# xuhao1/TaichiSLAM

Hardware: AMD Instinct MI355X
Metric: depth-frames/s integrated (640x480->512^3 TSDF) (higher is better)
Workload: dtype f16 storage / f32 + int64 fixed-point arithmetic; 1 GPU; BASELINE configs[1]: single 640x480 u16 depth stream (sphere room r=3 m, 1 deg/frame) -> DenseTSDF 512^3 / 2 cm, recast_step 2, max_ray 5 m; one stream+submap per GPU

## Files before the change

taichislam_amd/csrc/tsl_integrate.hip:

```cpp
#include "tsl_tsdf.hpp"
#include <hip/hip_ext.h>

namespace tsl {

#ifdef TSL_TIMING
#define TSL_T0() const int _wv = (blockIdx.x * (int)blockDim.x + (int)threadIdx.x) >> 6
#define TSL_TICK(F, k) do { long long _n = wall_clock64(); if (lane_id() == 0 && _wv < 16384) (F).dbg[_wv * 16 + (k)] = _n; } while (0)
#else
#define TSL_T0() do {} while (0)
#define TSL_TICK(F, k) do {} while (0)
#endif

#define SCATTER_TILE 4096

struct RayRegs { float pf0, pf1, pf2, d0, d1, d2, P0, P1, P2, w; long long qden; int n; };

__device__ __forceinline__ uint32_t wave_min_u32(uint32_t v)
{
    for (int d = 32; d > 0; d >>= 1) { const uint32_t o = (uint32_t)__shfl_xor((int)v, d); v = o < v ? o : v; }
    return v;
}
__device__ __forceinline__ RayRegs make_ray(const uint4 rec, int n, const FrameParams& P)
{
    RayRegs R;
    R.n = n;
    R.pf0 = h2f((h16)(rec.x & 0xffffu)); R.pf1 = h2f((h16)(rec.x >> 16)); R.pf2 = h2f((h16)(rec.y & 0xffffu));
    R.d0 = h2f((h16)(rec.y >> 16)); R.d1 = h2f((h16)(rec.z & 0xffffu)); R.d2 = h2f((h16)(rec.z >> 16));
    R.w = __uint_as_float(rec.w);
    R.qden = to_fix(R.w);
    R.P0 = R.pf0 + P.T[0]; R.P1 = R.pf1 + P.T[1]; R.P2 = R.pf2 + P.T[2];
    return R;
}
template <bool WITH_N = true>
__device__ __forceinline__ RayRegs load_ray(const FrameDev& F, const FrameParams& P, int r) { return make_ray(F.rayA[r], WITH_N ? F.rayN[r] : 0, P); }
__device__ __forceinline__ void step_voxel(const RayRegs& R, const FrameParams& P, int j, float* x, int* xi)
{
    const float jf = (float)j;
    x[0] = (R.d0 * jf) * P.vs + P.T[0]; x[1] = (R.d1 * jf) * P.vs + P.T[1]; x[2] = (R.d2 * jf) * P.vs + P.T[2];
    xi[0] = rnd_i(div_vs(x[0], P.vs, P.rvs, P.fastdiv)); xi[1] = rnd_i(div_vs(x[1], P.vs, P.rvs, P.fastdiv)); xi[2] = rnd_i(div_vs(x[2], P.vs, P.rvs, P.fastdiv));
}
__device__ __forceinline__ long long step_term(const RayRegs& R, const float* x)
{
    const float v0 = R.P0 - x[0], v1 = R.P1 - x[1], v2 = R.P2 - x[2];
    const float s2 = (v0 * v0 + v1 * v1) + v2 * v2;
    const float dist = s2 >= 1.2621774483536189e-29f ? sqrt_rn_norm(s2) : sqrt_rn(s2);
    const float dot = (v0 * R.pf0 + v1 * R.pf1) + v2 * R.pf2;
    const float sd = dist * (float)sgn_f(dot);
    return to_fix_wave(R.w * sd);
}
template <bool COOP = true>
__device__ __forceinline__ void mark_occupied(const MapDev& M, const FrameParams& P, const RayRegs& R)
{
    const int oi = rnd_i(div_vs(R.P0, P.vs, P.rvs, P.fastdiv)), oj = rnd_i(div_vs(R.P1, P.vs, P.rvs, P.fastdiv)), ok = rnd_i(div_vs(R.P2, P.vs, P.rvs, P.fastdiv));
    if (in_volume(M, oi, oj, ok)) {
        int l; const int b = brick_of(M, oi, oj, ok, &l);
        const int p = pool_claim<COOP>(M, P.slot, b);
        if (p >= 0) M.occ[(size_t)p * TSL_BRK3 + l] = 1;
    }
}
template <bool COOP = true>
__device__ __forceinline__ int frame_slot_slow(const MapDev& M, const FrameDev& F, int s, int b)
{
    const int sl = COOP ? claim_index(F.slot_tab + b, &F.counters[1], F.max_frame_bricks) : claim_index_1(F.slot_tab + b, &F.counters[1], F.max_frame_bricks);
    if (sl >= 0) {
        const int p = pool_claim<COOP>(M, s, b);
        if (p >= 0) { F.touched[sl] = p; F.touched_b[sl] = b; }
        else return -1;
    } else frame_fail(M, F, 2);
    return sl;
}
__device__ __forceinline__ int frame_slot(const MapDev& M, const FrameDev& F, int s, int b)
{
    const int sl = F.slot_tab[b];
    return sl >= 0 ? sl : frame_slot_slow(M, F, s, b);
}

__device__ __forceinline__ uint32_t apply_update(uint32_t old, long long qnum, long long qden)
{
    const float num = from_fix(qnum), den = from_fix(qden);
    const h16 T0 = (h16)(old & 0xffffu), W0 = (h16)(old >> 16);
    const h16 Tn = f2h((h2f(hmul(T0, W0)) + num) / (h2f(W0) + den));
    float wn = h2f(W0) + den; if (TSL_WMAX < wn) wn = TSL_WMAX;
    return (uint32_t)Tn | ((uint32_t)f2h(wn) << 16);
}
__device__ __forceinline__ uint32_t apply_update_f(uint32_t old, float num, float den)
{
    const h16 T0 = (h16)(old & 0xffffu), W0 = (h16)(old >> 16);
    const h16 Tn = f2h((h2f(hmul(T0, W0)) + num) / (h2f(W0) + den));
    float wn = h2f(W0) + den; if (TSL_WMAX < wn) wn = TSL_WMAX;
    return (uint32_t)Tn | ((uint32_t)f2h(wn) << 16);
}

template <int VARIANT>
__global__ void __launch_bounds__(256) k_integrate(MapDev M, FrameDev F, const FrameParams* __restrict__ Pp)
{
    const FrameParams& P = *Pp;
    const int split = P.split;
    const int gid = blockIdx.x * 256 + threadIdx.x;
    const int r = gid / split, sub = gid - r * split;
    const int nrays = *F.nrays;
    const bool live = r < nrays;
    long long n_ok = 0, n_oob = 0;
    RayRegs R; R.n = 0; R.qden = 0;
    if (live) { R = load_ray(F, P, r); if (sub == 0) mark_occupied(M, P, R); }
    int cur_b = -1; unsigned long long* cur_acc = nullptr;
    int nmax = R.n;
    if (VARIANT == 1) { for (int d = 32; d > 0; d >>= 1) { int o = __shfl_xor(nmax, d); nmax = o > nmax ? o : nmax; } }
    const int iters = (nmax + split - 1) / split;
    for (int it = 0; it < iters; ++it) {
        const int j = 1 + sub + it * split;
        const bool act = live && j <= R.n;
        unsigned long long* dst = nullptr;
        long long qn = 0;
        if (act) {
            float x[3]; int xi[3];
            step_voxel(R, P, j, x, xi);
            if (in_volume(M, xi[0], xi[1], xi[2])) {
                qn = step_term(R, x);
                int l; const int b = brick_of(M, xi[0], xi[1], xi[2], &l);
                if (b != cur_b) { cur_b = b; const int sl = frame_slot(M, F, P.slot, b); cur_acc = sl >= 0 ? F.acc + (size_t)sl * (TSL_BRK3 * 2) : nullptr; }
                if (cur_acc) { dst = cur_acc + (size_t)l * 2; ++n_ok; }
            } else ++n_oob;
        }
        if (VARIANT == 1) {
            const unsigned long long m = __ballot(dst != nullptr);
            if (m) {
                const int leader = (int)__builtin_ctzll(m);
                const unsigned long long lead = __shfl((unsigned long long)dst, leader);
                const bool same = (dst == nullptr) || ((unsigned long long)dst == lead);
                if (__all(same)) {
                    const long long sn = wave_sum_ll(dst ? qn : 0), sdn = wave_sum_ll(dst ? R.qden : 0);
                    if (lane_id() == leader) {
                        __hip_atomic_fetch_add(dst, (unsigned long long)sn, __ATOMIC_RELAXED, __HIP_MEMORY_SCOPE_AGENT);
                        __hip_atomic_fetch_add(dst + 1, (unsigned long long)sdn, __ATOMIC_RELAXED, __HIP_MEMORY_SCOPE_AGENT);
                    }
                    continue;
                }
            }
        }
        if (dst) {
            __hip_atomic_fetch_add(dst, (unsigned long long)qn, __ATOMIC_RELAXED, __HIP_MEMORY_SCOPE_AGENT);
            __hip_atomic_fetch_add(dst + 1, (unsigned long long)R.qden, __ATOMIC_RELAXED, __HIP_MEMORY_SCOPE_AGENT);
        }
    }
    n_ok = wave_sum_ll(n_ok); n_oob = wave_sum_ll(n_oob);
    if (lane_id() == 0) {
        if (n_ok) atomic_add_i64(&F.stats->steps, n_ok);
        if (n_oob) atomic_add_i64(&F.stats->steps_oob, n_oob);
    }
}

__global__ void __launch_bounds__(256) k_finalize(MapDev M, FrameDev F, const int* list, const int* nlist)
{
    const int ntouched = min(F.counters[1], F.max_frame_bricks);
    const int nwork = list ? min(*nlist, F.max_frame_bricks) : ntouched;
    long long uniq = 0;
    for (int q = blockIdx.x; q < nwork; q += gridDim.x) {
        const int sl = list ? list[q] : q;
        const int p = F.touched[sl];
        if (threadIdx.x == 0) M.touch[p] = 1;
        ulonglong2* acc = reinterpret_cast<ulonglong2*>(F.acc + (size_t)sl * (TSL_BRK3 * 2));
        uint32_t* tw = M.tw + (size_t)p * TSL_BRK3;
        int8_t* obs = M.obs + (size_t)p * TSL_BRK3;
        ulonglong2 a[TSL_BRK3 / 256]; uint32_t old[TSL_BRK3 / 256];
#pragma unroll
        for (int q = 0; q < TSL_BRK3 / 256; ++q) { a[q] = acc[q * 256 + threadIdx.x]; old[q] = tw[q * 256 + threadIdx.x]; }
#pragma unroll
        for (int q = 0; q < TSL_BRK3 / 256; ++q) {
            const int l = q * 256 + threadIdx.x;
            if (a[q].y != 0ull) {
                tw[l] = apply_update(old[q], (long long)a[q].x, (long long)a[q].y);
                obs[l] = 1;
                acc[l] = make_ulonglong2(0ull, 0ull);
                ++uniq;
            }
        }
    }
    for (int sl = blockIdx.x * 256 + threadIdx.x; sl < ntouched; sl += gridDim.x * 256) F.slot_tab[F.touched_b[sl]] = TSL_EMPTY;
    uniq = wave_sum_ll(uniq);
    if (lane_id() == 0 && uniq) atomic_add_i64(&F.stats->unique, uniq);
    if (!list && blockIdx.x == 0 && threadIdx.x == 0) F.stats->bricks = ntouched;
}

__device__ __forceinline__ int axis_coord(float d, float T, const FrameParams& P, int j) { return rnd_i(div_vs((d * (float)j) * P.vs + T, P.vs, P.rvs, P.fastdiv)); }
__device__ __forceinline__ int axis_cell(int c, int h, int N, int nb) { const int u = c + h; return u < 0 ? -1 : (u >= N ? nb : (u >> 4)); }

__device__ __forceinline__ int next_axis_event(float d, float inv_d, float T, const FrameParams& P, float t_over_vs, int j, int jb, int cell, int h, int N, int nb)
{
    if (j >= jb) return jb + 1;
    int bound;
    bool up;
    if (d > 0.0f) { if (cell >= nb) return jb + 1; up = true; bound = (cell < 0 ? 0 : min((cell + 1) * 16, N)) - h; }
    else if (d < 0.0f) { if (cell < 0) return jb + 1; up = false; bound = (cell >= nb ? N - 1 : cell * 16 - 1) - h; }
    else return jb + 1;
    const float est = ((float)bound + (up ? -0.5f : 0.5f) - t_over_vs) * inv_d;
    int e = (int)fminf(fmaxf(ceilf(est), (float)(j + 1)), (float)jb);
    #define TSL_PRED(q) (up ? (axis_coord(d, T, P, (q)) >= bound) : (axis_coord(d, T, P, (q)) <= bound))
    if (TSL_PRED(e)) { while (e - 1 > j && TSL_PRED(e - 1)) --e; }
    else { ++e; while (e <= jb && !TSL_PRED(e)) ++e; }
    #undef TSL_PRED
    return e;
}

#define LH_SIZE 1024
#define LH_EMPTY (-1)
template <int LOG2 = 10>
__device__ __forceinline__ int lh_slot(int* keys, int b)
{
    unsigned h = ((unsigned)b * 2654435761u) >> (32 - LOG2);
    for (int probe = 0; probe < (1 << LOG2); ++probe) {
        const int k = keys[h];
        if (k == b) return (int)h;
        if (k == LH_EMPTY) { const int old = atomicCAS(&keys[h], LH_EMPTY, b); if (old == LH_EMPTY || old == b) return (int)h; }
        h = (h + 1) & ((1u << LOG2) - 1u);
    }
    return -1;
}

#define SEG_RAY_SLOTS 16
#define SEG_LH_LOG2 9
#define SEG_LH (1 << SEG_LH_LOG2)
template <bool FUSED>
__global__ void __launch_bounds__(256) k_segments(MapDev M, BatchDev B)
{
    if ((int)blockIdx.y >= B.n) return;
    const FrameDev& F = B.f[blockIdx.y];
    const FrameParams& P = *B.p[blockIdx.y];
    __shared__ int s_key[SEG_LH];
    __shared__ int s_cnt[SEG_LH];
    TSL_T0();
    TSL_TICK(F, 8);
    for (int i = threadIdx.x; i < SEG_LH; i += 256) { s_key[i] = LH_EMPTY; s_cnt[i] = 0; }
    __syncthreads();
    TSL_TICK(F, 0);

    const int split = P.split;
    const int gid = blockIdx.x * 256 + threadIdx.x;
    const int r = gid / split, sub = gid - r * split;
    const int nrays = FUSED ? F.counters[6] : *F.nrays;
    long long n_ok = 0, n_oob = 0;
    const bool working = __any(r < nrays);
    const int spl = SEG_RAY_SLOTS / split;
    unsigned long long* myseg = F.seg + (size_t)gid * spl;
    int nslot = 0;
    bool ok = r < nrays;
    uint4 rec = make_uint4(0, 0, 0, 0);
    int nsteps = 0;
    if (FUSED) {
        const int lane = threadIdx.x & 63;
        bool big = false;
        int gn = 0, sl = 0;
        uint32_t first = 0;
        unsigned long long vkey = 0ull;
        ok = false;
        if (r < nrays && sub == 0) {
            sl = F.act[r];
            const uint4* sp = reinterpret_cast<const uint4*>(F.htab + sl);
            const uint4 w0 = sp[0], w1 = sp[1], w2 = sp[2], w3 = sp[3];
            vkey = ((unsigned long long)w0.x | ((unsigned long long)w0.y << 32)) - 1ull;
            gn = (int)w0.z;
            if (gn > H_INL) big = true;
            else {
                uint32_t id[H_INL] = { w0.w, w1.x, w1.y, w1.z, w1.w, w2.x, w2.y, w2.z, w2.w, w3.x, w3.y, w3.z, w3.w };
                uint2 pl[H_INL];
#pragma unroll
                for (int q = 0; q < H_INL; ++q) {
                    if (q >= gn) id[q] = 0xffffffffu;
                    pl[q] = q < gn ? F.pix[id[q]] : make_uint2(0u, 0u);
                }
                PixAcc A = {};
                for (int k = 0; k < gn; ++k) {
                    uint32_t best = 0xffffffffu; uint2 bp = make_uint2(0u, 0u);
#pragma unroll
                    for (int q = 0; q < H_INL; ++q) { const bool t = id[q] < best; best = t ? id[q] : best; bp.x = t ? pl[q].x : bp.x; bp.y = t ? pl[q].y : bp.y; }
#pragma unroll
                    for (int q = 0; q < H_INL; ++q) id[q] = id[q] == best ? 0xffffffffu : id[q];
                    if (k == 0) first = best;
                    if (P.tex) acc_colour(P, F, best, A);
                    acc_payload(bp, A);
                }
                ok = finish_ray(P, F, A, first, &rec, &nsteps);
            }
        }
        for (unsigned long long bm = __ballot(big); bm; bm &= bm - 1ull) {
            const int src = (int)__builtin_ctzll(bm);
            const int n = __shfl(gn, src), sl0 = __shfl(sl, src);
            const unsigned long long vk = ((unsigned long long)(uint32_t)__shfl((int)(vkey >> 32), src) << 32) | (unsigned long long)(uint32_t)__shfl((int)(uint32_t)vkey, src);
            const int nblk = (n + H_INL - 1) / H_INL;
            const uint32_t hmask = (1u << P.hlog2) - 1u;
            auto find_block = [&](int bq) -> int {
                if (bq == 0) return sl0;
                const unsigned long long k2 = h_key(vk, bq);
                uint32_t h = h_hash64(k2, P.hlog2);
                for (uint32_t probe = 0; probe <= hmask; ++probe) {
                    const unsigned long long cur = F.htab[h].key;
                    if (cur == k2) return (int)h;
                    if (cur == H_EMPTY) return -1;
                    h = (h + 1u) & hmask;
                }
                return -1;
            };
            const int mine = lane < nblk ? find_block(lane) : -1;
            const bool too_many = n > GROUP_BIG_CAP;
            if (too_many && lane == 0) atomicOr(M.err, 8);
            PixAcc A = {};
            long long last = -1; uint32_t f0 = 0;
            for (int k = 0; k < n && !too_many; ++k) {
                uint32_t best = 0xffffffffu;
                for (int bq = lane; bq < nblk; bq += 64) {
                    const int hs = bq == lane ? mine : find_block(bq);
                    if (hs < 0) continue;
                    const int cb = min(H_INL, n - bq * H_INL);
                    const uint32_t* ids = F.htab[hs].pix;
                    for (int q = 0; q < cb; ++q) { const uint32_t v = ids[q]; if ((long long)v > last && v < best) best = v; }
                }
                best = wave_min_u32(best);
                if (best == 0xffffffffu) break;
                if (k == 0) f0 = best;
                acc_pixel(P, F, best, A);
                last = (long long)best;
            }
            uint4 rc; int ns = 0;
            const bool k2 = A.cnt == n && finish_ray(P, F, A, f0, &rc, &ns, lane == src);
            if (lane == src) { rec = rc; nsteps = ns; ok = k2; first = f0; }
        }
        if (r < nrays && sub == 0) {
            F.rayA[r] = rec; F.rayFirst[r] = first;
            if (P.seq) {
                uint32_t u[3];
#pragma unroll
                for (int a = 0; a < 3; ++a) {
                    unsigned long long x = (vkey >> (2 - a)) & 0x1249249249249249ull;
                    x = (x | (x >> 2)) & 0x10c30c30c30c30c3ull; x = (x | (x >> 4)) & 0x100f00f00f00f00full; x = (x | (x >> 8)) & 0x1f0000ff0000ffull;
                    x = (x | (x >> 16)) & 0x1f00000000ffffull; x = (x | (x >> 32)) & 0x1fffffull;
                    u[a] = (uint32_t)x;
                }
                const unsigned long long nblk = (unsigned long long)(P.pcl_ext / P.pcl_blk), blk = (unsigned long long)P.pcl_blk;
                const unsigned long long kb = ((u[0] / P.pcl_blk) * nblk + (u[1] / P.pcl_blk)) * nblk + (u[2] / P.pcl_blk);
                const unsigned long long kl = ((u[0] % P.pcl_blk) * blk + (u[1] % P.pcl_blk)) * blk + (u[2] % P.pcl_blk);
                reinterpret_cast<unsigned long long*>(F.keys)[r] = kb * blk * blk * blk + kl;
                F.rayN[r] = ok ? nsteps : 0;
            }
        }
        block_count_add(&F.stats->v_pcl, r < nrays && sub == 0);
        block_count_add(&F.stats->v_skipped, r < nrays && sub == 0 && !ok);
        if (gid == 0) *F.nrays = nrays;
        const int src = lane - sub;
        rec.x = (uint32_t)__shfl((int)rec.x, src); rec.y = (uint32_t)__shfl((int)rec.y, src); rec.z = (uint32_t)__shfl((int)rec.z, src); rec.w = (uint32_t)__shfl((int)rec.w, src);
        nsteps = __shfl(nsteps, src);
        ok = __shfl((int)ok, src) != 0;
    }
    if (ok) {
        const RayRegs R = FUSED ? make_ray(rec, nsteps, P) : load_ray(F, P, r);
        if (sub == 0) mark_occupied(M, P, R);
        TSL_TICK(F, 1);
        const int len = (R.n + split - 1) / split;
        const int ja = 1 + sub * len, jb = min(R.n, ja + len - 1);
        const float d[3] = { R.d0, R.d1, R.d2 };
        const float id[3] = { __builtin_amdgcn_rcpf(R.d0), __builtin_amdgcn_rcpf(R.d1), __builtin_amdgcn_rcpf(R.d2) };
        const float tv[3] = { P.T[0] / P.vs, P.T[1] / P.vs, P.T[2] / P.vs };
        const int hh[3] = { M.hN, M.hN, M.hNz }, NN[3] = { M.N, M.N, M.Nz }, nb[3] = { M.nbx, M.nbx, M.nbz };
        if (ja <= jb) {
            int cell[3], ev[3];
#pragma unroll
            for (int a = 0; a < 3; ++a) {
                cell[a] = axis_cell(axis_coord(d[a], P.T[a], P, ja), hh[a], NN[a], nb[a]);
                ev[a] = next_axis_event(d[a], id[a], P.T[a], P, tv[a], ja, jb, cell[a], hh[a], NN[a], nb[a]);
            }
            int j = ja;
            while (j <= jb) {
                const int e = min(min(ev[0], ev[1]), ev[2]);
                const bool inside = cell[0] >= 0 && cell[0] < nb[0] && cell[1] >= 0 && cell[1] < nb[1] && cell[2] >= 0 && cell[2] < nb[2];
                if (inside) {
                    const int b = (cell[0] * M.nbx + cell[1]) * M.nbz + cell[2];
                    n_ok += e - j;
                    for (int j0 = j; j0 < e; j0 += SEG_MAX_CNT) {
                        const int cnt = min(e - j0, SEG_MAX_CNT);
                        const unsigned long long en = ((unsigned long long)b << STG_B_SHIFT) | ((unsigned long long)r << (SEG_CNT_BITS + SEG_J_BITS)) |
                                                      ((unsigned long long)j0 << SEG_CNT_BITS) | (unsigned long long)cnt;
                        bool stored = true;
                        if (nslot < spl) myseg[nslot++] = en;
                        else {
                            const long long pos = (long long)nrays * SEG_RAY_SLOTS + __hip_atomic_fetch_add(&F.counters[2], 1, __ATOMIC_RELAXED, __HIP_MEMORY_SCOPE_AGENT);
                            if (pos < F.seg_cap) F.seg[pos] = en; else { stored = false; frame_fail(M, F, 4); }
                        }
                        if (stored) {
                            const int hs = lh_slot<SEG_LH_LOG2>(s_key, b);
                            if (hs >= 0) atomicAdd(&s_cnt[hs], 1);
                            else if (__hip_atomic_fetch_add(&F.bhist[b], 1, __ATOMIC_RELAXED, __HIP_MEMORY_SCOPE_AGENT) == 0) {
                                const int q = __hip_atomic_fetch_add(&F.counters[1], 1, __ATOMIC_RELAXED, __HIP_MEMORY_SCOPE_AGENT);
                                if (q < F.max_frame_bricks) F.act_b[q] = b; else frame_fail(M, F, 2);
                            }
                        }
                    }
                } else n_oob += e - j;
                j = e;
                if (j > jb) break;
#pragma unroll
                for (int a = 0; a < 3; ++a) if (ev[a] == j) {
                    cell[a] += d[a] > 0.0f ? 1 : -1;
                    ev[a] = next_axis_event(d[a], id[a], P.T[a], P, tv[a], j, jb, cell[a], hh[a], NN[a], nb[a]);
                }
            }
        }
    }
    if (r < nrays) for (int q = nslot; q < spl; ++q) myseg[q] = ~0ull;
    TSL_TICK(F, 2);
    __syncthreads();
    TSL_TICK(F, 3);
    TSL_TICK(F, 5);
    for (int i = threadIdx.x; i < SEG_LH; i += 256) {
        const int c = s_cnt[i];
        const int b = c ? s_key[i] : 0;
        const bool first = c && __hip_atomic_fetch_add(&F.bhist[b], c, __ATOMIC_RELAXED, __HIP_MEMORY_SCOPE_AGENT) == 0;
        const int q = wave_reserve(&F.counters[1], first);
        if (first) { if (q < F.max_frame_bricks) F.act_b[q] = b; else frame_fail(M, F, 2); }
    }
    TSL_TICK(F, 6);
#ifdef TSL_TIMING
    if (lane_id() == 0 && _wv < 16384) F.dbg[_wv * 16 + 15] = working;
#endif
    (void)working;
    n_ok = wave_sum_ll(n_ok); n_oob = wave_sum_ll(n_oob);
    {
        __shared__ long long s_steps[2];
        if (threadIdx.x == 0) { s_steps[0] = 0; s_steps[1] = 0; }
        __syncthreads();
        if (lane_id() == 0) {
            if (n_ok) atomicAdd(reinterpret_cast<unsigned long long*>(&s_steps[0]), (unsigned long long)n_ok);
            if (n_oob) atomicAdd(reinterpret_cast<unsigned long long*>(&s_steps[1]), (unsigned long long)n_oob);
        }
        __syncthreads();
        if (threadIdx.x == 0) {
            if (s_steps[0]) atomic_add_i64(&F.stats->steps, s_steps[0]);
            if (s_steps[1]) atomic_add_i64(&F.stats->steps_oob, s_steps[1]);
        }
    }
}

__device__ __forceinline__ int plan_class(int w) { return w >= 2560 ? 0 : (w >= 1280 ? 1 : (w >= 512 ? 2 : 3)); }
__global__ void __launch_bounds__(256) k_plan(MapDev M, BatchDev B, int psegs, int unit_max, int unit_half)
{
    if ((int)blockIdx.y >= B.n) return;
    const int y = blockIdx.y;
    const FrameDev& F = B.f[y];
    const int listed = F.counters[1];
    const int nact = min(listed, F.max_frame_bricks);
    if ((int)blockIdx.x * 256 >= nact && blockIdx.x) return;
    const int i = blockIdx.x * 256 + threadIdx.x;
    int v = 0, b = 0, np = 0, pcls = -1, ucls = -1, tm = 0, wb = 0, tmu = 0, tmp = 0, wu = 0;
    if (i < nact) {
        b = F.act_b[i];
        v = F.bhist[b];
        int vq[TSL_NB];
#pragma unroll
        for (int q = 0; q < TSL_NB; ++q) { vq[q] = q < B.n ? B.f[q].bhist[b] : 0; if (vq[q] > 0) tm |= 1 << q; wb += vq[q]; }
        if (wb > unit_max) { tmp = tm; }
        else if (wb > unit_half) {
            int acc = 0;
#pragma unroll
            for (int q = 0; q < TSL_NB; ++q) if ((tm >> q) & 1) { if (2 * acc < wb) { tmu |= 1 << q; wu += vq[q]; } else tmp |= 1 << q; acc += vq[q]; }
        } else { tmu = tm; wu = wb; }
        if (tmu && (tmu & -tmu) == (1 << y)) ucls = plan_class(wu);
        if (((tmp >> y) & 1) && v > 0) { np = (v + psegs - 1) / psegs; pcls = plan_class((v + np - 1) / np); }
    }
    const int off = block_reserve_n(&F.counters[3], v);
    const int s0 = block_reserve_n(&B.f[0].counters[HDR_SLAB], np);
    int p0 = 0, u0 = 0;
    for (int c = 0; c < PLAN_NCLS; ++c) {
        const int q = block_reserve_n(&F.counters[HDR_PARTS + c], pcls == c ? np : 0); if (pcls == c) p0 = q;
        const int u = block_reserve_n(&B.f[0].counters[HDR_UNITS + c], ucls == c ? 1 : 0); if (ucls == c) u0 = u;
    }
    if (i < nact) {
        F.boffset[b] = off;
        F.bnseg[b] = v;
        const int pool = (np || ucls >= 0) ? pool_claim<false>(M, B.p[y]->slot, b) : -1;
        if (ucls >= 0) {
            if (u0 < B.f[0].unit_cap) B.f[0].unit_tab[(size_t)ucls * B.f[0].unit_cap + u0] = make_int4(b, wu, pool, tmu);
            else for (int q = 0; q < B.n; ++q) if ((tm >> q) & 1) frame_fail(M, B.f[q], 2);
        }
        if (np && pool >= 0) {
            if ((tmp & -tmp) == (1 << y)) {
                const int hi = __hip_atomic_fetch_add(&B.f[0].counters[HDR_HEAVY], 1, __ATOMIC_RELAXED, __HIP_MEMORY_SCOPE_AGENT);
                if (hi < B.f[0].max_frame_bricks) B.f[0].heavy_tab[hi] = make_int4(b, pool, tmp, 0);
                else for (int q = 0; q < B.n; ++q) if ((tm >> q) & 1) frame_fail(M, B.f[q], 2);
            }
            if (s0 + np > F.max_frame_bricks || np >= (1 << PART_NP_BITS) || p0 + np > F.part_cap) frame_fail(M, F, 2);
            else {
                F.bslab[b] = s0 | (np << SLAB_SLOT_BITS);
                const int per = (v + np - 1) / np;
                int4* tab = F.part_tab + (size_t)pcls * F.part_cap;
                for (int k = 0; k < np; ++k) {
                    const int pos = k * per, n = min(v, pos + per) - pos;
                    tab[p0 + k] = make_int4(off + pos, (int)((uint32_t)n | ((uint32_t)np << 16)), pool, s0 + k);
                }
            }
        }
    }
    if (i == 0) { F.stats->bricks = listed; if (listed > F.max_frame_bricks) frame_fail(M, F, 2); }
}

__global__ void __launch_bounds__(256) k_scatter(BatchDev B)
{
    if ((int)blockIdx.y >= B.n) return;
    const FrameDev& F = B.f[blockIdx.y];
    __shared__ int s_key[LH_SIZE];
    __shared__ int s_cnt[LH_SIZE];
    __shared__ int s_base[LH_SIZE];
    if (B.p[blockIdx.y]->group) {
        const int na = F.counters[6], nx = F.counters[7];
        for (int i = blockIdx.x * 256 + threadIdx.x; i < na + nx; i += gridDim.x * 256) {
            HSlot* const hs = F.htab + (i < na ? F.act[i] : F.actx[i - na]);
            hs->key = H_EMPTY; hs->cnt = 0;
        }
    }
    const int total = (int)min((long long)*F.nrays * SEG_RAY_SLOTS + F.counters[2], (long long)F.seg_cap);
    const int ntiles = (total + SCATTER_TILE - 1) / SCATTER_TILE;
    for (int tile = blockIdx.x; tile < ntiles; tile += gridDim.x) {
        for (int i = threadIdx.x; i < LH_SIZE; i += 256) { s_key[i] = LH_EMPTY; s_cnt[i] = 0; }
        __syncthreads();
        const int t0 = tile * SCATTER_TILE;
        unsigned long long key[SCATTER_TILE / 256]; int rank[SCATTER_TILE / 256]; int hs[SCATTER_TILE / 256];
#pragma unroll
        for (int q = 0; q < SCATTER_TILE / 256; ++q) {
            const int i = t0 + q * 256 + threadIdx.x;
            rank[q] = -1; hs[q] = -1;
            if (i < total) {
                key[q] = F.seg[i];
                if (key[q] != ~0ull) {
                    const int b = (int)(key[q] >> STG_B_SHIFT);
                    hs[q] = lh_slot<10>(s_key, b);
                    if (hs[q] >= 0) rank[q] = atomicAdd(&s_cnt[hs[q]], 1);
                    else rank[q] = F.boffset[b] + __hip_atomic_fetch_add(&F.bcursor[b], 1, __ATOMIC_RELAXED, __HIP_MEMORY_SCOPE_AGENT);
                }
            }
        }
        __syncthreads();
        for (int i = threadIdx.x; i < LH_SIZE; i += 256) {
            const int c = s_cnt[i];
            if (c) { const int b = s_key[i]; s_base[i] = F.boffset[b] + __hip_atomic_fetch_add(&F.bcursor[b], c, __ATOMIC_RELAXED, __HIP_MEMORY_SCOPE_AGENT); }
        }
        __syncthreads();
#pragma unroll
        for (int q = 0; q < SCATTER_TILE / 256; ++q)
            if (rank[q] >= 0) F.seg_sorted[(hs[q] >= 0 ? s_base[hs[q]] : 0) + rank[q]] = key[q];
        __syncthreads();
    }
}

#ifdef TSL_NOSWZ
__device__ __forceinline__ int acc_swz5(int l) { return l; }
#else
__device__ __forceinline__ int acc_swz5(int l) { return l ^ (((l >> 8) ^ (l >> 5)) & 31); }
#endif
struct StepK { float vs, rvs, T0, T1, T2; int hN, hNz; };

template <bool FASTDIV>
__device__ __forceinline__ void step_eval(const RayRegs& R, const StepK& K, int j, int* slot, float* qf)
{
    const float jf = (float)j;
    const float x0 = (R.d0 * jf) * K.vs + K.T0, x1 = (R.d1 * jf) * K.vs + K.T1, x2 = (R.d2 * jf) * K.vs + K.T2;
    const int i0 = rnd_i(div_vs(x0, K.vs, K.rvs, FASTDIV ? 1 : 0)), i1 = rnd_i(div_vs(x1, K.vs, K.rvs, FASTDIV ? 1 : 0)), i2 = rnd_i(div_vs(x2, K.vs, K.rvs, FASTDIV ? 1 : 0));
    *slot = acc_swz5((((i0 + K.hN) & 15) << 8) | (((i1 + K.hN) & 15) << 4) | ((i2 + K.hNz) & 15));
    const float v0 = R.P0 - x0, v1 = R.P1 - x1, v2 = R.P2 - x2;
    const float s2 = (v0 * v0 + v1 * v1) + v2 * v2;
    const float dist = sqrt_rn_norm(fmaxf(s2, 1.2621774483536189e-29f));
    const float dot = (v0 * R.pf0 + v1 * R.pf1) + v2 * R.pf2;
    const float sd = dot == 0.0f ? 0.0f : copysignf(dist, dot);
    *qf = rintf((R.w * sd) * TSL_FIX_SCALE);
}

__device__ __forceinline__ bool fits_i32(long long q) { return q == (long long)(int)q; }
__device__ __forceinline__ float from_fix32(long long q) { return (float)(int)q * (float)TSL_FIX_INV; }

#define FLUSH_CHUNK 4
template <int N>
__device__ __forceinline__ void apply_chunk(const uint32_t* old, const long long* qn, const long long* qd, uint32_t* nv, bool all_small)
{
    if (all_small) {
#pragma unroll
        for (int q = 0; q < N; ++q) nv[q] = apply_update_f(old[q], from_fix32(qn[q]), from_fix32(qd[q]));
    } else {
#pragma unroll
        for (int q = 0; q < N; ++q) nv[q] = apply_update_f(old[q], from_fix(qn[q]), from_fix(qd[q]));
    }
}

__device__ __forceinline__ int uni(int v) { return __builtin_amdgcn_readfirstlane(v); }
#define IT_UNIT 0
#define IT_POOL 1
#define IT_SLAB 2
#define IT_NP   3
#define IT_TMALL 4
#define IT_FMASK 5
#define IT_OFF  6
#define IT_N    (IT_OFF + TSL_NB)
#define IT_WORDS (IT_N + TSL_NB + 2)
#define NRANGE (PLAN_NCLS * (TSL_NB + 1))

template <bool TEX, bool FASTDIV, int NT, int SPT, int WPE>
__global__ void __launch_bounds__(NT, WPE) k_integrate_batch(MapDev M, BatchDev B, int kind)
{
    constexpr int CSEGS = SPT * NT, VPT = TSL_BRK3 / NT, CH = VPT < FLUSH_CHUNK ? VPT : FLUSH_CHUNK;
    static_assert(VPT <= 16, "the written / first-touch masks hold 16 voxels per thread");
#ifdef TSL_EXP_SLOT16
    __shared__ ulonglong2 s_acc[TSL_BRK3];
#define S_NUM(i) s_acc[i].x
#define S_DEN(i) s_acc[i].y
#else
    __shared__ unsigned long long s_num[TSL_BRK3];
    __shared__ unsigned long long s_den[TSL_BRK3];
#define S_NUM(i) s_num[i]
#define S_DEN(i) s_den[i]
#endif
    __shared__ unsigned long long s_keys[CSEGS];
    __shared__ uint32_t s_win[TEX ? TSL_BRK3 : 1];
    __shared__ int s_bin[64];
    __shared__ int s_claim[2];
    __shared__ int s_uq[TSL_NB];
    __shared__ int s_cum[NRANGE + 1];
    __shared__ int s_it[3][IT_WORDS];
    uint32_t okmask = 0u;
#pragma unroll
    for (int q = 0; q < TSL_NB; ++q) if (q < B.n) {
        const FrameDev& Fq = B.f[q];
        if (Fq.counters[HDR_FAIL] == 0) okmask |= 1u << q;
        const int nact = min(Fq.counters[1], Fq.max_frame_bricks);
        for (int i = blockIdx.x * NT + threadIdx.x; i < nact; i += gridDim.x * NT) { const int b = Fq.act_b[i]; Fq.bhist[b] = 0; Fq.bcursor[b] = 0; }
    }
    if (threadIdx.x < TSL_NB) s_uq[threadIdx.x] = 0;
    if (threadIdx.x == 0) {
        int acc = 0, k = 0;
#ifdef TSL_CLASS_MAJOR
        for (int c = 0; c < PLAN_NCLS; ++c) {
            s_cum[k++] = acc; acc += min(B.f[0].counters[HDR_UNITS + c], B.f[0].unit_cap);
            for (int q = 0; q < TSL_NB; ++q) { s_cum[k++] = acc; if ((okmask >> q) & 1u) acc += min(B.f[q].counters[HDR_PARTS + c], B.f[q].part_cap); }
        }
#else
        for (int c = 0; c < PLAN_NCLS; ++c) { s_cum[k++] = acc; if (kind != 2) acc += min(B.f[0].counters[HDR_UNITS + c], B.f[0].unit_cap); }
        for (int c = 0; c < PLAN_NCLS; ++c)
            for (int q = 0; q < TSL_NB; ++q) { s_cum[k++] = acc; if (kind != 1 && ((okmask >> q) & 1u)) acc += min(B.f[q].counters[HDR_PARTS + c], B.f[q].part_cap); }
#endif
        s_cum[NRANGE] = acc;
        s_claim[0] = __hip_atomic_fetch_add(&B.f[0].counters[kind == 2 ? HDR_CLAIM2 : HDR_CLAIM], 1, __ATOMIC_RELAXED, __HIP_MEMORY_SCOPE_AGENT);
    }
    __syncthreads();
    const int total = uni(s_cum[NRANGE]);
    int* const claim = &B.f[0].counters[kind == 2 ? HDR_CLAIM2 : HDR_CLAIM];
    auto entry_of = [&](int r, int* kq) -> int4 {
        int k = 0;
#pragma unroll
        for (int j = 1; j < NRANGE; ++j) k += r >= uni(s_cum[j]) ? 1 : 0;
#ifdef TSL_CLASS_MAJOR
        const int local = r - uni(s_cum[k]), cls = k / (TSL_NB + 1), sub = k - cls * (TSL_NB + 1);
#else
        const int local = r - uni(s_cum[k]), cls = k < PLAN_NCLS ? k : (k - PLAN_NCLS) / TSL_NB, sub = k < PLAN_NCLS ? 0 : 1 + (k - PLAN_NCLS) % TSL_NB;
#endif
        *kq = sub - 1;
        if (sub == 0) return B.f[0].unit_tab[(size_t)cls * B.f[0].unit_cap + local];
        const FrameDev& Fq = B.f[sub - 1];
        return Fq.part_tab[(size_t)cls * Fq.part_cap + local];
    };
    auto info_of = [&](const int4 e, int kq, int* io, int* in) {
        *io = 0; *in = 0;
        const int q = threadIdx.x;
        if (q < TSL_NB) {
            if (kq < 0) { if ((((uint32_t)e.w) & okmask) >> q & 1u) { *io = B.f[q].boffset[e.x]; *in = B.f[q].bnseg[e.x]; } }
            else if (q == kq) { *io = e.x; *in = e.y & 0xffff; }
        }
    };
    auto commit = [&](int slot, const int4 e, int kq, int io, int in) {
        int* it = s_it[slot];
        if (threadIdx.x < TSL_NB) { it[IT_OFF + threadIdx.x] = io; it[IT_N + threadIdx.x] = in; }
        if (threadIdx.x == 0) {
            const uint32_t tm = kq < 0 ? (uint32_t)e.w & okmask : 1u << kq;
            uint32_t fm = tm;
            int pool = e.z;
            if (fm == 0u) { fm = 1u; pool = -1; }
            it[IT_UNIT] = kq < 0 ? 1 : 0; it[IT_POOL] = pool; it[IT_SLAB] = kq < 0 ? 0 : e.w; it[IT_NP] = kq < 0 ? 1 : (e.y >> 16) & ((1 << PART_NP_BITS) - 1);
            it[IT_TMALL] = (int)tm; it[IT_FMASK] = (int)fm;
        }
    };
    const int r0 = uni(s_claim[0]);
    if (r0 >= total) return;
    { int kq, io, in; const int4 e = entry_of(r0, &kq); info_of(e, kq, &io, &in); commit(0, e, kq, io, in); }
    __syncthreads();
    auto steps_of = [&](int sl, uint32_t fm) -> int {
        int n = 0;
#pragma unroll
        for (int q = 0; q < TSL_NB; ++q) if ((fm >> q) & 1u) n += max(1, (uni(s_it[sl][IT_N + q]) + CSEGS - 1) / CSEGS);
        return n;
    };
    long long uniq = 0;
    int t = 0, slot = 0, c = 0; (void)t;
    int n_known = 0;
    bool exhausted = false;
    int f = __builtin_ctz((uint32_t)uni(s_it[0][IT_FMASK]));

    unsigned long long kk[SPT]; uint4 recs[SPT]; uint32_t wids[SPT];
#define TSL_SORT_DEAL(KIN, NSEG, FD)                                                                                    \
    {                                                                                                                   \
        int rr[SPT];                                                                                                    \
        _Pragma("unroll") for (int q = 0; q < SPT; ++q) {                                                               \
            const int i = q * NT + (int)threadIdx.x; rr[q] = -1;                                                        \
            if (i < (NSEG)) rr[q] = atomicAdd(&s_bin[63 - (int)(KIN[q] & 63ull)], 1);                                   \
        }                                                                                                               \
        __syncthreads();                                                                                                \
        if (threadIdx.x < 64) {                                                                                         \
            const int cb = s_bin[threadIdx.x]; int inc = cb;                                                            \
            for (int d = 1; d < 64; d <<= 1) { const int o = __shfl_up(inc, d); if ((int)threadIdx.x >= d) inc += o; }  \
            s_bin[threadIdx.x] = inc - cb;                                                                              \
        }                                                                                                               \
        __syncthreads();                                                                                                \
        _Pragma("unroll") for (int q = 0; q < SPT; ++q) if (rr[q] >= 0) s_keys[s_bin[63 - (int)(KIN[q] & 63ull)] + rr[q]] = KIN[q]; \
        __syncthreads();                                                                                                \
        _Pragma("unroll") for (int q = 0; q < SPT; ++q) {                                                               \
            const int i = q * NT + ((q & 1) ? NT - 1 - (int)threadIdx.x : (int)threadIdx.x);                            \
            if (i < (NSEG)) {                                                                                           \
                kk[q] = s_keys[i];                                                                                      \
                const int r = (int)((kk[q] >> (SEG_CNT_BITS + SEG_J_BITS)) & ((1u << STG_RAY_BITS) - 1));               \
                recs[q] = (FD).rayA[r];                                                                                 \
                wids[q] = TEX ? (FD).rayFirst[r] + 1u : 0u;                                                             \
            }                                                                                                           \
        }                                                                                                               \
        if (threadIdx.x < 64) s_bin[threadIdx.x] = 0;               \
    }
#define TSL_PRIME(SL, FQ)                                                                                               \
    {                                                                                                                   \
        const FrameDev& F0 = B.f[FQ];                                                                                   \
        const int off0 = uni(s_it[SL][IT_OFF + (FQ)]), nseg0 = min(uni(s_it[SL][IT_N + (FQ)]), CSEGS);                  \
        unsigned long long k0[SPT];                                                                                     \
        _Pragma("unroll") for (int q = 0; q < SPT; ++q) { const int i = q * NT + threadIdx.x; k0[q] = i < nseg0 ? F0.seg_sorted[off0 + i] : 0ull; } \
        TSL_SORT_DEAL(k0, nseg0, F0)                                                                                    \
    }

    {
#ifdef TSL_EXP_SLOT16
        for (int i = threadIdx.x; i < TSL_BRK3; i += NT) s_acc[i] = make_ulonglong2(0ull, 0ull);
#else
        ulonglong2* zn = reinterpret_cast<ulonglong2*>(s_num); ulonglong2* zd = reinterpret_cast<ulonglong2*>(s_den);
        for (int i = threadIdx.x; i < TSL_BRK3 / 2; i += NT) { zn[i] = make_ulonglong2(0ull, 0ull); zd[i] = make_ulonglong2(0ull, 0ull); }
#endif
        if (TEX) for (int i = threadIdx.x; i < TSL_BRK3; i += NT) s_win[i] = 0u;
        if (threadIdx.x < 64) s_bin[threadIdx.x] = 0;
        __syncthreads();
        TSL_PRIME(0, f)
    }
    uint32_t old[VPT];
    uint32_t vmask = 0u;
    bool have_old = false;
    for (;;) {
        const int* const it = s_it[slot];
        const int slot1 = slot == 2 ? 0 : slot + 1, slot2 = slot == 0 ? 2 : slot - 1;
        const bool unit = uni(it[IT_UNIT]) != 0;
        const int p = uni(it[IT_POOL]), rk = uni(it[IT_SLAB]);
        const uint32_t fmask = (uint32_t)uni(it[IT_FMASK]);
        const int n_f = uni(it[IT_N + f]);
        const FrameDev& F = B.f[f];
        const FrameParams& P = *B.p[f];
        const StepK K = { P.vs, P.rvs, P.T[0], P.T[1], P.T[2], M.hN, M.hNz };
        const uint32_t later = fmask >> (f + 1);
        const bool first_frame = (fmask & ((1u << f) - 1u)) == 0u, last_frame = later == 0u;
        const bool first_step = first_frame && c == 0;
        const int nseg = min(CSEGS, n_f - c * CSEGS);
        const bool last_chunk = (c + 1) * CSEGS >= n_f;
        const bool last_step = last_chunk && last_frame;
        int known = max(1, (n_f + CSEGS - 1) / CSEGS) - 1 - c + steps_of(slot, later << (f + 1));
        if (n_known >= 1) known += steps_of(slot1, (uint32_t)uni(s_it[slot1][IT_FMASK]));
        const bool do_claim = !exhausted && n_known < 2 && known <= 1;
        if (do_claim && threadIdx.x == 0) s_claim[0] = __hip_atomic_fetch_add(claim, 1, __ATOMIC_RELAXED, __HIP_MEMORY_SCOPE_AGENT);
#ifdef TSL_TIMING
        long long* const _rec = F.dbg + 131072 + (size_t)blockIdx.x * 128 + (size_t)(t < 16 ? t : 15) * 8;
        if (threadIdx.x == 0 && first_step) { _rec[0] = wall_clock64(); _rec[1] = (unit ? 1 : 0) | (uni(it[IT_NP]) << 8) | ((long long)fmask << 32); _rec[2] = 0; _rec[5] = 0; }
        if (threadIdx.x == 0 && c == 0) _rec[2] += n_f;
        long long* const _ph = F.dbg + 196608 + (size_t)blockIdx.x * 128 + (size_t)(t < 16 ? t : 15) * 8;
        if (threadIdx.x == 0 && first_step) { _ph[0] = _ph[1] = _ph[2] = _ph[3] = _ph[4] = 0; }
        const long long _ta = wall_clock64();
#endif
        const bool has_next = !last_step || n_known >= 1;
        int fx = f, cx = c + 1, slotx = slot;
        if (last_chunk) {
            cx = 0;
            if (!last_frame) fx = f + 1 + __builtin_ctz(later);
            else if (has_next) { slotx = slot1; fx = __builtin_ctz((uint32_t)uni(s_it[slotx][IT_FMASK])); }
        }
        const FrameDev& Fx = B.f[fx];
        unsigned long long kn[SPT];
        const int offx = uni(s_it[slotx][IT_OFF + fx]) + cx * CSEGS;
        const int nsegn = has_next ? min(CSEGS, uni(s_it[slotx][IT_N + fx]) - cx * CSEGS) : 0;
#pragma unroll
        for (int q = 0; q < SPT; ++q) { const int i = q * NT + threadIdx.x; kn[q] = i < nsegn ? Fx.seg_sorted[offx + i] : 0ull; }
        const uint32_t* const twr = M.tw + (size_t)(p >= 0 ? p : 0) * TSL_BRK3;
        if (first_step) { have_old = false; vmask = 0u; }
        if (!TEX && unit && p >= 0 && first_step) {
#pragma unroll
            for (int q = 0; q < VPT; ++q) old[q] = twr[q * NT + threadIdx.x];
            have_old = true;
        }
#pragma unroll
        for (int q = 0; q < SPT; ++q) {
            const int i = q * NT + ((q & 1) ? NT - 1 - (int)threadIdx.x : (int)threadIdx.x);
            if (i >= nseg) continue;
            const unsigned long long key = kk[q];
            const int cnt = (int)(key & ((1u << SEG_CNT_BITS) - 1)), j0 = (int)((key >> SEG_CNT_BITS) & ((1u << SEG_J_BITS) - 1));
            const RayRegs R = make_ray(recs[q], 0, P);
            const uint32_t wid = wids[q];
#ifndef TSL_EXP_STAGGER
#define TSL_EXP_STAGGER 27
#endif
            int off = ((int)((threadIdx.x * (unsigned)TSL_EXP_STAGGER) & 63u) * cnt) >> 6;
            for (int s = 0; s < cnt; s += 2) {
                const int ja = j0 + off; off = (off + 1 == cnt) ? 0 : off + 1;
                const int jb = j0 + off; off = (off + 1 == cnt) ? 0 : off + 1;
                int la, lb; float qa, qb;
                step_eval<FASTDIV>(R, K, ja, &la, &qa);
                step_eval<FASTDIV>(R, K, jb, &lb, &qb);
                long long na = (long long)(int)qa, nb = (long long)(int)qb;
                if (__builtin_expect(__any(!(fabsf(qa) < 2147483648.0f) || !(fabsf(qb) < 2147483648.0f)), 0)) { na = __float2ll_rn(qa); nb = __float2ll_rn(qb); }
                atomicAdd(&S_NUM(la), (unsigned long long)na);
                atomicAdd(&S_DEN(la), (unsigned long long)R.qden);
                if (TEX) atomicMax(&s_win[la], wid);
                const bool vb = s + 1 < cnt;
#ifdef TSL_EXP_ADDZERO
                atomicAdd(&S_NUM(lb), (unsigned long long)(vb ? nb : 0ll));
                atomicAdd(&S_DEN(lb), (unsigned long long)(vb ? R.qden : 0ll));
                if (TEX) atomicMax(&s_win[lb], vb ? wid : 0u);
#else
                if (vb) { atomicAdd(&S_NUM(lb), (unsigned long long)nb); atomicAdd(&S_DEN(lb), (unsigned long long)R.qden); if (TEX) atomicMax(&s_win[lb], wid); }
#endif
            }
        }
        __syncthreads();
#ifdef TSL_TIMING
        if (threadIdx.x == 0 && last_step) _rec[3] = wall_clock64();
        const long long _tb = wall_clock64();
#endif
        bool fetching = false;
        int4 ne = make_int4(0, 0, -1, 0); int nkq = 0, nio = 0, nin = 0;
        if (do_claim) {
            const int r = uni(s_claim[0]);
            if (r < total) { fetching = true; ne = entry_of(r, &nkq); } else exhausted = true;
        }
        if (has_next) TSL_SORT_DEAL(kn, nsegn, Fx)
        if (fetching) info_of(ne, nkq, &nio, &nin);
#ifdef TSL_TIMING
        const long long _tc = wall_clock64();
        if (threadIdx.x == 0) { _ph[0] += _tb - _ta; _ph[1] += _tc - _tb; _ph[4] += 1; }
#endif
        if (!last_chunk) {
            if (fetching) { commit(n_known == 0 ? slot1 : slot2, ne, nkq, nio, nin); ++n_known; __syncthreads(); }
            ++c; continue;
        }
        if (p >= 0 && threadIdx.x == 0) M.touch[p] = 1;
        if (p >= 0 && unit) {
            uint32_t* tw = M.tw + (size_t)p * TSL_BRK3;
            if (!have_old) {
#pragma unroll
                for (int q = 0; q < VPT; ++q) old[q] = tw[q * NT + threadIdx.x];
                have_old = true;
            }
            if (first_frame) {
#pragma unroll
                for (int q = 0; q < VPT; ++q) vmask |= ((old[q] >> 16) == 0u ? 1u : 0u) << (16 + q);
            }
#pragma unroll
            for (int h = 0; h < VPT; h += CH) {
                long long qn[CH], qd[CH]; uint32_t nv[CH]; bool small = true, anyu = false;
#pragma unroll
                for (int q = 0; q < CH; ++q) {
                    const int ls = acc_swz5((h + q) * NT + threadIdx.x);
                    qn[q] = (long long)S_NUM(ls); qd[q] = (long long)S_DEN(ls); S_NUM(ls) = 0ull; S_DEN(ls) = 0ull;
                    small = small && fits_i32(qn[q]) && fits_i32(qd[q]); anyu = anyu || qd[q] != 0;
                }
                if (!__any(anyu)) continue;
                apply_chunk<CH>(old + h, qn, qd, nv, __all(small));
#pragma unroll
                for (int q = 0; q < CH; ++q) {
                    const bool upd = qd[q] != 0;
                    old[h + q] = upd ? nv[q] : old[h + q];
                    vmask |= (upd ? 1u : 0u) << (h + q);
                    uniq += upd ? 1 : 0;
                    if (TEX && upd) {
                        const int l = (h + q) * NT + threadIdx.x;
                        reinterpret_cast<uint2*>(M.col)[(size_t)p * TSL_BRK3 + l] = F.colpix[s_win[acc_swz5(l)] - 1u];
                    }
                }
            }
            if (TEX) for (int i = threadIdx.x; i < TSL_BRK3; i += NT) s_win[i] = 0u;
            if (last_frame) {
                int8_t* obs = M.obs + (size_t)p * TSL_BRK3;
#pragma unroll
                for (int q = 0; q < VPT; ++q) {
                    const int l = q * NT + threadIdx.x;
                    if ((vmask >> q) & 1u) {
                        tw[l] = old[q];
                        if ((vmask >> (16 + q)) & 1u) obs[l] = 1;
                    }
                }
            }
        } else if (p >= 0) {
            ulonglong2* acc = reinterpret_cast<ulonglong2*>(F.acc) + (size_t)rk * TSL_BRK3;
#pragma unroll
            for (int q = 0; q < VPT; ++q) {
                const int l = q * NT + threadIdx.x, ls = acc_swz5(l);
                acc[l] = make_ulonglong2(S_NUM(ls), S_DEN(ls));
                S_NUM(ls) = 0ull; S_DEN(ls) = 0ull;
                if (TEX) { F.accw[(size_t)rk * TSL_BRK3 + l] = s_win[ls]; s_win[ls] = 0u; }
            }
        } else {
#ifdef TSL_EXP_SLOT16
            for (int i = threadIdx.x; i < TSL_BRK3; i += NT) s_acc[i] = make_ulonglong2(0ull, 0ull);
#else
            ulonglong2* zn = reinterpret_cast<ulonglong2*>(s_num); ulonglong2* zd = reinterpret_cast<ulonglong2*>(s_den);
            for (int i = threadIdx.x; i < TSL_BRK3 / 2; i += NT) { zn[i] = make_ulonglong2(0ull, 0ull); zd[i] = make_ulonglong2(0ull, 0ull); }
#endif
            if (TEX) for (int i = threadIdx.x; i < TSL_BRK3; i += NT) s_win[i] = 0u;
        }
#ifdef TSL_TIMING
        const long long _td = wall_clock64();
#endif
        {
            const long long u = wave_sum_ll(uniq);
            if (lane_id() == 0 && u) atomicAdd(&s_uq[f], (int)u);
            uniq = 0;
        }
        if (fetching) { commit(n_known == 0 ? slot1 : slot2, ne, nkq, nio, nin); ++n_known; }
#ifdef TSL_TIMING
        if (threadIdx.x == 0 && last_step) _rec[4] = wall_clock64();
        if (threadIdx.x == 0) { _ph[2] += _td - _tc; _ph[3] += wall_clock64() - _td; }
#endif
        if (!has_next && n_known == 0) break;
        __syncthreads();
        c = 0;
        if (last_frame) { ++t; slot = slot1; --n_known; f = __builtin_ctz((uint32_t)uni(s_it[slot][IT_FMASK])); }
        else f = fx;
        if (!has_next) TSL_PRIME(slot, f)
    }
#undef TSL_PRIME
#undef TSL_SORT_DEAL
    __syncthreads();
    if (threadIdx.x < TSL_NB && s_uq[threadIdx.x]) atomic_add_i64(&B.f[threadIdx.x].stats->unique, (long long)s_uq[threadIdx.x]);
}

#ifndef APPLY_SPLIT
#define APPLY_SPLIT 8
#endif
#ifndef APPLY_ROUND
#define APPLY_ROUND 2
#endif
template <bool TEX>
__global__ void __launch_bounds__(256) k_apply_slab(MapDev M, BatchDev B)
{
    __shared__ int s_uq[TSL_NB];
    constexpr int VP = TSL_BRK3 / APPLY_SPLIT / 256;
    uint32_t okmask = 0u;
#pragma unroll
    for (int q = 0; q < TSL_NB; ++q) if (q < B.n && B.f[q].counters[HDR_FAIL] == 0) okmask |= 1u << q;
    const int nheavy = min(B.f[0].counters[HDR_HEAVY], B.f[0].max_frame_bricks);
    const ulonglong2* const slab = reinterpret_cast<const ulonglong2*>(B.f[0].acc);
    if (threadIdx.x < TSL_NB) s_uq[threadIdx.x] = 0;
    __syncthreads();
    for (int item = blockIdx.x; item < nheavy * APPLY_SPLIT; item += gridDim.x) {
        const int4 e = B.f[0].heavy_tab[item / APPLY_SPLIT];
        const int b = e.x, p = e.y;
        const uint32_t tm = (uint32_t)e.z & okmask;
        if (p < 0 || tm == 0u) continue;
        const int l0 = (item % APPLY_SPLIT) * (TSL_BRK3 / APPLY_SPLIT) + (int)threadIdx.x;
        uint32_t* tw = M.tw + (size_t)p * TSL_BRK3;
        int w[TSL_NB];
#pragma unroll
        for (int q = 0; q < TSL_NB; ++q) w[q] = ((tm >> q) & 1u) ? B.f[q].bslab[b] : 0;
        uint32_t cur[VP], first[VP];
#pragma unroll
        for (int k = 0; k < VP; ++k) { cur[k] = tw[l0 + k * 256]; first[k] = cur[k]; }
        ulonglong2 a[TSL_NB][VP]; uint32_t win[TSL_NB][VP];
#pragma unroll
        for (int q = 0; q < TSL_NB; ++q) {
            const bool on = (tm >> q) & 1u;
            const size_t base = (size_t)(w[q] & ((1 << SLAB_SLOT_BITS) - 1)) * TSL_BRK3 + l0;
#pragma unroll
            for (int k = 0; k < VP; ++k) {
                a[q][k] = on ? slab[base + k * 256] : make_ulonglong2(0ull, 0ull);
                win[q][k] = (TEX && on) ? B.f[q].accw[base + k * 256] : 0u;
            }
        }
        int npmax = 0;
#pragma unroll
        for (int q = 0; q < TSL_NB; ++q) npmax = max(npmax, w[q] >> SLAB_SLOT_BITS);
        for (int j0 = 1; j0 < npmax; j0 += APPLY_ROUND) {
            ulonglong2 x[TSL_NB][APPLY_ROUND][VP];
#pragma unroll
            for (int q = 0; q < TSL_NB; ++q) {
                const int np = w[q] >> SLAB_SLOT_BITS, s0 = w[q] & ((1 << SLAB_SLOT_BITS) - 1);
#pragma unroll
                for (int t = 0; t < APPLY_ROUND; ++t) {
                    const bool on = j0 + t < np;
                    const size_t base = (size_t)(s0 + (on ? j0 + t : 0)) * TSL_BRK3 + l0;
#pragma unroll
                    for (int k = 0; k < VP; ++k) {
                        x[q][t][k] = on ? slab[base + k * 256] : make_ulonglong2(0ull, 0ull);
                        if (TEX && on) win[q][k] = max(win[q][k], B.f[q].accw[base + k * 256]);
                    }
                }
            }
#pragma unroll
            for (int q = 0; q < TSL_NB; ++q)
#pragma unroll
                for (int t = 0; t < APPLY_ROUND; ++t)
#pragma unroll
                    for (int k = 0; k < VP; ++k) { a[q][k].x += x[q][t][k].x; a[q][k].y += x[q][t][k].y; }
        }
        bool changed[VP];
#pragma unroll
        for (int k = 0; k < VP; ++k) changed[k] = false;
#pragma unroll
        for (int q = 0; q < TSL_NB; ++q) {
            if (!((tm >> q) & 1u)) continue;
            long long ug = 0;
#pragma unroll
            for (int k = 0; k < VP; ++k) {
                if (a[q][k].y != 0ull) {
                    cur[k] = apply_update(cur[k], (long long)a[q][k].x, (long long)a[q][k].y);
                    changed[k] = true; ++ug;
                    if (TEX) reinterpret_cast<uint2*>(M.col)[(size_t)p * TSL_BRK3 + l0 + k * 256] = B.f[q].colpix[win[q][k] - 1u];
                }
            }
            ug = wave_sum_ll(ug);
            if (lane_id() == 0 && ug) atomicAdd(&s_uq[q], (int)ug);
        }
        __syncthreads();
        if (threadIdx.x < TSL_NB && s_uq[threadIdx.x]) { atomic_add_i64(&B.f[threadIdx.x].stats->unique, (long long)s_uq[threadIdx.x]); s_uq[threadIdx.x] = 0; }
        int8_t* obs = M.obs + (size_t)p * TSL_BRK3;
#pragma unroll
        for (int k = 0; k < VP; ++k) if (changed[k]) {
            tw[l0 + k * 256] = cur[k];
            if ((first[k] >> 16) == 0u) obs[l0 + k * 256] = 1;
        }
    }
}

int check_variant2(tsl_tsdf* m)
{
    TSL_REQUIRE(m->F.max_frame_bricks <= 4096 && m->P.max_steps_f < (float)(1 << SEG_J_BITS) && m->F.max_points < (1 << STG_RAY_BITS) && m->nb3 < (1 << 24) && 3 * m->pcl_bits <= H_BLOCK_SHIFT,
                "variant 2: ray too long / too many points / too many bricks for the segment key (use variant 1)");
    return TSL_OK;
}

int launch_segments(tsl_tsdf* m, const BatchDev& B, const FrameParams* hp, int total, hipStream_t st)
{
    const FrameParams& P = hp[0];
    if (P.variant != 2) return TSL_OK;
    const int iblocks = (int)(((int64_t)total * P.split + 255) / 256);
    prof_begin(m, TSL_K_SEGMENTS, st);
    if (P.group) hipLaunchKernelGGL(k_segments<true>, dim3(iblocks, B.n), dim3(256), 0, st, m->M, B);
    else hipLaunchKernelGGL(k_segments<false>, dim3(iblocks, B.n), dim3(256), 0, st, m->M, B);
    prof_end(m, st);
    int unit_max = m->unit_max <= m->unit_floor ? m->unit_max : std::max(m->unit_floor, (int)((long long)m->unit_max * B.n / TSL_NB));
    int unit_half = std::min(unit_max, m->unit_half <= 2048 ? m->unit_half : std::max(2048, (int)((long long)m->unit_half * B.n / TSL_NB)));
    if (P.seq && m->seq_impl) unit_max = unit_half = 1 << 30;
    prof_begin(m, TSL_K_BIN, st);
    hipLaunchKernelGGL(k_plan, dim3((B.f[0].max_frame_bricks + 255) / 256, B.n), dim3(256), 0, st, m->M, B, m->chunks * m->wg * m->spt, unit_max, unit_half);
    hipLaunchKernelGGL(k_scatter, dim3(256, B.n), dim3(256), 0, st, B);
    prof_end(m, st);
    return TSL_OK;
}

int launch_brick(tsl_tsdf* m, const BatchDev& B, const FrameParams& P, int kind, hipStream_t st, hipEvent_t start, hipEvent_t stop)
{
    const int bg = kind == 2 ? m->pgrid : (B.n <= 2 ? (m->bgrid + 1) / 2 : (kind == 1 ? m->ugrid : m->bgrid));
#define TSL_LAUNCH_IB(TEXV, FD) do { \
        if (m->wg == 512 && m->spt == 2 && !TEXV) hipExtLaunchKernelGGL((k_integrate_batch<false, FD, 512, 2, 4>), dim3((2 * m->ncu * bg + 99) / 100), dim3(512), 0, st, start, stop, 0, m->M, B, kind); \
        else if (m->wg == 512) hipExtLaunchKernelGGL((k_integrate_batch<TEXV, FD, 512, 4, 2>), dim3((m->ncu * bg + 99) / 100), dim3(512), 0, st, start, stop, 0, m->M, B, kind); \
        else hipExtLaunchKernelGGL((k_integrate_batch<TEXV, FD, 256, 4, (TEXV ? 1 : 2)>), dim3(((TEXV ? 1 : 2) * m->ncu * bg + 99) / 100), dim3(256), 0, st, start, stop, 0, m->M, B, kind); } while (0)
    if (P.tex) { if (P.fastdiv) TSL_LAUNCH_IB(true, true); else TSL_LAUNCH_IB(true, false); }
    else { if (P.fastdiv) TSL_LAUNCH_IB(false, true); else TSL_LAUNCH_IB(false, false); }
#undef TSL_LAUNCH_IB
    TSL_HIP(hipGetLastError());
    return TSL_OK;
}
int launch_slab_apply(tsl_tsdf* m, const BatchDev& B, const FrameParams& P)
{
    prof_begin(m, TSL_K_FINALIZE);
    if (P.tex) hipLaunchKernelGGL(k_apply_slab<true>, dim3(16 * m->ncu), dim3(256), 0, m->stream_, m->M, B);
    else hipLaunchKernelGGL(k_apply_slab<false>, dim3(16 * m->ncu), dim3(256), 0, m->stream_, m->M, B);
    prof_end(m);
    TSL_HIP(hipGetLastError());
    return TSL_OK;
}
int launch_apply_batch(tsl_tsdf* m, const BatchDev& B, const FrameParams& P, hipEvent_t start, hipEvent_t stop)
{
    const int rc = launch_brick(m, B, P, 0, m->stream_, start, stop);
    return rc ? rc : launch_slab_apply(m, B, P);
}

int launch_apply(tsl_tsdf* m, FSet& S, int total)
{
    FrameParams& P = m->P;
    FrameDev& F = S.F;
    const int iblocks = (int)(((int64_t)total * P.split + 255) / 256);
    prof_begin(m, TSL_K_INTEGRATE);
    if (P.variant == 1) hipLaunchKernelGGL(k_integrate<1>, dim3(iblocks), dim3(256), 0, m->stream_, m->M, F, (const FrameParams*)S.Pd);
    else hipLaunchKernelGGL(k_integrate<0>, dim3(iblocks), dim3(256), 0, m->stream_, m->M, F, (const FrameParams*)S.Pd);
    prof_end(m);
    prof_begin(m, TSL_K_FINALIZE);
    hipLaunchKernelGGL(k_finalize, dim3(1024), dim3(256), 0, m->stream_, m->M, F, (const int*)nullptr, (const int*)nullptr);
    prof_end(m);
    TSL_HIP(hipGetLastError());
    return TSL_OK;
}

}
```

taichislam_amd/csrc/tsl_tsdf.hip:

```cpp
#include "tsl_tsdf.hpp"
#include <rocprim/rocprim.hpp>
#include <algorithm>
#include <cmath>
#include <cstdio>
#include <cstdlib>
#include <cstring>
#include <mutex>

namespace tsl {

static thread_local std::string g_err;
void set_error(const std::string& s) { g_err = s; }

__device__ __forceinline__ uint32_t part1by2_32(uint32_t x)
{
    x &= 0x3ffu;
    x = (x ^ (x << 16)) & 0xff0000ffu;
    x = (x ^ (x << 8)) & 0x0300f00fu;
    x = (x ^ (x << 4)) & 0x030c30c3u;
    x = (x ^ (x << 2)) & 0x09249249u;
    return x;
}
__device__ __forceinline__ uint64_t part1by2_64(uint64_t x)
{
    x &= 0x1fffffull;
    x = (x | (x << 32)) & 0x1f00000000ffffull;
    x = (x | (x << 16)) & 0x1f0000ff0000ffull;
    x = (x | (x << 8)) & 0x100f00f00f00f00full;
    x = (x | (x << 4)) & 0x10c30c30c30c30c3ull;
    x = (x | (x << 2)) & 0x1249249249249249ull;
    return x;
}
template <typename K> struct KeyOps;
template <> struct KeyOps<uint32_t> {
    static __device__ __forceinline__ uint32_t make(int x, int y, int z) { return (part1by2_32(x) << 2) | (part1by2_32(y) << 1) | part1by2_32(z); }
    static __device__ __host__ __forceinline__ uint32_t invalid(int bits) { return 1u << (3 * bits); }
};
template <> struct KeyOps<uint64_t> {
    static __device__ __forceinline__ uint64_t make(int x, int y, int z) { return (part1by2_64(x) << 2) | (part1by2_64(y) << 1) | part1by2_64(z); }
    static __device__ __host__ __forceinline__ uint64_t invalid(int bits) { return 1ull << (3 * bits); }
};

__device__ __forceinline__ int group_insert(const FrameDev& F, unsigned long long vkey, bool inside, uint32_t pid, int log2n, bool* opened, int* xslot);

template <typename K>
__global__ void __launch_bounds__(256) k_voxelize_depth(BatchDev B)
{
    const int fq = blockIdx.y;
    if (fq >= B.n) return;
    const FrameDev& F = B.f[fq];
    const FrameParams& P = *B.p[fq];
    if (P.points) return;
    K* __restrict__ keys = reinterpret_cast<K*>(F.keys);
    const uint16_t* __restrict__ depth = static_cast<const uint16_t*>(P.input);
    const int tiles_x = (P.ww + 15) >> 4;
    if ((int)blockIdx.x >= tiles_x * ((P.hh + 15) >> 4)) return;
    const int ty = blockIdx.x / tiles_x, tx = blockIdx.x - ty * tiles_x;
    const int jj = ty * 16 + ((int)threadIdx.x >> 4), ii = tx * 16 + ((int)threadIdx.x & 15);
    const int p = jj * P.ww + ii;
    bool gate = false, inside = false, opened = false;
    int slot = -1, xslot = -1;
    unsigned long long vkey = 0ull;
    if (jj < P.hh && ii < P.ww) {
        const int j = jj * P.step, i = ii * P.step;
        const uint16_t d = depth[(size_t)jj * P.rstride + (size_t)ii * P.cstride];
        K key = KeyOps<K>::invalid(P.pcl_bits);
        uint2 payload = make_uint2(0u, 0u);
        const float df = (float)d;
        if (d != 0 && !(df > P.thr_max) && !(df < P.thr_min)) {
            gate = true;
            const float dep = df / 1000.0f;
            const float px = ((float)i - P.cx) * dep / P.fx;
            const float py = ((float)j - P.cy) * dep / P.fy;
            const float pz = dep;
            const float mx = (P.R[0] * px + P.R[1] * py) + P.R[2] * pz;
            const float my = (P.R[3] * px + P.R[4] * py) + P.R[5] * pz;
            const float mz = (P.R[6] * px + P.R[7] * py) + P.R[8] * pz;
            const int cx = rnd_i(div_vs(mx, P.vs, P.rvs, P.fastdiv)) - P.pcl_lo, cy = rnd_i(div_vs(my, P.vs, P.rvs, P.fastdiv)) - P.pcl_lo, cz = rnd_i(div_vs(mz, P.vs, P.rvs, P.fastdiv)) - P.pcl_lo;
            if (cx >= 0 && cx < P.pcl_ext && cy >= 0 && cy < P.pcl_ext && cz >= 0 && cz < P.pcl_ext) {
                inside = true;
                key = KeyOps<K>::make(cx, cy, cz);
                payload.x = (uint32_t)f2h(mx) | ((uint32_t)f2h(my) << 16);
                payload.y = (uint32_t)f2h(mz) | ((uint32_t)f2h(dep) << 16);
            }
        }
        F.pix[p] = payload;
        if (!P.group) { keys[p] = key; F.vals[p] = (uint32_t)p; }
        vkey = (unsigned long long)key;
    }
    if (P.group) {
        slot = group_insert(F, vkey, inside, (uint32_t)p, P.hlog2, &opened, &xslot);
        const int q = block_reserve(&F.counters[6], opened); if (opened) F.act[q] = slot;
        const int x = wave_reserve(&F.counters[7], xslot >= 0); if (xslot >= 0) F.actx[x] = xslot;
    }
    block_count_add(&F.stats->p_valid, inside);
    block_count_add(&F.stats->p_oob, gate && !inside);
}

template <typename K>
__global__ void __launch_bounds__(256) k_voxelize_points(BatchDev B)
{
    const int fq = blockIdx.y;
    if (fq >= B.n) return;
    const FrameDev& F = B.f[fq];
    const FrameParams& P = *B.p[fq];
    if (!P.points || (int)blockIdx.x * 256 >= P.total) return;
    K* __restrict__ keys = reinterpret_cast<K*>(F.keys);
    const float* __restrict__ xyz = static_cast<const float*>(P.input);
    const int n = P.total;
    const int p = blockIdx.x * 256 + threadIdx.x;
    bool gate = false, inside = false, opened = false;
    int slot = -1, xslot = -1;
    unsigned long long vkey = 0ull;
    if (p < n) {
        const float px = xyz[(size_t)p * 3], py = xyz[(size_t)p * 3 + 1], pz = xyz[(size_t)p * 3 + 2];
        const float mx = (P.R[0] * px + P.R[1] * py) + P.R[2] * pz;
        const float my = (P.R[3] * px + P.R[4] * py) + P.R[5] * pz;
        const float mz = (P.R[6] * px + P.R[7] * py) + P.R[8] * pz;
        const float len = sqrt_rn((mx * mx + my * my) + mz * mz);
        K key = KeyOps<K>::invalid(P.pcl_bits);
        uint2 payload = make_uint2(0u, 0u);
        if (len < P.max_ray_f) {
            gate = true;
            const int cx = rnd_i(div_vs(mx, P.vs, P.rvs, P.fastdiv)) - P.pcl_lo, cy = rnd_i(div_vs(my, P.vs, P.rvs, P.fastdiv)) - P.pcl_lo, cz = rnd_i(div_vs(mz, P.vs, P.rvs, P.fastdiv)) - P.pcl_lo;
            if (cx >= 0 && cx < P.pcl_ext && cy >= 0 && cy < P.pcl_ext && cz >= 0 && cz < P.pcl_ext) {
                inside = true;
                key = KeyOps<K>::make(cx, cy, cz);
                payload.x = (uint32_t)f2h(mx) | ((uint32_t)f2h(my) << 16);
                payload.y = (uint32_t)f2h(mz) | ((uint32_t)f2h(len) << 16);
            }
        }
        F.pix[p] = payload;
        if (!P.group) { keys[p] = key; F.vals[p] = (uint32_t)p; }
        vkey = (unsigned long long)key;
    }
    if (P.group) {
        slot = group_insert(F, vkey, inside, (uint32_t)p, P.hlog2, &opened, &xslot);
        const int q = block_reserve(&F.counters[6], opened); if (opened) F.act[q] = slot;
        const int x = wave_reserve(&F.counters[7], xslot >= 0); if (xslot >= 0) F.actx[x] = xslot;
    }
    block_count_add(&F.stats->p_valid, inside);
    block_count_add(&F.stats->p_oob, gate && !inside);
}

template <typename K>
__global__ void __launch_bounds__(256) k_build_rays(const FrameParams* __restrict__ Pp, FrameDev F, const K* __restrict__ keys_s)
{
    const FrameParams& P = *Pp;
    const int total = P.total;
    const int i = blockIdx.x * 256 + threadIdx.x;
    const K bad = KeyOps<K>::invalid(P.pcl_bits);
    bool head = false, ok = false;
    uint4 rec = make_uint4(0, 0, 0, 0);
    int nsteps = 0;
    uint32_t first = 0;
    if (i < total) {
        const K k = keys_s[i];
        head = (k != bad) && (i == 0 || keys_s[i - 1] != k);
        if (head) {
            PixAcc A = {};
            first = F.vals_s[i];
            for (int q = i; q < total && keys_s[q] == k; ++q) acc_pixel(P, F, F.vals_s[q], A);
            ok = finish_ray(P, F, A, first, &rec, &nsteps);
        }
    }
    const int r = block_reserve(F.nrays, ok);
    if (ok) { F.rayA[r] = rec; F.rayN[r] = nsteps; F.rayFirst[r] = first; }
    block_count_add(&F.stats->v_pcl, head);
    block_count_add(&F.stats->v_skipped, head && !ok);
}

__device__ __forceinline__ int group_insert(const FrameDev& F, unsigned long long vkey, bool inside, uint32_t pid, int log2n, bool* opened, int* xslot)
{
    HSlot* const tab = F.htab;
    const uint32_t mask = (1u << log2n) - 1u;
    const int lane = lane_id();
    const uint32_t klo = (uint32_t)vkey, khi = (uint32_t)(vkey >> 32);
    int leader = lane, grank = 0, gsize = 1;
    for (unsigned long long todo = __ballot(inside); todo; ) {
        const int l0 = (int)__builtin_ctzll(todo);
        const uint32_t lo = (uint32_t)__builtin_amdgcn_readlane((int)klo, l0), hi = (uint32_t)__builtin_amdgcn_readlane((int)khi, l0);
        const bool mine = inside && klo == lo && khi == hi;
        const unsigned long long grp = __ballot(mine);
        if (mine) { leader = l0; grank = rank_below(grp); gsize = popc64(grp); }
        todo &= ~grp;
    }
    int h = -1, r0 = 0;
    if (inside && lane == leader) {
        const unsigned long long k0 = h_key(vkey, 0);
        uint32_t hh = h_hash64(k0, log2n);
        for (;;) {
            const unsigned long long cur = atomicCAS(&tab[hh].key, H_EMPTY, k0);
            if (cur == H_EMPTY) { *opened = true; break; }
            if (cur == k0) break;
            hh = (hh + 1u) & mask;
        }
        h = (int)hh;
        r0 = atomicAdd(&tab[hh].cnt, gsize);
    }
    h = __shfl(h, leader); r0 = __shfl(r0, leader);
    if (!inside) return -1;
    const int r = r0 + grank;
    if (r < H_INL) tab[h].pix[r] = pid;
    else {
        const unsigned long long k2 = h_key(vkey, r / H_INL);
        uint32_t h2 = h_hash64(k2, log2n);
        for (;;) {
            const unsigned long long cur = atomicCAS(&tab[h2].key, H_EMPTY, k2);
            if (cur == H_EMPTY) { *xslot = (int)h2; break; }
            if (cur == k2) break;
            h2 = (h2 + 1u) & mask;
        }
        tab[h2].pix[r % H_INL] = pid;
    }
    return h;
}

__global__ void __launch_bounds__(256) k_count_active(MapDev M, int s, long long* out)
{
    long long c = 0;
    for (int b = blockIdx.x; b < M.nb3; b += gridDim.x) {
        const int p = pool_lookup_ro(M, s, b);
        if (p < 0) continue;
        const int8_t* obs = M.obs + (size_t)p * TSL_BRK3;
        for (int l = threadIdx.x; l < TSL_BRK3; l += 256) c += obs[l] > 0;
    }
    c = wave_sum_ll(c);
    if (lane_id() == 0 && c) __hip_atomic_fetch_add(out, c, __ATOMIC_RELAXED, __HIP_MEMORY_SCOPE_AGENT);
}

__device__ __forceinline__ void voxel_ijk(const MapDev& M, int b, int l, int* i, int* j, int* k)
{
    const int bk = b % M.nbz, bj = (b / M.nbz) % M.nbx, bi = b / (M.nbz * M.nbx);
    *i = bi * 16 + (l >> 8) - M.hN; *j = bj * 16 + ((l >> 4) & 15) - M.hN; *k = bk * 16 + (l & 15) - M.hNz;
}

__global__ void __launch_bounds__(256) k_export_sparse(MapDev M, int s, int mode, int16_t* idx, uint16_t* t, uint16_t* w, int8_t* occ, uint16_t* col,
                                                       long long cap, int* counter)
{
    for (int b = blockIdx.x; b < M.nb3; b += gridDim.x) {
        const int p = pool_lookup_ro(M, s, b);
        if (p < 0) continue;
        for (int l0 = 0; l0 < TSL_BRK3; l0 += 256) {
            const int l = l0 + threadIdx.x;
            const size_t v = (size_t)p * TSL_BRK3 + l;
            const bool pred = mode == 0 ? (M.obs[v] > 0) : (M.occ[v] != 0);
            const int o = wave_reserve(counter, pred);
            if (pred && o < cap) {
                int i, j, k; voxel_ijk(M, b, l, &i, &j, &k);
                idx[(size_t)o * 3] = (int16_t)i; idx[(size_t)o * 3 + 1] = (int16_t)j; idx[(size_t)o * 3 + 2] = (int16_t)k;
                const uint32_t tv = M.tw[v];
                if (t) t[o] = (uint16_t)(tv & 0xffffu);
                if (w) w[o] = (uint16_t)(tv >> 16);
                if (occ) occ[o] = M.occ[v];
                if (col && M.col) for (int a = 0; a < 3; ++a) col[(size_t)o * 3 + a] = M.col[v * 4 + a];
            }
        }
    }
}

__global__ void __launch_bounds__(256) k_import_sparse(MapDev M, int s, const int16_t* idx, const uint16_t* t, const uint16_t* w, const int8_t* occ,
                                                       const uint16_t* col, long long n)
{
    const long long q = (long long)blockIdx.x * 256 + threadIdx.x;
    if (q >= n) return;
    const int i = idx[q * 3], j = idx[q * 3 + 1], k = idx[q * 3 + 2];
    if (!in_volume(M, i, j, k)) return;
    int l; const int b = brick_of(M, i, j, k, &l);
    const int p = pool_claim(M, s, b);
    if (p < 0) return;
    const size_t v = (size_t)p * TSL_BRK3 + l;
    M.tw[v] = (uint32_t)t[q] | ((uint32_t)w[q] << 16);
    M.occ[v] = occ ? occ[q] : (int8_t)0;
    if (col && M.col) for (int a = 0; a < 3; ++a) M.col[v * 4 + a] = col[q * 3 + a];
    M.obs[v] = 1;
}

struct PoseF { float R[9], T[3]; };
__device__ __forceinline__ int colormap_index(float z, float lo, float hi)
{
    float t = ((z - lo) / (hi - lo)) * 1023.0f;
    if (t > 1023.0f) t = 1023.0f;
    if (!(t > 0.0f)) t = 0.0f;
    return (int)t;
}
__device__ __forceinline__ void voxel_xyz(const PoseF& B, int is_global, float vs, int i, int j, int k, float* o)
{
    const float p0 = (float)i * vs, p1 = (float)j * vs, p2 = (float)k * vs;
    if (is_global) { o[0] = p0; o[1] = p1; o[2] = p2; return; }
    for (int a = 0; a < 3; ++a) o[a] = ((B.R[a * 3] * p0 + B.R[a * 3 + 1] * p1) + B.R[a * 3 + 2] * p2) + B.T[a];
}

__global__ void __launch_bounds__(256) k_export_particles(MapDev M, int s, int mode, PoseF B, int is_global, float vs, float thres, float zfloor, float zceil,
                                                          int slice_index, float slice_dz, const float* __restrict__ cmap,
                                                          float* xyz, float* rgb, float* val, long long cap, int* counter)
{
    for (int b = blockIdx.x; b < M.nb3; b += gridDim.x) {
        const int p = pool_lookup_ro(M, s, b);
        if (p < 0) continue;
        for (int l0 = 0; l0 < TSL_BRK3; l0 += 256) {
            const int l = l0 + threadIdx.x;
            const size_t v = (size_t)p * TSL_BRK3 + l;
            const int8_t ob = M.obs[v];
            const float tv = h2f((h16)(M.tw[v] & 0xffffu));
            int i, j, k; voxel_ijk(M, b, l, &i, &j, &k);
            float o[3] = {0, 0, 0};
            bool pred;
            if (mode == 0) {
                pred = (ob == 1) && (fabsf(tv) < thres);
                if (pred) { voxel_xyz(B, is_global, vs, i, j, k, o); pred = !(o[2] > zceil || o[2] < zfloor); }
            } else {
                pred = (ob > 0) && ((float)slice_index - slice_dz < (float)k) && ((float)k < (float)slice_index + slice_dz);
                if (pred) voxel_xyz(B, is_global, vs, i, j, k, o);
            }
            const int idx = wave_reserve(counter, pred);
            if (pred && idx < cap) {
                for (int a = 0; a < 3; ++a) xyz[(size_t)idx * 3 + a] = o[a];
                if (mode == 1 && val) val[idx] = tv;
                if (rgb) {
                    if (mode == 0 && M.col) { for (int a = 0; a < 3; ++a) rgb[(size_t)idx * 3 + a] = h2f(M.col[v * 4 + a]); }
                    else {
                        const int ci = mode == 0 ? colormap_index(o[2], zfloor, zceil) : colormap_index(tv, -0.5f, 0.5f);
                        for (int a = 0; a < 3; ++a) rgb[(size_t)idx * 3 + a] = cmap[ci * 3 + a];
                    }
                }
            }
        }
    }
}

__global__ void __launch_bounds__(256) k_pack_pointcloud2(const float* __restrict__ xyz, const float* __restrict__ rgb, float* __restrict__ out, long long n, int stride)
{
    const long long q = (long long)blockIdx.x * 256 + threadIdx.x;
    if (q >= n * stride) return;
    const long long row = q / stride; const int c = (int)(q - row * stride);
    out[q] = c < 3 ? xyz[row * 3 + c] : rgb[row * 3 + c - 3];
}

__global__ void __launch_bounds__(256) k_reset_bricks(MapDev M, int nused)
{
    for (int p = blockIdx.x; p < nused; p += gridDim.x) {
        uint32_t* tw = M.tw + (size_t)p * TSL_BRK3;
        uint32_t* ob = reinterpret_cast<uint32_t*>(M.obs + (size_t)p * TSL_BRK3);
        uint32_t* oc = reinterpret_cast<uint32_t*>(M.occ + (size_t)p * TSL_BRK3);
        for (int l = threadIdx.x; l < TSL_BRK3; l += 256) tw[l] = 0u;
        for (int l = threadIdx.x; l < TSL_BRK3 / 4; l += 256) { ob[l] = 0u; oc[l] = 0u; }
        if (M.col) { uint2* c = reinterpret_cast<uint2*>(M.col + (size_t)p * TSL_BRK3 * 4); for (int l = threadIdx.x; l < TSL_BRK3; l += 256) c[l] = make_uint2(0u, 0u); }
        if (threadIdx.x == 0) M.table[M.owner[p]] = TSL_EMPTY;
    }
}

__global__ void __launch_bounds__(256) k_verify_div(float vs, float rvs, unsigned long long* bad)
{
    unsigned long long nbad = 0;
    for (unsigned long long i = (unsigned long long)blockIdx.x * 256 + threadIdx.x; i < (1ull << 32); i += (unsigned long long)gridDim.x * 256) {
        const float x = __uint_as_float((uint32_t)i);
        const float ax = fabsf(x);
        if (!(ax >= 7.8886090522101181e-31f) || !(ax < 2147483648.0f * vs)) continue;
        const float q = x / vs;
        const float f = div_vs(x, vs, rvs, 1);
        if (__float_as_uint(q) != __float_as_uint(f)) ++nbad;
    }
    if (nbad) atomicAdd(bad, nbad);
}

__global__ void __launch_bounds__(256) k_selftest(int which, unsigned long long* bad)
{
    unsigned long long nbad = 0;
    for (unsigned long long i = (unsigned long long)blockIdx.x * 256 + threadIdx.x; i < (1ull << 32); i += (unsigned long long)gridDim.x * 256) {
        const float x = __uint_as_float((uint32_t)i);
        if (which == 0) {
            if (!(fabsf(x) < 2147483648.0f)) continue;
            if (rnd_i(x) != rnd_i_ref(x)) ++nbad;
        } else {
            if (!(x >= 1.2621774483536189e-29f) || !(x < INFINITY)) continue;
            if (__float_as_uint(sqrt_rn_norm(x)) != __float_as_uint(sqrt_rn(x))) ++nbad;
        }
    }
    if (nbad) atomicAdd(bad, nbad);
}

int grow(void** p, size_t* have, size_t need)
{
    if (*have >= need) return TSL_OK;
    if (*p) (void)hipFree(*p);
    *p = nullptr; *have = 0;
    size_t want = need + need / 4 + 4096;
    TSL_HIP(hipMalloc(p, want));
    *have = want;
    return TSL_OK;
}

int dev_alloc(tsl_tsdf* m, void** p, size_t bytes, int fill)
{
    TSL_HIP(hipMalloc(p, bytes));
    TSL_HIP(hipMemsetAsync(*p, fill, bytes, m->stream_));
    m->bytes += (int64_t)bytes;
    return TSL_OK;
}

void prof_begin(tsl_tsdf* m, int kid, hipStream_t st, int count)
{
    if (m->prof_group) return;
    m->prof_open = false;
    if (!m->prof_on || !((m->prof_mask >> kid) & 1)) return;
    ProfSlot s; s.kid = kid; s.count = count;
    if (m->prof_free.size() >= 2) { s.a = m->prof_free.back(); m->prof_free.pop_back(); s.b = m->prof_free.back(); m->prof_free.pop_back(); }
    else if (hipEventCreate(&s.a) != hipSuccess || hipEventCreate(&s.b) != hipSuccess) return;
    (void)hipEventRecord(s.a, st ? st : m->stream_);
    m->prof.push_back(s);
    m->prof_open = true;
}
bool prof_slot(tsl_tsdf* m, int kid, int count, hipEvent_t* a, hipEvent_t* b)
{
    if (m->prof_group || !m->prof_on || !((m->prof_mask >> kid) & 1)) return false;
    ProfSlot s; s.kid = kid; s.count = count;
    if (m->prof_free.size() >= 2) { s.a = m->prof_free.back(); m->prof_free.pop_back(); s.b = m->prof_free.back(); m->prof_free.pop_back(); }
    else if (hipEventCreate(&s.a) != hipSuccess || hipEventCreate(&s.b) != hipSuccess) return false;
    m->prof.push_back(s);
    *a = s.a; *b = s.b;
    return true;
}
void prof_end(tsl_tsdf* m, hipStream_t st)
{
    if (m->prof_group || !m->prof_open) return;
    (void)hipEventRecord(m->prof.back().b, st ? st : m->stream_);
    m->prof_open = false;
}

void convert_pose(const double* Rb, const double* Tb, const double* R, const double* T, float* outR, float* outT)
{
    const double d[3] = { T[0] - Tb[0], T[1] - Tb[1], T[2] - Tb[2] };
    for (int i = 0; i < 3; ++i) {
        for (int j = 0; j < 3; ++j) {
            double acc = 0.0;
            for (int k = 0; k < 3; ++k) acc += Rb[k * 3 + i] * R[k * 3 + j];
            outR[i * 3 + j] = (float)acc;
        }
        double acc = 0.0;
        for (int k = 0; k < 3; ++k) acc += Rb[k * 3 + i] * d[k];
        outT[i] = (float)acc;
    }
}

static int map_slot(const tsl_tsdf* m, int s) { return m->cfg.is_global_map ? 0 : s; }

static PoseF pose_of(const tsl_tsdf* m, int s)
{
    PoseF B;
    for (int a = 0; a < 9; ++a) B.R[a] = m->baseRf[(size_t)s * 9 + a];
    for (int a = 0; a < 3; ++a) B.T[a] = m->baseTf[(size_t)s * 3 + a];
    return B;
}

__global__ void __launch_bounds__(256) k_stage_host(StageCopy C)
{
    const int k = blockIdx.y;
    const int n = C.n16[k];
    const uint4* __restrict__ src = C.src[k];
    uint4* __restrict__ dst = C.dst[k];
    for (int i = blockIdx.x * 1024 + threadIdx.x; i < n; i += gridDim.x * 1024) {
        uint4 v[4];
#pragma unroll
        for (int u = 0; u < 4; ++u) { const int j = i + u * 256; v[u] = j < n ? src[j] : make_uint4(0u, 0u, 0u, 0u); }
#pragma unroll
        for (int u = 0; u < 4; ++u) { const int j = i + u * 256; if (j < n) dst[j] = v[u]; }
    }
}

__global__ void k_set_params(ParamPack PP, SetPtrs S)
{
    if (threadIdx.x == 0) *S.p[blockIdx.x] = PP.p[blockIdx.x];
    S.header[blockIdx.x][threadIdx.x] = 0;
}

template <typename K>
static int enqueue_phase_a(tsl_tsdf* m, const BatchDev& B, const FrameParams* hp, hipStream_t sa)
{
    const int n = B.n;
    int total = 0, tiles = 0, any_points = 0, any_depth = 0;
    for (int q = 0; q < n; ++q) {
        total = hp[q].total > total ? hp[q].total : total;
        const int t = ((hp[q].ww + 15) / 16) * ((hp[q].hh + 15) / 16);
        if (hp[q].points) any_points = 1; else { any_depth = 1; tiles = t > tiles ? t : tiles; }
    }
    if (total <= 0) return TSL_OK;
    const FrameParams& P0 = hp[0];
    const int blocks = (total + 255) / 256;
    prof_begin(m, TSL_K_VOXELIZE, sa);
    if (any_points) hipLaunchKernelGGL(k_voxelize_points<K>, dim3(blocks, n), dim3(256), 0, sa, B);
    if (any_depth) hipLaunchKernelGGL(k_voxelize_depth<K>, dim3(tiles, n), dim3(256), 0, sa, B);
    prof_end(m, sa);
    if (!P0.group) {
        const FrameDev& F = B.f[0];
        prof_begin(m, TSL_K_SORT, sa);
        size_t tb = m->sort_temp_bytes;
        TSL_HIP(rocprim::radix_sort_pairs(m->fset[m->cur * TSL_NB].sort_temp, tb, reinterpret_cast<K*>(F.keys), reinterpret_cast<K*>(F.keys_s), F.vals, F.vals_s, (size_t)total, 0u, (unsigned)(3 * P0.pcl_bits + 1), sa));
        prof_end(m, sa);
        prof_begin(m, TSL_K_RAYS, sa);
        hipLaunchKernelGGL(k_build_rays<K>, dim3(blocks), dim3(256), 0, sa, B.p[0], F, (const K*)reinterpret_cast<K*>(F.keys_s));
        prof_end(m, sa);
    }
    return launch_segments(m, B, hp, total, sa);
}

template <typename K>
static int launch_batch_t(tsl_tsdf* m)
{
    const int n = m->npend;
    if (n == 0) return TSL_OK;
    m->npend = 0;
    (void)hipGetLastError();
    m->last_batch_n = n;
    const int bi = m->cur;
    BatchHost& H = m->batch[bi];
    const bool serial = m->overlap == 0;
    {
        const BatchHost& L = m->batch[(bi + TSL_NBATCH - 1) % TSL_NBATCH];
        if (!L.b_pending || hipEventQuery(L.b_done) == hipSuccess) { m->ramp = 0; ++m->dry_launches; } else if (m->ramp < 1000) ++m->ramp;
        m->shape_hash = (m->shape_hash ^ (uint32_t)n) * 16777619u;
    }
    hipStream_t sa = serial ? m->stream_ : H.st;
    const int ring = (int)(m->batch_seq % TSL_INFLIGHT);
    if (m->ring_upto[ring] > 0) {
        TSL_HIP(hipEventSynchronize(m->ring_ev[ring]));
        if (m->ring_upto[ring] > m->frames_consumed) m->frames_consumed = m->ring_upto[ring];
    }
#ifdef TSL_TEST_HOOKS
    static const bool fault_no_wait = std::getenv("TSL_FAULT_NO_BDONE_WAIT") != nullptr;
#else
    constexpr bool fault_no_wait = false;
#endif
    if (!serial && H.b_pending && !fault_no_wait) TSL_HIP(hipStreamWaitEvent(sa, H.b_done, 0));
    if (!serial && m->esdf_gate_set) {
        TSL_HIP(hipStreamWaitEvent(sa, m->esdf_gate_ev, 0));
        m->esdf_gate_mask |= 1u << (bi % TSL_NSTREAMS);
        if (m->esdf_gate_mask == (1u << TSL_NSTREAMS) - 1u) m->esdf_gate_set = false;
    }
    for (int k = 0; k < m->nproducers; ++k) {
        if (m->producers[k] == sa) continue;
        if (hipStreamQuery(m->producers[k]) == hipSuccess) continue;
        if (!m->in_ev[0]) for (auto& e : m->in_ev) TSL_HIP(hipEventCreateWithFlags(&e, hipEventDisableTiming));
        hipEvent_t e = m->in_ev[m->in_ev_next]; m->in_ev_next = (m->in_ev_next + 1) % 8;
        TSL_HIP(hipEventRecord(e, m->producers[k]));
        TSL_HIP(hipStreamWaitEvent(sa, e, 0));
    }
    m->nproducers = 0;
    BatchDev B; ParamPack PP;
    for (int q = 0; q < n; ++q) { FSet& S = m->fset[bi * TSL_NB + q]; B.f[q] = S.F; B.p[q] = S.Pd; PP.p[q] = m->pend[q]; }
    for (int q = n; q < TSL_NB; ++q) { B.f[q] = B.f[0]; B.p[q] = B.p[0]; PP.p[q] = PP.p[0]; }
    B.n = n;
    SetPtrs SP;
    for (int q = 0; q < TSL_NB; ++q) { SP.p[q] = const_cast<FrameParams*>(B.p[q]); SP.header[q] = reinterpret_cast<int*>(B.f[q].stats); }
    hipLaunchKernelGGL(k_set_params, dim3(n), dim3(64), 0, sa, PP, SP);
    {
        StageCopy C; int most = 0; bool any_host = false;
        for (int q = 0; q < TSL_NB; ++q) {
            FSet& S = m->fset[bi * TSL_NB + q];
            const bool on = q < n;
            C.src[2 * q] = static_cast<const uint4*>(S.pin_dev); C.dst[2 * q] = static_cast<uint4*>(S.stage_in); C.n16[2 * q] = on ? (int)((S.copy_in + 15) / 16) : 0;
            C.src[2 * q + 1] = reinterpret_cast<const uint4*>(static_cast<const char*>(S.pin_dev) + S.copy_tex_off); C.dst[2 * q + 1] = static_cast<uint4*>(S.stage_tex); C.n16[2 * q + 1] = on ? (int)((S.copy_tex + 15) / 16) : 0;
            most = std::max(most, std::max(C.n16[2 * q], C.n16[2 * q + 1]));
            any_host = any_host || C.n16[2 * q] || C.n16[2 * q + 1];
            if (on) { S.copy_in = 0; S.copy_tex = 0; }
        }
        if (any_host) {
            prof_begin(m, TSL_K_VOXELIZE, sa);
            hipLaunchKernelGGL(k_stage_host, dim3(std::min(64, (most + 1023) / 1024), 2 * n), dim3(256), 0, sa, C);
            prof_end(m, sa);
            if (!serial) { TSL_HIP(hipEventRecord(H.c_done, sa)); H.c_recorded = true; }
        }
    }
    if (m->phases & 1) { int rc = enqueue_phase_a<K>(m, B, m->pend, sa); if (rc) return rc; }
    const bool seq_bricks = m->pend[0].seq && m->seq_impl && m->pend[0].variant == 2;
    if (seq_bricks && (m->phases & 1)) { int rc = launch_seq_group(m, B, m->pend, bi, sa); if (rc) return rc; }
    m->frames_issued += n;
    if (!serial) {
        TSL_HIP(hipEventRecord(H.a_done, sa)); H.a_recorded = true;
        TSL_HIP(hipStreamWaitEvent(m->stream_, H.a_done, 0));
    }
    bool any = false; for (int q = 0; q < n; ++q) any = any || m->pend[q].total > 0;
    const bool split = !serial && m->split_launch && (m->phases & 2) && m->pend[0].variant == 2 && !m->pend[0].seq && n > 2 && any;
    if (split) {
        hipEvent_t pa = nullptr, pb = nullptr;
        const bool timed = prof_slot(m, TSL_K_INTEGRATE, 0, &pa, &pb);
        int rc = launch_brick(m, B, m->pend[0], 2, sa, timed ? pa : nullptr, timed ? pb : nullptr);
        if (rc) return rc;
        TSL_HIP(hipEventRecord(H.p_done, sa));
    }
    if (m->phases & 2) {
        int rc = TSL_OK;
        if (m->pend[0].variant == 2) {
            if (any) {
                hipEvent_t ea = nullptr, eb = nullptr;
                const bool timed = !m->pend[0].seq && prof_slot(m, TSL_K_INTEGRATE, 1, &ea, &eb);
                if (seq_bricks) { prof_begin(m, TSL_K_INTEGRATE); rc = launch_seq_apply(m, B, m->pend[0], bi); prof_end(m); }
                else if (m->pend[0].seq) { prof_begin(m, TSL_K_INTEGRATE); rc = launch_apply_sequential(m, B, m->pend[0]); prof_end(m); }
                else if (split) {
                    rc = launch_brick(m, B, m->pend[0], 1, m->stream_, timed ? ea : nullptr, timed ? eb : nullptr);
                    TSL_HIP(hipStreamWaitEvent(m->stream_, H.p_done, 0));
                    if (!rc) rc = launch_slab_apply(m, B, m->pend[0]);
                }
                else rc = launch_apply_batch(m, B, m->pend[0], timed ? ea : nullptr, timed ? eb : nullptr);
            }
        } else {
            for (int q = 0; q < n && !rc; ++q) {
                FSet& S = m->fset[bi * TSL_NB + q];
                m->P = m->pend[q];
                if (m->P.total > 0) rc = launch_apply(m, S, m->P.total);
            }
        }
        if (rc) return rc;
    }
    TSL_HIP(hipEventRecord(m->ring_ev[ring], m->stream_)); m->ring_upto[ring] = m->frames_issued; m->batch_seq++;
    if (!serial) { H.b_done = m->ring_ev[ring]; H.b_pending = true; }
    m->cur = (bi + 1) % TSL_NBATCH;
    TSL_HIP(hipGetLastError());
    return TSL_OK;
}
int flush_pending(tsl_tsdf* m)
{
    if (m->npend == 0) return TSL_OK;
    const FrameParams keep = m->P;
    const int rc = m->pcl_bits <= 10 ? launch_batch_t<uint32_t>(m) : launch_batch_t<uint64_t>(m);
    m->P = keep;
    if (rc && !m->deferred_rc) m->deferred_rc = rc;
    return rc;
}
hipStream_t ms(tsl_tsdf* m) { if (m->clean) (void)hipGetLastError(); m->clean = false; (void)flush_pending(m); return m->stream_; }

static int batch_cap(const tsl_tsdf* m)
{ return (m->overlap > 0 && m->variant == 2 && m->P.group && (!m->semantics || m->seq_impl)) ? (m->overlap < TSL_NB ? m->overlap : TSL_NB) : 1; }
static int reserve_slot(tsl_tsdf* m, int points, int* set_index)
{
    const int slot = map_slot(m, m->active);
    if (m->npend && (m->npend >= batch_cap(m) || m->pend_points != points || m->pend[0].slot != slot)) { int rc = flush_pending(m); if (rc) return rc; }
    *set_index = m->cur * TSL_NB + m->npend;
    return TSL_OK;
}
template <int PICK>
static void pick_pixels(uint16_t* __restrict__ dst, const uint16_t* __restrict__ src, int n, int pick)
{
    if (PICK) { for (int i = 0; i < n; ++i) dst[i] = src[(size_t)i * PICK]; }
    else for (int i = 0; i < n; ++i) dst[i] = src[(size_t)i * pick];
}
static int stage_host(tsl_tsdf* m, int si, const void* in, size_t row_bytes, int rows, size_t src_pitch, const void* tex, size_t tex_bytes, void** in_dev, void** tex_dev,
                      int pick = 1)
{
    const int npick = pick > 1 ? (int)(row_bytes / sizeof(uint16_t)) / pick : 0;
    const size_t out_row = pick > 1 ? (size_t)npick * sizeof(uint16_t) : row_bytes;
    const size_t in_bytes = out_row * (size_t)rows;
    FSet& S = m->fset[si];
    BatchHost& H = m->batch[si / TSL_NB];
    if (m->overlap == 0) TSL_HIP(hipStreamSynchronize(m->stream_));
    else if (H.c_recorded) TSL_HIP(hipEventSynchronize(H.c_done));
    const size_t tex_off = (in_bytes + 255) & ~(size_t)255;
    const size_t need = tex_off + ((tex && tex_bytes) ? tex_bytes : 0) + 256;
    if (S.pin_bytes < need) {
        if (S.pin) (void)hipHostFree(S.pin);
        S.pin = nullptr; S.pin_bytes = 0; S.pin_dev = nullptr;
#ifdef TSL_TEST_HOOKS
        static const bool legacy = std::getenv("TSL_PIN_LEGACY") != nullptr;
#else
        constexpr bool legacy = false;
#endif
        TSL_HIP(hipHostMalloc(&S.pin, need + need / 4, legacy ? hipHostMallocMapped : (hipHostMallocMapped | hipHostMallocCoherent)));
        S.pin_bytes = need + need / 4;
        TSL_HIP(hipHostGetDevicePointer(&S.pin_dev, S.pin, 0));
    }
    char* pin = static_cast<char*>(S.pin);
    if (in_bytes && pick > 1) {
        for (int r = 0; r < rows; ++r) {
            uint16_t* d = reinterpret_cast<uint16_t*>(pin + (size_t)r * out_row);
            const uint16_t* sp = reinterpret_cast<const uint16_t*>(static_cast<const char*>(in) + (size_t)r * src_pitch);
            if (pick == 2) pick_pixels<2>(d, sp, npick, 2); else if (pick == 4) pick_pixels<4>(d, sp, npick, 4); else pick_pixels<0>(d, sp, npick, pick);
        }
    } else if (in_bytes) {
        if (rows > 1 && src_pitch != row_bytes) { for (int r = 0; r < rows; ++r) std::memcpy(pin + (size_t)r * row_bytes, static_cast<const char*>(in) + (size_t)r * src_pitch, row_bytes); }
        else std::memcpy(pin, in, in_bytes);
    }
    const size_t in16 = (in_bytes + 15) & ~(size_t)15, tex16 = ((tex && tex_bytes) ? tex_bytes + 15 : 0) & ~(size_t)15;
    if (S.stage_in_bytes < in16 || S.stage_tex_bytes < tex16) {
        if (m->overlap != 0 && H.a_recorded) TSL_HIP(hipEventSynchronize(H.a_done));
        int rc = grow(&S.stage_in, &S.stage_in_bytes, in16); if (rc) return rc;
        if (tex16) { rc = grow(&S.stage_tex, &S.stage_tex_bytes, tex16); if (rc) return rc; }
    }
    *in_dev = S.stage_in; *tex_dev = nullptr;
    S.copy_in = in_bytes; S.copy_tex = 0; S.copy_tex_off = tex_off;
    if (tex && tex_bytes) { std::memcpy(pin + tex_off, tex, tex_bytes); *tex_dev = S.stage_tex; S.copy_tex = tex_bytes; }
    return TSL_OK;
}

static int ensure_frame_scratch(tsl_tsdf* m)
{
    if (m->scratch_ready) return TSL_OK;
    const tsl_tsdf_cfg* cfg = &m->cfg;
    FrameDev& F = m->F;
    int rc;
    const size_t np = (size_t)F.max_points;
    if ((rc = dev_alloc(m, (void**)&F.slot_tab, sizeof(int) * (size_t)m->nb3, 0xff))) return rc;
    if ((rc = dev_alloc(m, (void**)&F.touched, sizeof(int) * (size_t)F.max_frame_bricks, 0))) return rc;
    if ((rc = dev_alloc(m, (void**)&F.touched_b, sizeof(int) * (size_t)F.max_frame_bricks, 0))) return rc;
    if ((rc = dev_alloc(m, (void**)&F.acc, 16 * (size_t)F.max_frame_bricks * TSL_BRK3, 0))) return rc;
    if ((rc = dev_alloc(m, (void**)&F.dbg, sizeof(long long) * 16384 * 16, 0))) return rc;
    if (cfg->texture_enabled) { if ((rc = dev_alloc(m, (void**)&F.accw, 4 * (size_t)F.max_frame_bricks * TSL_BRK3, 0))) return rc; }
    for (int si = 0; si < TSL_NSETS; ++si) {
        FSet& S = m->fset[si];
        S.F = F;
        FrameDev& G = S.F;
        auto own = [&](void** p, size_t bytes) -> int { int r = dev_alloc(m, p, bytes, 0); if (!r) S.owned.push_back(*p); return r; };
        if (si >= TSL_NB) {
            FrameDev& G0 = m->fset[(si / TSL_NB) * TSL_NB].F;
            if (si % TSL_NB == 0) {
                if ((rc = own((void**)&G.acc, 16 * (size_t)F.max_frame_bricks * TSL_BRK3))) return rc;
                if (cfg->texture_enabled) { if ((rc = own((void**)&G.accw, 4 * (size_t)F.max_frame_bricks * TSL_BRK3))) return rc; }
            } else { G.acc = G0.acc; G.accw = G0.accw; }
        }
        if ((rc = own((void**)&G.keys, 8 * np))) return rc;
        if ((rc = own((void**)&G.keys_s, 8 * np))) return rc;
        if ((rc = own((void**)&G.vals, 4 * np))) return rc;
        if ((rc = own((void**)&G.vals_s, 4 * np))) return rc;
        if ((rc = own((void**)&G.pix, 8 * np))) return rc;
        if ((rc = own((void**)&G.rayA, 16 * np))) return rc;
        if ((rc = own((void**)&G.rayN, 4 * np))) return rc;
        if ((rc = own((void**)&G.rayFirst, 4 * np))) return rc;
        {
            int lg = 10; while ((1ll << lg) < 2 * (long long)np) ++lg;
            G.hlog2 = lg;
            void* tab = nullptr;
            if ((rc = dev_alloc(m, &tab, sizeof(HSlot) << lg, 0))) return rc;
            S.owned.push_back(tab); G.htab = static_cast<HSlot*>(tab);
            if ((rc = own((void**)&G.act, 4 * np))) return rc;
            if ((rc = own((void**)&G.actx, 4 * np))) return rc;
        }
        if (cfg->texture_enabled) { if ((rc = own((void**)&G.colpix, 8 * np))) return rc; }
        S.header_bytes = 256;
        if ((rc = own(&S.header, S.header_bytes))) return rc;
        G.stats = reinterpret_cast<tsl_frame_stats*>(S.header);
        G.nrays = reinterpret_cast<int*>((char*)S.header + 80);
        G.counters = reinterpret_cast<int*>((char*)S.header + 96);
        if ((rc = own((void**)&G.seg, 8 * (size_t)F.seg_cap))) return rc;
        if ((rc = own((void**)&G.seg_sorted, 8 * (size_t)F.seg_cap))) return rc;
        if ((rc = own((void**)&G.bhist, sizeof(int) * (size_t)m->nb3))) return rc;
        if ((rc = own((void**)&G.bcursor, sizeof(int) * (size_t)m->nb3))) return rc;
        if ((rc = own((void**)&G.boffset, sizeof(int) * (size_t)m->nb3))) return rc;
        if ((rc = own((void**)&G.bnseg, sizeof(int) * (size_t)m->nb3))) return rc;
        if ((rc = own((void**)&G.bslab, sizeof(int) * (size_t)m->nb3))) return rc;
        if ((rc = own((void**)&G.act_b, sizeof(int) * (size_t)(F.max_frame_bricks + 8)))) return rc;
        G.part_cap = F.seg_cap / 256 + F.max_frame_bricks + 8;
        if ((rc = own((void**)&G.part_tab, sizeof(int4) * 4 * (size_t)G.part_cap))) return rc;
        G.unit_cap = TSL_NB * F.max_frame_bricks;
        if (si % TSL_NB == 0) {
            if ((rc = own((void**)&G.unit_tab, sizeof(int4) * 4 * (size_t)G.unit_cap))) return rc;
            if ((rc = own((void**)&G.heavy_tab, sizeof(int4) * (size_t)(F.max_frame_bricks + 8)))) return rc;
        }
        if ((rc = own(&S.sort_temp, m->sort_temp_bytes + 256))) return rc;
        if ((rc = own((void**)&S.Pd, sizeof(FrameParams)))) return rc;
    }
    TSL_HIP(hipStreamSynchronize(m->stream_));
    for (int bi = 0; bi < TSL_NSTREAMS; ++bi) {
        TSL_HIP(hipMemsetAsync(m->fset[bi * TSL_NB].header, 0, 4, m->batch[bi].st));
        TSL_HIP(hipEventRecord(m->batch[bi].a_done, m->batch[bi].st));
    }
    TSL_HIP(hipMemsetAsync(m->fset[0].header, 0, 4, m->copy_st));
    for (int bi = 0; bi < TSL_NSTREAMS; ++bi) TSL_HIP(hipStreamSynchronize(m->batch[bi].st));
    TSL_HIP(hipStreamSynchronize(m->copy_st));
    for (int k = 0; k < TSL_INFLIGHT; ++k) TSL_HIP(hipEventRecord(m->ring_ev[k], m->stream_));
    TSL_HIP(hipStreamSynchronize(m->stream_));
    m->scratch_ready = true;
    return TSL_OK;
}

static int queue_frame(tsl_tsdf* m, const void* depth_dev, const void* xyz_dev, int64_t npts)
{
    FrameParams& P = m->P;
    const int total = xyz_dev ? (int)npts : P.hh * P.ww;
    TSL_REQUIRE(total <= m->F.max_points, "integrate: more pixels/points than max_points");
    { int rc = ensure_frame_scratch(m); if (rc) return rc; }
    if (P.variant == 2) { int rc = check_variant2(m); if (rc) return rc; }
    P.input = xyz_dev ? xyz_dev : depth_dev; P.total = total; P.points = xyz_dev ? 1 : 0;
    {
        int lg = 10; while ((1ll << lg) < 2 * (long long)total) ++lg;
        P.hlog2 = lg < m->fset[0].F.hlog2 ? lg : m->fset[0].F.hlog2;
    }
    TSL_REQUIRE(!P.tex || P.variant == 2, "texture integration needs the brick-binned path (variant 2)");
    const int cap = batch_cap(m);
    { int si = 0; int rc = reserve_slot(m, P.points, &si); if (rc) return rc; }
    m->clean = false;
    m->pend_points = P.points;
    m->pend[m->npend] = P;
    m->pend[m->npend].group = (P.group && P.variant == 2) ? 1 : 0;
    m->last_set = m->cur * TSL_NB + m->npend;
    m->npend++;
    if (m->npend >= cap || (cap > 4 && m->ramp < m->ramp_batches && m->npend >= m->ramp_size)) return flush_pending(m);
    if (cap > 1 && m->adaptive) {
        const int last = (m->cur + TSL_NBATCH - 1) % TSL_NBATCH;
        const BatchHost& H = m->batch[last];
        if (!H.a_recorded || hipEventQuery(H.a_done) == hipSuccess) return flush_pending(m);
    }
    return TSL_OK;
}

static int sort_temp_size(tsl_tsdf* m, size_t* bytes)
{
    size_t a = 0, b = 0;
    TSL_HIP(rocprim::radix_sort_pairs(nullptr, a, (uint32_t*)nullptr, (uint32_t*)nullptr, (uint32_t*)nullptr, (uint32_t*)nullptr,
                                      (size_t)m->F.max_points, 0u, 32u, m->stream_));
    TSL_HIP(rocprim::radix_sort_pairs(nullptr, b, (uint64_t*)nullptr, (uint64_t*)nullptr, (uint32_t*)nullptr, (uint32_t*)nullptr,
                                      (size_t)m->F.max_points, 0u, 64u, m->stream_));
    *bytes = a > b ? a : b;
    return TSL_OK;
}

static void fill_frame_params(tsl_tsdf* m, const double R[9], const double T[3])
{
    const int s = m->active;
    convert_pose(&m->baseR[(size_t)s * 9], &m->baseT[(size_t)s * 3], R, T, m->P.R, m->P.T);
    m->P.slot = map_slot(m, s);
    m->P.variant = m->variant; m->P.split = (m->variant == 2 && m->split > 8) ? 8 : m->split;
}

}

using namespace tsl;

extern "C" {

const char* tsl_version(void) { return "taichislam_hip 0.1 (gfx950)"; }
const char* tsl_last_error(void) { return g_err.c_str(); }
int tsl_selftest(int which, int64_t* mismatches)
{
    TSL_REQUIRE(mismatches && which >= 0 && which <= 2, "tsl_selftest: bad argument");
    unsigned long long* bad = nullptr;
    TSL_HIP(hipMalloc((void**)&bad, sizeof(unsigned long long)));
    TSL_HIP(hipMemset(bad, 0, sizeof(unsigned long long)));
    if (which == 2) (void)selftest_seqdiv(bad);
    else hipLaunchKernelGGL(k_selftest, dim3(8192), dim3(256), 0, 0, which, bad);
    unsigned long long h = ~0ull;
    hipError_t e = hipMemcpy(&h, bad, sizeof(h), hipMemcpyDeviceToHost);
    (void)hipFree(bad);
    TSL_HIP(e);
    *mismatches = (int64_t)h;
    return TSL_OK;
}
int tsl_device_count(int* n)
{
    int c = 0;
    hipError_t e = hipGetDeviceCount(&c);
    if (e != hipSuccess) { c = 0; }
    if (n) *n = c;
    return TSL_OK;
}

static int init_handle(tsl_tsdf* m, const tsl_tsdf_cfg* cfg, int device)
{
    m->cfg = *cfg; m->device = device; m->bytes = 0;
    (void)hipGetLastError();
    TSL_HIP(hipStreamCreateWithFlags(&m->stream_, hipStreamNonBlocking));
    m->overlap = TSL_NB; m->last_set = 0;
    for (auto& S : m->fset) { S.sort_temp = nullptr; S.header = nullptr; S.Pd = nullptr; S.stage_in = nullptr; S.stage_in_bytes = 0; S.stage_tex = nullptr; S.stage_tex_bytes = 0; S.pin = nullptr; S.pin_bytes = 0; S.pin_dev = nullptr; S.copy_in = S.copy_tex = S.copy_tex_off = 0; }
    for (auto& H : m->batch) { H.st = nullptr; H.a_done = nullptr; H.b_done = nullptr; H.p_done = nullptr; H.c_done = nullptr; H.b_pending = false; H.a_recorded = false; H.c_recorded = false; }
    m->frames_issued = 0; m->frames_consumed = 0; m->batch_seq = 0;
    for (int k = 0; k < TSL_INFLIGHT; ++k) { m->ring_ev[k] = nullptr; m->ring_upto[k] = 0; }
    m->cur = 0; m->npend = 0; m->pend_points = 0; m->deferred_rc = 0;
    const int blk = cfg->num_voxel_per_blk_axis;
    m->N = (int)std::ceil(cfg->map_size_xy / cfg->voxel_scale / (double)blk) * blk;
    m->Nz = (int)std::ceil(cfg->map_size_z / cfg->voxel_scale / (double)blk) * blk;
    TSL_REQUIRE(m->N > 0 && m->Nz > 0 && m->N <= 32768 && m->Nz <= 32768, "tsl_tsdf_create: map extent must fit int16 voxel indices");
    m->nbx = (m->N + 15) / 16; m->nbz = (m->Nz + 15) / 16; m->nb3 = m->nbx * m->nbx * m->nbz;
    m->nsub = cfg->is_global_map ? 1 : (cfg->max_submap_num > 0 ? cfg->max_submap_num : 1);
    m->npose = cfg->max_submap_num > m->nsub ? cfg->max_submap_num : m->nsub;
    {
        int grp = (int)(3.2 * cfg->max_ray_length / (double)blk / cfg->voxel_scale);
        if (grp < 1) grp = 1;
        const int ext = blk * grp;
        int off = -ext / 2; if ((-ext) % 2 != 0) off -= 1;
        m->pcl_lo = off; m->pcl_ext = ext;
        int bits = 1; while ((1 << bits) < ext) ++bits;
        m->pcl_bits = bits;
        TSL_REQUIRE(bits <= 20, "tsl_tsdf_create: sensor grid too large");
    }
    FrameParams& P = m->P; std::memset(&P, 0, sizeof(P));
    for (int i = 0; i < 3; ++i) P.R[i * 4] = 1.0f;
    P.vs = (float)cfg->voxel_scale;
    {
        const float y0 = (float)(1.0 / (double)P.vs);
        float best = y0; double err = std::fabs(1.0 - (double)y0 * (double)P.vs);
        const float cand[2] = { std::nextafterf(y0, 0.0f), std::nextafterf(y0, INFINITY) };
        for (float c : cand) { const double e = std::fabs(1.0 - (double)c * (double)P.vs); if (e < err) { err = e; best = c; } }
        P.rvs = best; P.fastdiv = 0;
    }
    P.thr_max = (float)(cfg->max_ray_length * 1000.0); P.thr_min = (float)(cfg->min_ray_length * 1000.0);
    P.max_ray_f = (float)cfg->max_ray_length;
    P.max_steps_f = (float)(cfg->max_ray_length / cfg->voxel_scale);
    P.internal_f = (float)cfg->internal_voxels;
    P.pcl_lo = m->pcl_lo; P.pcl_ext = m->pcl_ext; P.pcl_bits = m->pcl_bits; P.pcl_blk = blk; P.seq = 0;
    P.step = cfg->recast_step; P.same_proj = cfg->color_same_proj;
    m->surf_thres = (float)(cfg->voxel_scale * 1.8);
    m->disp_floor = (float)cfg->disp_floor; m->disp_ceiling = (float)cfg->disp_ceiling;
    m->baseR.assign((size_t)m->npose * 9, 0.0); m->baseT.assign((size_t)m->npose * 3, 0.0);
    m->baseRf.assign((size_t)m->npose * 9, 0.0f); m->baseTf.assign((size_t)m->npose * 3, 0.0f);
    for (int s = 0; s < m->npose; ++s) for (int i = 0; i < 3; ++i) { m->baseR[(size_t)s * 9 + i * 4] = 1.0; m->baseRf[(size_t)s * 9 + i * 4] = 1.0f; }
    std::memset(m->gbaseR, 0, sizeof(m->gbaseR)); std::memset(m->gbaseT, 0, sizeof(m->gbaseT));
    for (int i = 0; i < 3; ++i) m->gbaseR[i * 4] = 1.0;
    m->P.group = 1; m->phases = 3; m->wg = 512; m->spt = 2; m->adaptive = 0; m->ramp_batches = 2; m->ramp_size = 4; m->bgrid = 75; m->ugrid = 75; m->pgrid = 25; m->split_launch = 0; m->chunks = 4; m->unit_max = 1024 * TSL_NB; m->unit_half = 1 << 20; m->unit_floor = 4096; m->batch_gen = 0;
    { hipDeviceProp_t pr; TSL_HIP(hipGetDeviceProperties(&pr, device)); m->ncu = pr.multiProcessorCount > 0 ? pr.multiProcessorCount : 256; }
    m->active = 0; m->variant = 2; m->split = 2; m->semantics = 0; m->seq_impl = 1; m->seq_ready = false; m->seq_bytes0 = 0; m->seq_d = nullptr; m->seq_tuple_cap = 0;
    m->prof_on = false; m->prof_open = false; m->prof_group = false; m->prof_mask = ~0u; std::memset(m->prof_ms, 0, sizeof(m->prof_ms)); std::memset(m->prof_n, 0, sizeof(m->prof_n));
    m->sort_temp = nullptr; m->sort_temp_bytes = 0;
    m->xbuf = nullptr; m->xbuf_bytes = 0; m->mesh_v = m->mesh_n = m->mesh_c = nullptr; m->mesh_count = nullptr; m->mesh_cap = 0; m->mesh_flags = nullptr;
    m->fuse_acc = nullptr; m->fuse_cnt = nullptr; m->fuse_cacc = nullptr; m->fuse_dirty = false; m->mrg_nunion = -1;
    m->esdf = nullptr; m->esdf_par = nullptr; m->esdf_ok = nullptr; m->esdf_mode = 0; m->esdf_grid = 0; m->fuse_direct = false; m->merge_exchange = 0; m->mrg_racc = m->mrg_rcnt = m->mrg_rec = nullptr; m->mrg_racc_bytes = m->mrg_rcnt_bytes = m->mrg_rec_bytes = 0; m->esdf_orphans = 0; m->esdf_last = nullptr; m->esdf_in = nullptr; m->esdf_read = nullptr; m->esdf_overlap = true; m->esdf_ctr_idx = 0; for (int k = 0; k < 2; ++k) { m->fseq_keys[k] = m->fseq_vals[k] = nullptr; m->fseq_bytes[k] = m->fseq_vbytes[k] = 0; } m->fseq_temp = nullptr; m->fseq_tbytes = 0; m->fseq_ctr = nullptr; m->esdf_gate = nullptr; m->esdf_gate_ev = nullptr; m->esdf_gate_set = false; m->esdf_gate_mask = 0; m->esdf_valid = false; m->esdf_force_full = false; m->pose_dev = nullptr;

    MapDev& M = m->M; std::memset(&M, 0, sizeof(M));
    M.N = m->N; M.Nz = m->Nz; M.nbx = m->nbx; M.nbz = m->nbz; M.nb3 = m->nb3; M.nsub = m->nsub; M.hN = m->N / 2; M.hNz = m->Nz / 2;
    int64_t want = cfg->max_bricks > 0 ? cfg->max_bricks : 32768 * (int64_t)(m->nsub > 4 ? 4 : (m->nsub > 1 ? m->nsub : 1));
    const int64_t all = (int64_t)m->nsub * m->nb3;
    if (want > all) want = all;
    M.max_bricks = (int)want;
    int rc;
    if ((rc = dev_alloc(m, (void**)&M.table, sizeof(int) * (size_t)all, 0xff))) return rc;
    if ((rc = dev_alloc(m, (void**)&M.tw, sizeof(uint32_t) * (size_t)want * TSL_BRK3, 0))) return rc;
    if ((rc = dev_alloc(m, (void**)&M.obs, (size_t)want * TSL_BRK3, 0))) return rc;
    if ((rc = dev_alloc(m, (void**)&M.occ, (size_t)want * TSL_BRK3, 0))) return rc;
    if (cfg->texture_enabled) { if ((rc = dev_alloc(m, (void**)&M.col, sizeof(uint16_t) * 4 * (size_t)want * TSL_BRK3, 0))) return rc; }
    if ((rc = dev_alloc(m, (void**)&M.owner, sizeof(int) * (size_t)want, 0))) return rc;
    if ((rc = dev_alloc(m, (void**)&M.touch, (size_t)want, 0))) return rc;
    if ((rc = dev_alloc(m, (void**)&M.pool_top, sizeof(int) * 4, 0))) return rc;
    M.err = M.pool_top + 1;

    FrameDev& F = m->F; std::memset(&F, 0, sizeof(F));
    F.max_points = cfg->max_points > 0 ? cfg->max_points : 640 * 480;
    F.max_frame_bricks = cfg->max_frame_bricks > 0 ? cfg->max_frame_bricks : 4096;
    if (F.max_frame_bricks > M.max_bricks) F.max_frame_bricks = M.max_bricks;
    {
        const int64_t cap = (int64_t)F.max_points * 32;
        F.seg_cap = (int)(cap > (1ll << 30) ? (1ll << 30) : cap);
    }
    if ((rc = sort_temp_size(m, &m->sort_temp_bytes))) return rc;
#ifdef TSL_TEST_HOOKS
    static const bool ev_sys = std::getenv("TSL_EV_SYS") != nullptr;
#else
    constexpr bool ev_sys = false;
#endif
    const unsigned evf = hipEventDisableTiming | (ev_sys ? 0u : (unsigned)hipEventDisableSystemFence);
    for (int bi = 0; bi < TSL_NBATCH; ++bi) {
        BatchHost& H = m->batch[bi];
        if (bi < TSL_NSTREAMS) TSL_HIP(hipStreamCreateWithFlags(&H.st, hipStreamNonBlocking)); else H.st = m->batch[bi % TSL_NSTREAMS].st;
        TSL_HIP(hipEventCreateWithFlags(&H.a_done, evf));
        TSL_HIP(hipEventCreateWithFlags(&H.p_done, evf));
        TSL_HIP(hipEventCreateWithFlags(&H.c_done, evf));
    }
    for (int k = 0; k < TSL_INFLIGHT; ++k) TSL_HIP(hipEventCreateWithFlags(&m->ring_ev[k], evf));
    TSL_HIP(hipStreamCreateWithFlags(&m->copy_st, hipStreamNonBlocking));
    TSL_HIP(hipHostMalloc((void**)&m->h_stats, sizeof(tsl_frame_stats), hipHostMallocDefault));
    TSL_HIP(hipHostMalloc((void**)&m->h_ints, sizeof(long long) * 256, hipHostMallocDefault));
    std::memset(m->h_stats, 0, sizeof(tsl_frame_stats));

    m->max_disp = cfg->max_disp_particles > 0 ? cfg->max_disp_particles : 1024 * 1024;
    if ((rc = dev_alloc(m, (void**)&m->exp_xyz, sizeof(float) * 3 * (size_t)m->max_disp, 0))) return rc;
    if ((rc = dev_alloc(m, (void**)&m->exp_rgb, sizeof(float) * 3 * (size_t)m->max_disp, 0))) return rc;
    if ((rc = dev_alloc(m, (void**)&m->exp_val, sizeof(float) * (size_t)m->max_disp, 0))) return rc;
    if ((rc = dev_alloc(m, (void**)&m->num_particles, sizeof(int) * 4, 0))) return rc;
    if ((rc = dev_alloc(m, (void**)&m->colormap, sizeof(float) * 3 * 1024, 0))) return rc;
    if ((rc = dev_alloc(m, (void**)&m->pose_dev, sizeof(float) * 12 * (size_t)m->npose, 0))) return rc;
    {
        unsigned long long* bad = reinterpret_cast<unsigned long long*>(m->num_particles + 2);
        TSL_HIP(hipMemsetAsync(bad, 0, sizeof(unsigned long long), m->stream_));
        hipLaunchKernelGGL(k_verify_div, dim3(8192), dim3(256), 0, m->stream_, P.vs, P.rvs, bad);
        unsigned long long nbad = 1;
        TSL_HIP(hipMemcpyAsync(&nbad, bad, sizeof(nbad), hipMemcpyDeviceToHost, m->stream_));
        TSL_HIP(hipStreamSynchronize(m->stream_));
        TSL_HIP(hipMemsetAsync(bad, 0, sizeof(unsigned long long), m->stream_));
        P.fastdiv = nbad == 0 ? 1 : 0;
    }
    TSL_HIP(hipStreamSynchronize(m->stream_));
    return TSL_OK;
}

int tsl_tsdf_create(const tsl_tsdf_cfg* cfg, int device, tsl_tsdf** out)
{
    TSL_REQUIRE(cfg && out, "tsl_tsdf_create: null argument");
    TSL_REQUIRE(cfg->voxel_scale > 0 && cfg->num_voxel_per_blk_axis >= 1 && cfg->recast_step >= 1, "tsl_tsdf_create: bad config");
    int ndev = 0;
    if (hipGetDeviceCount(&ndev) != hipSuccess || ndev <= 0) { set_error("no HIP device available"); return TSL_ERR_NO_DEVICE; }
    TSL_REQUIRE(device >= 0 && device < ndev, "tsl_tsdf_create: bad device index");
    TSL_HIP(hipSetDevice(device));
    tsl_tsdf* m = new tsl_tsdf();
    const int rc = init_handle(m, cfg, device);
    if (rc) { const std::string keep = g_err; tsl_tsdf_destroy(m); g_err = keep; return rc; }
    *out = m;
    return TSL_OK;
}

void tsl_tsdf_destroy(tsl_tsdf* m)
{
    if (!m) return;
    (void)hipSetDevice(m->device);
    if (m->stream_) (void)hipStreamSynchronize(m->stream_);
    for (auto& H : m->batch) if (H.st) (void)hipStreamSynchronize(H.st);
    if (m->stream_) (void)hipStreamSynchronize(m->stream_);
    (void)hipDeviceSynchronize();
    for (int bi = 0; bi < TSL_NBATCH; ++bi) {
        BatchHost& H = m->batch[bi];
        if (H.st && bi < TSL_NSTREAMS) (void)hipStreamDestroy(H.st);
        if (H.a_done) (void)hipEventDestroy(H.a_done);
        if (H.p_done) (void)hipEventDestroy(H.p_done);
        if (H.c_done) (void)hipEventDestroy(H.c_done);
    }
    for (auto& S : m->fset) {

        for (void* p : S.owned) if (p) (void)hipFree(p);
        if (S.stage_in) (void)hipFree(S.stage_in);
        if (S.stage_tex) (void)hipFree(S.stage_tex);
        if (S.pin) (void)hipHostFree(S.pin);

    }
    esdf_release(m);
    seq_release(m);
    void* ptrs[] = { m->M.table, m->M.tw, m->M.obs, m->M.occ, m->M.col, m->M.owner, m->M.pool_top, m->F.slot_tab, m->F.touched, m->F.touched_b, m->F.acc, m->F.accw, m->F.dbg,
                     m->exp_xyz, m->exp_rgb, m->exp_val, m->num_particles, m->colormap, m->pose_dev, m->xbuf,
                     m->mesh_v, m->mesh_n, m->mesh_c, m->mesh_count, m->mesh_flags, m->esdf, m->esdf_fl, m->esdf_region, m->esdf_list, m->esdf_queue, m->esdf_ctr, m->esdf_inq, m->esdf_nbr, m->esdf_par, m->esdf_ok, m->esdf_note, m->fseq_keys[0], m->fseq_keys[1], m->fseq_vals[0], m->fseq_vals[1], m->fseq_temp, m->fseq_ctr, m->esdf_exp_xyz, m->esdf_exp_val, m->esdf_exp_count, m->M.touch, m->fuse_acc, m->fuse_cnt, m->fuse_cacc, m->seq_keys[0], m->seq_keys[1], m->seq_vals[0], m->seq_vals[1], m->seq_ctr, m->seq_temp,
                     m->mrg_mask, m->mrg_list, m->mrg_pacc, m->mrg_pcnt, m->mrg_racc, m->mrg_rcnt, m->mrg_rec };
    for (void* p : ptrs) if (p) (void)hipFree(p);
    if (m->h_stats) (void)hipHostFree(m->h_stats);
    if (m->h_ints) (void)hipHostFree(m->h_ints);
    for (auto& s : m->prof) { (void)hipEventDestroy(s.a); (void)hipEventDestroy(s.b); }
    for (auto& e : m->prof_free) (void)hipEventDestroy(e);
    for (auto& e : m->in_ev) if (e) (void)hipEventDestroy(e);
    for (auto& e : m->ring_ev) if (e) (void)hipEventDestroy(e);
    if (m->copy_st) (void)hipStreamDestroy(m->copy_st);
    if (m->stream_) (void)hipStreamDestroy(m->stream_);
    delete m;
}

int tsl_tsdf_get_dims(const tsl_tsdf* m, int32_t* N, int32_t* Nz, int32_t* bxy, int32_t* bz)
{
    TSL_REQUIRE(m, "null handle");
    const int blk = m->cfg.num_voxel_per_blk_axis;
    if (N) *N = m->N; if (Nz) *Nz = m->Nz;
    if (bxy) *bxy = m->N / blk; if (bz) *bz = m->Nz / blk;
    return TSL_OK;
}
static int take_dev_err(tsl_tsdf* m)
{
    TSL_HIP(hipMemcpyAsync(&m->h_ints[28], m->M.err, sizeof(int), hipMemcpyDeviceToHost, m->stream_));
    TSL_HIP(hipStreamSynchronize(m->stream_));
    const int e = m->h_ints[28];
    if (!e) return TSL_OK;
    set_error(std::string("device capacity exhausted:") + ((e & 1) ? " brick pool (max_bricks)" : "") + ((e & 2) ? " frame scratch (max_frame_bricks)" : "") +
              ((e & 4) ? " ray segments / ray-step tuples of the sequential semantics (seq_tuple_cap)" : "") + ((e & 8) ? " more than 16384 points in one sensor voxel" : "") + "; the affected frames / bricks were not integrated");
    TSL_HIP(hipMemsetAsync(m->M.err, 0, sizeof(int), m->stream_));
    return TSL_ERR_CAPACITY;
}
int tsl_tsdf_sync(tsl_tsdf* m)
{
    TSL_REQUIRE(m, "null handle");
    if (m->clean && m->npend == 0 && !m->deferred_rc) return TSL_OK;
    TSL_HIP(hipSetDevice(m->device));
    int rc = flush_pending(m);
    for (auto& H : m->batch) if (H.st) TSL_HIP(hipStreamSynchronize(H.st));
    if (m->copy_st) TSL_HIP(hipStreamSynchronize(m->copy_st));
    const int ec = take_dev_err(m);
    m->frames_consumed = m->frames_issued;
    if (!rc && m->deferred_rc) { rc = m->deferred_rc; }
    m->deferred_rc = 0;
    m->clean = true;
    return rc ? rc : ec;
}
int tsl_tsdf_memory_bytes(const tsl_tsdf* m, int64_t* b) { TSL_REQUIRE(m && b, "null"); *b = m->bytes; return TSL_OK; }

static int take_deferred(tsl_tsdf* m) { const int rc = m->deferred_rc; m->deferred_rc = 0; return rc; }
static int read_int(tsl_tsdf* m, const int* dev, int* out)
{
    TSL_HIP(hipMemcpyAsync(m->h_ints, dev, sizeof(int), hipMemcpyDeviceToHost, ms(m)));
    TSL_HIP(hipStreamSynchronize(ms(m)));
    *out = m->h_ints[0];
    return take_deferred(m);
}
static int check_dev_err(tsl_tsdf* m) { (void)ms(m); return take_dev_err(m); }
int tsl_tsdf_get_option(tsl_tsdf* m, const char* name, int* value)
{
    TSL_REQUIRE(m && name && value, "null");
    if (!std::strcmp(name, "group")) { *value = m->P.group; return TSL_OK; }
    if (!std::strcmp(name, "esdf_mode")) { *value = m->esdf_mode; return TSL_OK; }
    if (!std::strcmp(name, "fuse_window_misses")) { return read_int(m, m->M.pool_top + 2, value); }
    if (!std::strcmp(name, "esdf_orphans")) { int rc = esdf_finish(m); if (rc) return rc; *value = (int)m->esdf_orphans; return TSL_OK; }
    if (!std::strcmp(name, "semantics")) { *value = m->semantics; return TSL_OK; }
    if (!std::strcmp(name, "seq_impl")) { *value = m->seq_impl; return TSL_OK; }
    if (!std::strcmp(name, "last_heavy_bricks") || !std::strcmp(name, "last_slab_slots")) {
        TSL_REQUIRE(m->scratch_ready, "nothing integrated yet");
        int rc = tsl_tsdf_sync(m); if (rc) return rc;
        const int bi = (m->cur + TSL_NBATCH - 1) % TSL_NBATCH;
        int v[40];
        TSL_HIP(hipMemcpy(v, m->fset[bi * TSL_NB].F.counters, sizeof(v), hipMemcpyDeviceToHost));
        *value = name[5] == 'h' ? v[14] : v[13];
        return TSL_OK;
    }
    if (!std::strcmp(name, "seq_longest_run")) {
        TSL_REQUIRE(m->scratch_ready, "nothing integrated yet");
        int rc = tsl_tsdf_sync(m); if (rc) return rc;
        const int bi = (m->cur + TSL_NBATCH - 1) % TSL_NBATCH;
        long long sum = 0;
        for (int q = 0; q < m->last_batch_n; ++q) { int v[40]; TSL_HIP(hipMemcpy(v, m->fset[bi * TSL_NB + q].F.counters, sizeof(v), hipMemcpyDeviceToHost)); sum += (unsigned)v[31]; }
        *value = (int)(sum > 0x7fffffffll ? 0x7fffffffll : sum);
        return TSL_OK;
    }
    if (!std::strcmp(name, "seq_long_voxels")) {
        TSL_REQUIRE(m->scratch_ready, "nothing integrated yet");
        int rc = tsl_tsdf_sync(m); if (rc) return rc;
        const int bi = (m->cur + TSL_NBATCH - 1) % TSL_NBATCH;
        int v[40]; TSL_HIP(hipMemcpy(v, m->fset[bi * TSL_NB].F.counters, sizeof(v), hipMemcpyDeviceToHost));
        *value = v[28] + v[30];
#ifdef TSL_SEQ_DBG
        fprintf(stderr, "seq dbg (long role, last batch): evaluations %d, commits that moved T %d, commits that moved W only %d\n", v[32], v[33], v[34]);
#endif
        return TSL_OK;
    }
    if (!std::strcmp(name, "fastdiv")) { *value = m->P.fastdiv; return TSL_OK; }
    if (!std::strcmp(name, "seq_verify_mismatches")) {
        int rc = tsl_tsdf_sync(m); if (rc) return rc;
        std::vector<int> buf(4 + 4 * 64);
        rc = seq_verify_report(m, buf.data(), (int)buf.size()); if (rc) return rc;
        *value = buf[0];
        for (int e = 0; e < buf[0] && e < 64; ++e)
            fprintf(stderr, "seq_verify: batch %d frame %d stage %d slot %d what %d T %d  (stage 3: voxel %d expected %d found %d)\n", buf[4 + 4 * e], buf[5 + 4 * e] & 255, buf[5 + 4 * e] >> 8, buf[6 + 4 * e], buf[7 + 4 * e] & 15, buf[7 + 4 * e] >> 4,
                    buf[7 + 4 * e] & 4095, (buf[7 + 4 * e] >> 12) & 1023, (buf[7 + 4 * e] >> 22) & 1023);
        return TSL_OK;
    }
    if (!std::strcmp(name, "batch_shape_hash")) { *value = (int)(m->shape_hash & 0x7fffffffu); return TSL_OK; }
    if (!std::strcmp(name, "dry_launches")) { *value = m->dry_launches; return TSL_OK; }
    if (!std::strcmp(name, "overlapped_launches")) { *value = (int)m->batch_seq - m->dry_launches; return TSL_OK; }
    if (!std::strcmp(name, "variant")) { *value = m->variant; return TSL_OK; }
    if (!std::strcmp(name, "split")) { *value = m->split; return TSL_OK; }
    set_error("unknown option"); return TSL_ERR_ARG;
}
int tsl_tsdf_bricks_in_use(tsl_tsdf* m, int32_t* n)
{
    TSL_REQUIRE(m && n, "null"); TSL_HIP(hipSetDevice(m->device));
    int v = 0; int rc = read_int(m, m->M.pool_top, &v); if (rc) return rc;
    *n = v > m->M.max_bricks ? m->M.max_bricks : v;
    return TSL_OK;
}

int tsl_tsdf_reset(tsl_tsdf* m)
{
    TSL_REQUIRE(m, "null handle"); TSL_HIP(hipSetDevice(m->device));
    const int pending = tsl_tsdf_sync(m);
    if (pending && pending != TSL_ERR_CAPACITY) return pending;
    int used = 0; int rc = tsl_tsdf_bricks_in_use(m, &used); if (rc) return rc;
    m->esdf_valid = false; m->esdf_query_ok = false;
    if (used > 0) hipLaunchKernelGGL(k_reset_bricks, dim3(used < 4096 ? used : 4096), dim3(256), 0, ms(m), m->M, used);
    TSL_HIP(hipMemsetAsync(m->M.pool_top, 0, sizeof(int), ms(m)));
    TSL_HIP(hipGetLastError());
    return pending;
}

int tsl_tsdf_set_intrinsics(tsl_tsdf* m, const double Kd[9], const double Kc[9])
{
    TSL_REQUIRE(m, "null handle");
    if (Kd) { m->P.fx = (float)Kd[0]; m->P.fy = (float)Kd[4]; m->P.cx = (float)Kd[2]; m->P.cy = (float)Kd[5]; }
    if (Kc) { m->P.fxc = (float)Kc[0]; m->P.fyc = (float)Kc[4]; m->P.cxc = (float)Kc[2]; m->P.cyc = (float)Kc[5]; }
    return TSL_OK;
}
int tsl_tsdf_set_base_pose(tsl_tsdf* m, const double R[9], const double T[3])
{ TSL_REQUIRE(m && R && T, "null"); std::memcpy(m->gbaseR, R, 72); std::memcpy(m->gbaseT, T, 24); return TSL_OK; }
int tsl_tsdf_set_base_pose_submap(tsl_tsdf* m, int sid, const double R[9], const double T[3])
{
    TSL_REQUIRE(m && R && T, "null"); TSL_REQUIRE(sid >= 0 && sid < m->npose, "set_base_pose_submap: submap id out of range");
    std::memcpy(&m->baseR[(size_t)sid * 9], R, 72); std::memcpy(&m->baseT[(size_t)sid * 3], T, 24);
    for (int a = 0; a < 9; ++a) m->baseRf[(size_t)sid * 9 + a] = (float)R[a];
    for (int a = 0; a < 3; ++a) m->baseTf[(size_t)sid * 3 + a] = (float)T[a];
    return TSL_OK;
}
int tsl_tsdf_get_active_submap(const tsl_tsdf* m, int32_t* sid) { TSL_REQUIRE(m && sid, "null"); *sid = m->active; return TSL_OK; }
int tsl_tsdf_set_active_submap(tsl_tsdf* m, int32_t sid)
{ TSL_REQUIRE(m, "null"); TSL_REQUIRE(sid >= 0 && sid < m->npose, "set_active_submap: id out of range"); m->active = sid; return TSL_OK; }
int tsl_tsdf_set_colormap(tsl_tsdf* m, const float* rgb)
{
    TSL_REQUIRE(m && rgb, "null"); TSL_HIP(hipSetDevice(m->device));
    TSL_HIP(hipMemcpyAsync(m->colormap, rgb, sizeof(float) * 3 * 1024, hipMemcpyHostToDevice, ms(m)));
    TSL_HIP(hipStreamSynchronize(ms(m)));
    return TSL_OK;
}

static int integrate_depth_dev_impl(tsl_tsdf* m, const double R[9], const double T[3], const void* depth_dev, int h, int w,
                                    const void* tex_dev, int th, int tw, bool packed)
{
    TSL_REQUIRE(m && R && T && depth_dev, "integrate_depth: null argument");
    TSL_REQUIRE(h > 0 && w > 0, "integrate_depth: bad image size");
    TSL_REQUIRE(!(m->cfg.texture_enabled && tex_dev) || true, "");
    TSL_REQUIRE(m->active < m->nsub || m->cfg.is_global_map, "integrate: active submap beyond max_submap_num");
    TSL_HIP(hipSetDevice(m->device));
    fill_frame_params(m, R, T);
    FrameParams& P = m->P;
    P.H = h; P.W = w;
    P.hh = (int)((float)h / (float)P.step); P.ww = (int)((float)w / (float)P.step);
    P.rstride = packed ? w / P.step : P.step * w;
    P.cstride = packed ? 1 : P.step;
    P.th = th; P.tw = tw; P.tex = (m->cfg.texture_enabled && tex_dev) ? 1 : 0; P.tex_input = (const uint8_t*)tex_dev;
    TSL_REQUIRE(!P.tex || (th > 0 && tw > 0 && (!P.same_proj || (th >= h && tw >= w))), "integrate_depth: texture smaller than the depth image");
    m->h_stats->p_used = (int64_t)P.hh * P.ww;
    return queue_frame(m, depth_dev, nullptr, 0);
}
int tsl_tsdf_integrate_depth_dev(tsl_tsdf* m, const double R[9], const double T[3], const void* depth_dev, int h, int w,
                                 const void* tex_dev, int th, int tw)
{ return integrate_depth_dev_impl(m, R, T, depth_dev, h, w, tex_dev, th, tw, false); }

int tsl_tsdf_integrate_depth(tsl_tsdf* m, const double R[9], const double T[3], const uint16_t* depth, int h, int w,
                             const uint8_t* tex, int th, int tw)
{
    TSL_REQUIRE(m && depth, "integrate_depth: null argument"); TSL_REQUIRE(h > 0 && w > 0, "integrate_depth: bad image size");
    TSL_HIP(hipSetDevice(m->device));
    int si = 0; int rc = reserve_slot(m, 0, &si); if (rc) return rc;
    const bool use_tex = tex && m->cfg.texture_enabled && th > 0 && tw > 0;
    void *ddev = nullptr, *tdev = nullptr;
    const int step = m->P.step, hh = (int)((float)h / (float)step);
    rc = stage_host(m, si, depth, (size_t)w * sizeof(uint16_t), step > 1 ? hh : h, (size_t)(step > 1 ? step : 1) * w * sizeof(uint16_t),
                    use_tex ? tex : nullptr, use_tex ? (size_t)th * tw * 3 : 0, &ddev, &tdev, step); if (rc) return rc;
    return integrate_depth_dev_impl(m, R, T, ddev, h, w, tdev, th, tw, step > 1);
}

int tsl_tsdf_integrate_points_dev(tsl_tsdf* m, const double R[9], const double T[3], const void* xyz_dev, const void* rgb_dev, int64_t n)
{
    TSL_REQUIRE(m && R && T, "integrate_points: null argument"); TSL_REQUIRE(n >= 0 && (n == 0 || xyz_dev), "integrate_points: bad input");
    TSL_HIP(hipSetDevice(m->device));
    fill_frame_params(m, R, T);
    m->P.tex = (m->cfg.texture_enabled && rgb_dev) ? 1 : 0; m->P.tex_input = (const uint8_t*)rgb_dev;
    m->h_stats->p_used = n;
    return queue_frame(m, nullptr, xyz_dev, n);
}

int tsl_tsdf_integrate_points(tsl_tsdf* m, const double R[9], const double T[3], const float* xyz, const uint8_t* rgb, int64_t n)
{
    TSL_REQUIRE(m, "null handle"); TSL_REQUIRE(n >= 0 && (n == 0 || xyz), "integrate_points: bad input");
    TSL_HIP(hipSetDevice(m->device));
    int si = 0; int rc = reserve_slot(m, 1, &si); if (rc) return rc;
    const bool use_tex = rgb && m->cfg.texture_enabled && n;
    void *xdev = nullptr, *cdev = nullptr;
    rc = stage_host(m, si, xyz, (size_t)n * 3 * sizeof(float), 1, 0, use_tex ? rgb : nullptr, use_tex ? (size_t)n * 3 : 0, &xdev, &cdev); if (rc) return rc;
    return tsl_tsdf_integrate_points_dev(m, R, T, xdev, cdev, n);
}

int tsl_tsdf_input_stream(tsl_tsdf* m, int points, int ordered, void* producer, void** hip_stream)
{
    TSL_REQUIRE(m, "input_stream: null argument"); TSL_HIP(hipSetDevice(m->device));
    int si = 0; int rc = reserve_slot(m, points ? 1 : 0, &si); if (rc) return rc;
    hipStream_t consumer = m->overlap == 0 ? m->stream_ : m->batch[si / TSL_NB].st;
    if (hip_stream) *hip_stream = (void*)consumer;
    if (ordered && (hipStream_t)producer != consumer) {
        bool seen = false;
        for (int k = 0; k < m->nproducers; ++k) seen = seen || m->producers[k] == (hipStream_t)producer;
        if (!seen) {
            if (m->nproducers == 4) { rc = flush_pending(m); if (rc) return rc; }
            m->producers[m->nproducers++] = (hipStream_t)producer;
        }
    }
    return TSL_OK;
}

int tsl_tsdf_integrate_depth_stream(tsl_tsdf* m, const double R[9], const double T[3], const void* depth_dev, int h, int w,
                                    const void* tex_dev, int th, int tw, void* producer, int64_t* queued_total, int64_t* consumed)
{
    int rc = tsl_tsdf_input_stream(m, 0, 1, producer, nullptr); if (rc) return rc;
    rc = tsl_tsdf_integrate_depth_dev(m, R, T, depth_dev, h, w, tex_dev, th, tw); if (rc) return rc;
    return tsl_tsdf_frames_consumed(m, queued_total, consumed);
}

int tsl_tsdf_queued_frames(const tsl_tsdf* m, int32_t* n) { TSL_REQUIRE(m && n, "null"); *n = m->npend; return TSL_OK; }

int tsl_tsdf_frames_consumed(tsl_tsdf* m, int64_t* queued_total, int64_t* consumed)
{
    TSL_REQUIRE(m, "null");
    if (queued_total) *queued_total = m->frames_issued + m->npend;
    if (consumed) *consumed = m->frames_consumed;
    return TSL_OK;
}

int tsl_tsdf_last_frame_stats(tsl_tsdf* m, tsl_frame_stats* out)
{
    TSL_REQUIRE(m && out, "null"); TSL_HIP(hipSetDevice(m->device));
    const int64_t used = m->h_stats->p_used;
    tsl_frame_stats tmp;
    if (!m->scratch_ready) { std::memset(out, 0, sizeof(*out)); return TSL_OK; }
    { int rc2 = tsl_tsdf_sync(m); if (rc2) return rc2; }
    TSL_HIP(hipMemcpyAsync(m->h_ints, m->fset[m->last_set].F.stats, sizeof(tsl_frame_stats), hipMemcpyDeviceToHost, ms(m)));
    TSL_HIP(hipStreamSynchronize(ms(m)));
    std::memcpy(&tmp, m->h_ints, sizeof(tmp));
    tmp.p_used = used;
    *out = tmp;
    return TSL_OK;
}

int tsl_tsdf_count_active(tsl_tsdf* m, int64_t* n)
{
    TSL_REQUIRE(m && n, "null"); TSL_HIP(hipSetDevice(m->device));
    long long* tmp = reinterpret_cast<long long*>(m->num_particles + 2);
    TSL_HIP(hipMemsetAsync(tmp, 0, sizeof(long long), ms(m)));
    hipLaunchKernelGGL(k_count_active, dim3(m->nb3 < 4096 ? m->nb3 : 4096), dim3(256), 0, ms(m), m->M, map_slot(m, m->active), tmp);
    long long v = 0;
    TSL_HIP(hipMemcpyAsync(&v, tmp, sizeof(long long), hipMemcpyDeviceToHost, ms(m)));
    TSL_HIP(hipStreamSynchronize(ms(m)));
    *n = v;
    return take_deferred(m);
}

static int export_common(tsl_tsdf* m, int mode, int16_t* idx, uint16_t* t, uint16_t* w, int8_t* occ, uint16_t* col, int64_t cap, int64_t* n)
{
    TSL_REQUIRE(m && n, "null"); TSL_REQUIRE(cap >= 0, "bad capacity"); TSL_HIP(hipSetDevice(m->device));
    const size_t c = (size_t)cap;
    const size_t o_idx = 0, o_t = o_idx + c * 6, o_w = o_t + c * 2, o_occ = o_w + c * 2, o_col = ((o_occ + c + 15) / 16) * 16, total = o_col + c * 6 + 64;
    int rc = grow(&m->xbuf, &m->xbuf_bytes, total); if (rc) return rc;
    char* base = (char*)m->xbuf;
    int* counter = m->num_particles + 2;
    TSL_HIP(hipMemsetAsync(counter, 0, sizeof(int), ms(m)));
    hipLaunchKernelGGL(k_export_sparse, dim3(m->nb3 < 4096 ? m->nb3 : 4096), dim3(256), 0, ms(m), m->M, map_slot(m, m->active), mode,
                       (int16_t*)(base + o_idx), (uint16_t*)(base + o_t), (uint16_t*)(base + o_w), (int8_t*)(base + o_occ),
                       (col && m->M.col) ? (uint16_t*)(base + o_col) : (uint16_t*)nullptr, (long long)cap, counter);
    int cnt = 0; rc = read_int(m, counter, &cnt); if (rc) return rc;
    *n = cnt;
    const size_t k = (size_t)(cnt < cap ? cnt : cap);
    if (k) {
        if (idx) TSL_HIP(hipMemcpy(idx, base + o_idx, k * 6, hipMemcpyDeviceToHost));
        if (t) TSL_HIP(hipMemcpy(t, base + o_t, k * 2, hipMemcpyDeviceToHost));
        if (w) TSL_HIP(hipMemcpy(w, base + o_w, k * 2, hipMemcpyDeviceToHost));
        if (occ) TSL_HIP(hipMemcpy(occ, base + o_occ, k, hipMemcpyDeviceToHost));
        if (col && m->M.col) TSL_HIP(hipMemcpy(col, base + o_col, k * 6, hipMemcpyDeviceToHost));
    }
    return TSL_OK;
}
int tsl_tsdf_export_sparse(tsl_tsdf* m, int16_t* idx, uint16_t* t, uint16_t* w, int8_t* occ, uint16_t* col, int64_t cap, int64_t* n)
{ return export_common(m, 0, idx, t, w, occ, col, cap, n); }
int tsl_tsdf_export_occupied(tsl_tsdf* m, int16_t* idx, int8_t* occ, int64_t cap, int64_t* n)
{ return export_common(m, 1, idx, nullptr, nullptr, occ, nullptr, cap, n); }

int tsl_tsdf_import_sparse(tsl_tsdf* m, int sid, const int16_t* idx, const uint16_t* t, const uint16_t* w, const int8_t* occ, const uint16_t* col, int64_t n)
{
    TSL_REQUIRE(m, "null handle"); TSL_REQUIRE(n >= 0, "bad count"); if (n == 0) return TSL_OK;
    TSL_REQUIRE(idx && t && w, "import_sparse: null arrays");
    TSL_REQUIRE(sid >= 0 && (m->cfg.is_global_map || sid < m->nsub), "import_sparse: submap id out of range");
    TSL_HIP(hipSetDevice(m->device));
    m->esdf_valid = false; m->esdf_query_ok = false;
    const size_t c = (size_t)n;
    const size_t o_idx = 0, o_t = o_idx + c * 6, o_w = o_t + c * 2, o_occ = o_w + c * 2, o_col = ((o_occ + c + 15) / 16) * 16, total = o_col + c * 6 + 64;
    int rc = grow(&m->xbuf, &m->xbuf_bytes, total); if (rc) return rc;
    char* base = (char*)m->xbuf;
    TSL_HIP(hipMemcpy(base + o_idx, idx, c * 6, hipMemcpyHostToDevice));
    TSL_HIP(hipMemcpy(base + o_t, t, c * 2, hipMemcpyHostToDevice));
    TSL_HIP(hipMemcpy(base + o_w, w, c * 2, hipMemcpyHostToDevice));
    if (occ) TSL_HIP(hipMemcpy(base + o_occ, occ, c, hipMemcpyHostToDevice));
    const bool hc = col && m->M.col;
    if (hc) TSL_HIP(hipMemcpy(base + o_col, col, c * 6, hipMemcpyHostToDevice));
    hipLaunchKernelGGL(k_import_sparse, dim3((unsigned)((n + 255) / 256)), dim3(256), 0, ms(m), m->M, map_slot(m, sid),
                       (const int16_t*)(base + o_idx), (const uint16_t*)(base + o_t), (const uint16_t*)(base + o_w),
                       occ ? (const int8_t*)(base + o_occ) : (const int8_t*)nullptr, hc ? (const uint16_t*)(base + o_col) : (const uint16_t*)nullptr, (long long)n);
    TSL_HIP(hipStreamSynchronize(ms(m)));
    return check_dev_err(m);
}

static int export_particles(tsl_tsdf* m, tsl_tsdf* dst, int mode, int keep, int slice_index, float dz, int32_t* n)
{
    TSL_REQUIRE(m, "null handle"); TSL_HIP(hipSetDevice(m->device));
    if (!dst) dst = m;
    TSL_REQUIRE(dst->device == m->device, "export: destination map lives on another device");
    if (!keep) TSL_HIP(hipMemsetAsync(dst->num_particles, 0, sizeof(int), ms(m)));
    const PoseF B = pose_of(m, m->active);
    hipLaunchKernelGGL(k_export_particles, dim3(m->nb3 < 4096 ? m->nb3 : 4096), dim3(256), 0, ms(m), m->M, map_slot(m, m->active), mode, B,
                       m->cfg.is_global_map, m->P.vs, m->surf_thres, m->disp_floor, m->disp_ceiling, slice_index, dz, m->colormap,
                       dst->exp_xyz, dst->exp_rgb, dst->exp_val, (long long)dst->max_disp, dst->num_particles);
    int cnt = 0; int rc = read_int(m, dst->num_particles, &cnt); if (rc) return rc;
    if (n) *n = cnt;
    return TSL_OK;
}
int tsl_tsdf_surface_voxels(tsl_tsdf* m, tsl_tsdf* dst, int add_to_cur, int32_t* n) { return export_particles(m, dst, 0, add_to_cur, 0, 0.0f, n); }
int tsl_tsdf_slice_voxels(tsl_tsdf* m, float z, float dz, int clear_last, int32_t* n)
{
    TSL_REQUIRE(m, "null handle");
    _Float16 zh = (_Float16)z; const float zq = (float)zh;
    return export_particles(m, nullptr, 1, !clear_last, (int)(zq / m->P.vs), dz, n);
}
int tsl_tsdf_read_exports(tsl_tsdf* m, float* xyz, float* rgb, float* val, int64_t n)
{
    TSL_REQUIRE(m, "null handle"); TSL_REQUIRE(n >= 0 && n <= m->max_disp, "read_exports: n out of range"); TSL_HIP(hipSetDevice(m->device));
    TSL_HIP(hipStreamSynchronize(ms(m)));
    if (n == 0) return TSL_OK;
    if (xyz) TSL_HIP(hipMemcpy(xyz, m->exp_xyz, sizeof(float) * 3 * (size_t)n, hipMemcpyDeviceToHost));
    if (rgb) TSL_HIP(hipMemcpy(rgb, m->exp_rgb, sizeof(float) * 3 * (size_t)n, hipMemcpyDeviceToHost));
    if (val) TSL_HIP(hipMemcpy(val, m->exp_val, sizeof(float) * (size_t)n, hipMemcpyDeviceToHost));
    return TSL_OK;
}
int tsl_tsdf_exports_dev(tsl_tsdf* m, void** xyz_dev, void** rgb_dev, void** val_dev, int32_t* n)
{
    TSL_REQUIRE(m, "null handle"); TSL_HIP(hipSetDevice(m->device));
    if (xyz_dev) *xyz_dev = m->exp_xyz; if (rgb_dev) *rgb_dev = m->exp_rgb; if (val_dev) *val_dev = m->exp_val;
    int v = 0; const int rc = read_int(m, m->num_particles, &v); if (rc) return rc;
    if (n) *n = v;
    return TSL_OK;
}
int tsl_tsdf_set_export_row(tsl_tsdf* m, int field, int64_t row, const float v[3])
{
    TSL_REQUIRE(m && v && (field == 0 || field == 1), "set_export_row: bad argument"); TSL_REQUIRE(row >= 0 && row < m->max_disp, "set_export_row: row out of range");
    TSL_HIP(hipSetDevice(m->device));
    TSL_HIP(hipMemcpyAsync((field ? m->exp_rgb : m->exp_xyz) + 3 * row, v, sizeof(float) * 3, hipMemcpyHostToDevice, ms(m)));
    TSL_HIP(hipStreamSynchronize(ms(m)));
    return TSL_OK;
}

int tsl_tsdf_pack_pointcloud2(tsl_tsdf* m, int has_rgb, int64_t n, void* out_host)
{
    TSL_REQUIRE(m && (n == 0 || out_host), "pack_pointcloud2: null argument"); TSL_REQUIRE(n >= 0 && n <= m->max_disp, "pack_pointcloud2: n out of range");
    TSL_HIP(hipSetDevice(m->device));
    if (n == 0) return TSL_OK;
    const int stride = has_rgb ? 6 : 3;
    int rc = grow(&m->xbuf, &m->xbuf_bytes, sizeof(float) * (size_t)stride * (size_t)n); if (rc) return rc;
    hipLaunchKernelGGL(k_pack_pointcloud2, dim3((unsigned)(((long long)n * stride + 255) / 256)), dim3(256), 0, ms(m), m->exp_xyz, m->exp_rgb, (float*)m->xbuf, (long long)n, stride);
    TSL_HIP(hipMemcpyAsync(out_host, m->xbuf, sizeof(float) * (size_t)stride * (size_t)n, hipMemcpyDeviceToHost, ms(m)));
    TSL_HIP(hipStreamSynchronize(ms(m)));
    return TSL_OK;
}

int tsl_tsdf_num_particles(tsl_tsdf* m, int32_t* n) { TSL_REQUIRE(m && n, "null"); TSL_HIP(hipSetDevice(m->device)); int v = 0; int rc = read_int(m, m->num_particles, &v); *n = v; return rc; }
int tsl_tsdf_set_num_particles(tsl_tsdf* m, int32_t n)
{
    TSL_REQUIRE(m, "null"); TSL_HIP(hipSetDevice(m->device));
    m->h_ints[8] = n;
    TSL_HIP(hipMemcpyAsync(m->num_particles, &m->h_ints[8], sizeof(int), hipMemcpyHostToDevice, ms(m)));
    TSL_HIP(hipStreamSynchronize(ms(m)));
    return TSL_OK;
}

int tsl_tsdf_prof_enable(tsl_tsdf* m, int on)
{
    TSL_REQUIRE(m, "null");
    m->prof_on = on != 0;
    m->prof_mask = (on == 0 || on == 1) ? ~0u : (unsigned)on >> 1;
    if (on) {
        TSL_HIP(hipSetDevice(m->device));
        while (m->prof_free.size() < 256) { hipEvent_t e; TSL_HIP(hipEventCreate(&e)); m->prof_free.push_back(e); }
    }
    return TSL_OK;
}
int tsl_tsdf_prof_query(tsl_tsdf* m, int kid, double* total_ms, int64_t* launches)
{
    TSL_REQUIRE(m, "null"); TSL_REQUIRE(kid >= 0 && kid < TSL_K_COUNT, "bad kernel id"); TSL_HIP(hipSetDevice(m->device));
    TSL_HIP(hipStreamSynchronize(ms(m)));
    for (auto& s : m->prof) {
        float ms = 0.0f;
        if (hipEventElapsedTime(&ms, s.a, s.b) == hipSuccess) { m->prof_ms[s.kid] += ms; m->prof_n[s.kid] += s.count; }
        m->prof_free.push_back(s.a); m->prof_free.push_back(s.b);
    }
    m->prof.clear();
    (void)hipGetLastError();
    if (total_ms) *total_ms = m->prof_ms[kid];
    if (launches) *launches = m->prof_n[kid];
    m->prof_ms[kid] = 0.0; m->prof_n[kid] = 0;
    return TSL_OK;
}

int tsl_tsdf_debug_counters(tsl_tsdf* m, int64_t* out, int reset)
{
    TSL_REQUIRE(m && out, "null"); TSL_HIP(hipSetDevice(m->device));
    int rc = tsl_tsdf_sync(m); if (rc) return rc;
    TSL_REQUIRE(m->scratch_ready, "debug_counters: nothing integrated yet");
    TSL_HIP(hipMemcpy(out, m->F.dbg, sizeof(long long) * 16384 * 16, hipMemcpyDeviceToHost));
    if (reset) TSL_HIP(hipMemset(m->F.dbg, 0, sizeof(long long) * 16384 * 16));
    return TSL_OK;
}

int tsl_tsdf_set_option(tsl_tsdf* m, const char* name, int value)
{
    TSL_REQUIRE(m && name, "null");
    if (!std::strcmp(name, "variant")) {
        TSL_REQUIRE(value >= 0 && value <= 2, "variant must be 0, 1 or 2");
        TSL_REQUIRE(value == 2 || !m->semantics, "variant: the sequential semantics run on variant 2 only (set semantics 0 first)");
        if (value != 2 && m->variant == 2 && m->scratch_ready) {
            int rc = tsl_tsdf_sync(m); if (rc) return rc;
            for (int bi = 0; bi < TSL_NBATCH; ++bi) TSL_HIP(hipMemsetAsync(m->fset[bi * TSL_NB].F.acc, 0, 16 * (size_t)m->F.max_frame_bricks * TSL_BRK3, m->stream_));
            TSL_HIP(hipStreamSynchronize(m->stream_));
        }
        m->variant = value; return TSL_OK;
    }
    if (!std::strcmp(name, "group")) { TSL_REQUIRE(value != 0 || !m->semantics, "group: the sequential semantics need the hash grouping (set semantics 0 first)"); int rc = tsl_tsdf_sync(m); if (rc) return rc; m->P.group = value != 0; return TSL_OK; }
    if (!std::strcmp(name, "semantics")) {
        TSL_REQUIRE(value == 0 || value == 1, "semantics must be 0 (batched exact sums) or 1 (sequential replay of the reference)");
        TSL_REQUIRE(value == 0 || m->M.max_bricks <= (1 << 17), "sequential semantics: maps with at most 2^17 bricks");
        TSL_REQUIRE(value == 0 || (m->variant == 2 && m->P.group), "sequential semantics needs variant 2 and the hash grouping (group 1)");
        TSL_REQUIRE(value == 0 || m->F.max_points <= (1 << 21), "sequential semantics: at most 2^21 points per frame");
        int rc = tsl_tsdf_sync(m); if (rc) return rc;
        if (value && m->seq_impl && !m->cfg.is_global_map) { TSL_HIP(hipSetDevice(m->device)); rc = seq_prepare(m); if (rc) return rc; }
        m->semantics = value; m->P.seq = value; return TSL_OK;
    }
    if (!std::strcmp(name, "seq_impl")) {
        TSL_REQUIRE(value == 0 || value == 1, "seq_impl must be 1 (per-brick replay runs) or 0 (round 3's global sorts)");
        int rc = tsl_tsdf_sync(m); if (rc) return rc;
        m->seq_impl = value; return TSL_OK;
    }
    if (!std::strcmp(name, "seq_tuple_cap")) {
        TSL_REQUIRE(value >= (1 << 16), "seq_tuple_cap: at least 2^16 ray steps per frame");
        int rc = tsl_tsdf_sync(m); if (rc) return rc;
        const long long old_cap = m->seq_tuple_cap;
        m->seq_tuple_cap = value;
        if (m->seq_ready) {
            TSL_HIP(hipSetDevice(m->device));
            seq_release(m);
            if (m->semantics && m->seq_impl && (rc = seq_prepare(m))) {
                m->seq_tuple_cap = old_cap;
                if (seq_prepare(m)) m->semantics = 0;
                return rc;
            }
        }
        return TSL_OK;
    }
    if (!std::strcmp(name, "fastdiv")) { if (value == 0) m->P.fastdiv = 0; return TSL_OK; }
    if (!std::strcmp(name, "mesh_gather")) { m->mesh_gather = value != 0; return TSL_OK; }
    if (!std::strcmp(name, "esdf_full")) { m->esdf_force_full = value != 0; return TSL_OK; }
    if (!std::strcmp(name, "esdf_mode")) { TSL_REQUIRE(value == 0 || value == 1, "esdf_mode: 0 = regional recompute (default), 1 = raise / lower wavefront with parent directions"); int rc = esdf_finish(m); if (rc) return rc; m->esdf_mode = value; m->esdf_valid = false; return TSL_OK; }
    if (!std::strcmp(name, "esdf_round_cap")) { m->esdf_round_cap = value; return TSL_OK; }
    if (!std::strcmp(name, "merge_exchange")) { TSL_REQUIRE(value == 0 || value == 1, "merge_exchange: 0 = all-reduce of the packed sums, 1 = reduce-scatter + all-gather of finalised voxels"); m->merge_exchange = value; return TSL_OK; }
    if (!std::strcmp(name, "fuse_direct")) { m->fuse_direct = value != 0; return TSL_OK; }
    if (!std::strcmp(name, "esdf_grid")) { TSL_REQUIRE(value >= 0, "esdf_grid: workgroups of a relaxation round (0 = four per CU)"); m->esdf_grid = value; return TSL_OK; }
    if (!std::strcmp(name, "esdf_overlap")) { int rc = esdf_finish(m); if (rc) return rc; m->esdf_overlap = value != 0; return TSL_OK; }
    if (!std::strcmp(name, "unit")) { TSL_REQUIRE(value >= 0 && value <= (1 << 20), "unit must be 0..2^20 segments"); int rc = tsl_tsdf_sync(m); if (rc) return rc; m->unit_max = value; return TSL_OK; }
    if (!std::strcmp(name, "unit_floor")) { TSL_REQUIRE(value >= 0 && value <= (1 << 20), "unit_floor must be 0..2^20 segments"); int rc = tsl_tsdf_sync(m); if (rc) return rc; m->unit_floor = value; return TSL_OK; }
    if (!std::strcmp(name, "unit_half")) { TSL_REQUIRE(value >= 0 && value <= (1 << 20), "unit_half must be 0..2^20 segments"); int rc = tsl_tsdf_sync(m); if (rc) return rc; m->unit_half = value; return TSL_OK; }
    if (!std::strcmp(name, "chunks")) { TSL_REQUIRE(value >= 1 && value <= 8, "chunks must be 1..8"); int rc = tsl_tsdf_sync(m); if (rc) return rc; m->chunks = value; return TSL_OK; }
    if (!std::strcmp(name, "adaptive")) { m->adaptive = value != 0; return TSL_OK; }
    if (!std::strcmp(name, "ramp_size")) { TSL_REQUIRE(value >= 1 && value <= TSL_NB, "ramp_size must be 1..8 frames"); m->ramp_size = value; return TSL_OK; }
    if (!std::strcmp(name, "ramp")) { TSL_REQUIRE(value >= 0 && value <= 16, "ramp must be 0..16 half batches"); m->ramp_batches = value; return TSL_OK; }
    if (!std::strcmp(name, "ugrid") || !std::strcmp(name, "pgrid")) { TSL_REQUIRE(value >= 5 && value <= 200, "ugrid / pgrid must be 5..200 (percent of the resident workgroup slots)"); { int rc = tsl_tsdf_sync(m); if (rc) return rc; } (name[0] == 'u' ? m->ugrid : m->pgrid) = value; return TSL_OK; }
    if (!std::strcmp(name, "split_launch")) { TSL_REQUIRE(value == 0 || value == 1, "split_launch must be 0 or 1"); { int rc = tsl_tsdf_sync(m); if (rc) return rc; } m->split_launch = value; return TSL_OK; }
    if (!std::strcmp(name, "bgrid")) { TSL_REQUIRE(value >= 10 && value <= 200, "bgrid must be 10..200 (percent of the resident workgroup slots)"); { int rc = tsl_tsdf_sync(m); if (rc) return rc; } m->bgrid = value; return TSL_OK; }
    if (!std::strcmp(name, "spt")) { TSL_REQUIRE(value == 2 || value == 4, "spt must be 2 or 4"); { int rc = tsl_tsdf_sync(m); if (rc) return rc; } m->spt = value; return TSL_OK; }
    if (!std::strcmp(name, "wg")) { TSL_REQUIRE(value == 256 || value == 512, "wg must be 256 or 512"); { int rc = tsl_tsdf_sync(m); if (rc) return rc; } m->wg = value; return TSL_OK; }
    if (!std::strcmp(name, "phases")) { int rc = tsl_tsdf_sync(m); if (rc) return rc; m->phases = value & 3; return TSL_OK; }
    if (!std::strcmp(name, "overlap")) { int rc = tsl_tsdf_sync(m); if (rc) return rc; m->overlap = value < 0 ? 0 : (value > TSL_NB ? TSL_NB : value); for (auto& H : m->batch) H.b_pending = false; return TSL_OK; }
    if (!std::strcmp(name, "split")) { TSL_REQUIRE(value >= 1 && value <= 64 && (64 % value) == 0, "split must divide 64"); m->split = value; return TSL_OK; }
    set_error("unknown option"); return TSL_ERR_ARG;
}

}
```

taichislam_amd/csrc/tsl_tsdf.hpp:

```cpp
#pragma once
#include "tsl_common.hpp"

namespace tsl {

struct FrameParams {
    float R[9], T[3];
    float fx, fy, cx, cy;
    float fxc, fyc, cxc, cyc;
    float vs;
    float rvs; int fastdiv;
    float thr_max, thr_min;
    float max_ray_f;
    float max_steps_f;
    float internal_f;
    int   pcl_lo, pcl_ext, pcl_bits;
    int   step, hh, ww, H, W;
    int   rstride;
    int   cstride;
    int   th, tw, tex, same_proj;
    int   slot;
    int   variant, split;
    int   group;
    int   seq, pcl_blk;
    int   hlog2;
    const void* input; int total;
    const uint8_t* tex_input; int points;
};

struct FrameDev {
    uint32_t *keys, *keys_s, *vals, *vals_s;
    uint2* pix;
    uint4* rayA;
    int*   rayN;
    uint32_t* rayFirst;
    struct HSlot* htab; int hlog2;
    int*   act;
    int*   actx;
    uint2* colpix;
    tsl_frame_stats* stats;
    int*   nrays;
    int*   counters;
    unsigned long long *seg, *seg_sorted;
    int   *bhist, *bcursor, *boffset, *bnseg;
    int   *bslab;
    int   *act_b;
    int4  *part_tab; int part_cap;
    int4  *unit_tab; int unit_cap;
    int4  *heavy_tab;
    int*   slot_tab;
    int*   touched;
    int*   touched_b;
    unsigned long long* acc;
    uint32_t* accw;
    long long* dbg;
    int    seg_cap;
    int    max_frame_bricks;
    int    max_points;
};

#define SEG_CNT_BITS 6
#define SEG_J_BITS   12
#define SEG_RAY_BITS 24
#define SEG_SLOT_SHIFT (SEG_CNT_BITS + SEG_J_BITS + SEG_RAY_BITS)
#define SEG_MAX_CNT 63
#define STG_RAY_BITS 22
#define STG_B_SHIFT (SEG_CNT_BITS + SEG_J_BITS + STG_RAY_BITS)
#define PART_NP_BITS 12
#define SLAB_SLOT_BITS 20
#define PLAN_NCLS 4
#define HDR_FAIL 11
#define HDR_CLAIM 12
#define HDR_SLAB 13
#define HDR_HEAVY 14
#define HDR_PARTS 16
#define HDR_UNITS 20
#define HDR_CLAIM2 24
#define HDR_SEQ_TUPLES 26
#define HDR_SEQ_LONG 28
#define HDR_SEQ_XLONG 30
#define HDR_SEQ_MAXRUN 31
#define HDR_SEQ_CLAIM 35
#define HDR_SEQ_SLOTS 29

__device__ __forceinline__ void frame_fail(const MapDev& M, const FrameDev& F, int bits) { atomicOr(&F.counters[11], bits); atomicOr(M.err, bits); }

#define H_INL 13
#define H_BLOCK_SHIFT 44
#define H_EMPTY 0ull
__device__ __forceinline__ unsigned long long h_key(unsigned long long vkey, int block) { return (vkey | ((unsigned long long)block << H_BLOCK_SHIFT)) + 1ull; }
#define GROUP_BIG_CAP 16384
struct HSlot { unsigned long long key; int cnt; uint32_t pix[H_INL]; };
static_assert(sizeof(HSlot) == 64, "one slot per 64 bytes");
__device__ __forceinline__ uint32_t h_hash64(unsigned long long key, int log2n) { return (uint32_t)((key * 0x9E3779B97F4A7C15ull) >> (64 - log2n)); }

struct PixAcc { int cnt; h16 sx, sy, sz, zs, cr, cg, cb; };

__device__ __forceinline__ void acc_colour(const FrameParams& P, const FrameDev& F, uint32_t pid, PixAcc& A)
{
    const uint8_t* rgb;
    if (P.points) rgb = P.tex_input + (size_t)pid * 3;
    else {
        const int jj = (int)pid / P.ww, ii = (int)pid - jj * P.ww;
        const int pj = jj * P.step, pi = ii * P.step;
        if (P.same_proj) rgb = P.tex_input + ((size_t)pj * P.tw + pi) * 3;
        else {
            int ci = (int)((((float)pi - P.cx) / P.fx) * P.fxc + P.cxc);
            int cj = (int)((((float)pj - P.cy) / P.fy) * P.fyc + P.cyc);
            if (ci < 0 || ci >= P.th || cj < 0 || cj >= P.tw) { ci = 0; cj = 0; }
            if (cj >= P.th || ci >= P.tw) { ci = 0; cj = 0; }
            rgb = P.tex_input + ((size_t)cj * P.tw + ci) * 3;
        }
    }
    A.cr = hadd(A.cr, f2h((float)rgb[0])); A.cg = hadd(A.cg, f2h((float)rgb[1])); A.cb = hadd(A.cb, f2h((float)rgb[2]));
}
__device__ __forceinline__ void acc_payload(const uint2 pl, PixAcc& A)
{
    A.sx = hadd(A.sx, (h16)(pl.x & 0xffffu)); A.sy = hadd(A.sy, (h16)(pl.x >> 16));
    A.sz = hadd(A.sz, (h16)(pl.y & 0xffffu)); A.zs = hadd(A.zs, (h16)(pl.y >> 16));
    ++A.cnt;
}
__device__ __forceinline__ void acc_pixel(const FrameParams& P, const FrameDev& F, uint32_t pid, PixAcc& A)
{
    if (P.tex) acc_colour(P, F, pid, A);
    acc_payload(F.pix[pid], A);
}

__device__ __forceinline__ bool finish_ray(const FrameParams& P, const FrameDev& F, const PixAcc& A, uint32_t first, uint4* rec, int* nsteps, bool write_colour = true)
{
    const h16 c = f2h((float)A.cnt);
    const h16 px = hdiv(A.sx, c), py = hdiv(A.sy, c), pz = hdiv(A.sz, c);
    const h16 len = hsqrt(hadd(hadd(hmul(px, px), hmul(py, py)), hmul(pz, pz)));
    const h16 zbar = hdiv(A.zs, c);
    const float lenf = h2f(len), zzf = h2f(hmul(zbar, zbar));
    if (!((lenf > 0.0f) && isfinite(lenf) && (zzf > 0.0f) && isfinite(zzf))) return false;
    const h16 dx = hdiv(px, len), dy = hdiv(py, len), dz = hdiv(pz, len);
    float nf = lenf / P.vs + P.internal_f;
    if (P.max_steps_f < nf) nf = P.max_steps_f;
    *nsteps = (int)nf;
    float w = 1.0f / zzf;
    if (w > TSL_W_CLAMP) w = TSL_W_CLAMP;
    rec->x = (uint32_t)px | ((uint32_t)py << 16);
    rec->y = (uint32_t)pz | ((uint32_t)dx << 16);
    rec->z = (uint32_t)dy | ((uint32_t)dz << 16);
    rec->w = __float_as_uint(w);
    if (P.tex && write_colour) {
        const h16 r16 = f2h(h2f(hdiv(A.cr, c)) / 255.0f), g16 = f2h(h2f(hdiv(A.cg, c)) / 255.0f), b16 = f2h(h2f(hdiv(A.cb, c)) / 255.0f);
        F.colpix[first] = make_uint2((uint32_t)r16 | ((uint32_t)g16 << 16), (uint32_t)b16);
    }
    return true;
}


#define SQ_CSR_STRIDE 4104
#define SQ_CSR_BASE 4097
#define SQ_CSR_UNSAFE 4098
struct SeqDev {
    unsigned long long* stash;
    float2* tup;
    uint32_t* csr;
    int4* items; int slot_cap;
    uint32_t* stash_ray;
    uint32_t* tup_ray;
    long long cap;
};

struct ProfSlot { hipEvent_t a, b; int kid; int count; };

#define TSL_NB 8
#define TSL_NBATCH 3
#define TSL_NSTREAMS 3
#define TSL_NSETS (TSL_NB * TSL_NBATCH)
struct FSet {
    FrameDev F; void* sort_temp; void* header; size_t header_bytes;
    void* stage_in; size_t stage_in_bytes; void* stage_tex; size_t stage_tex_bytes;
    void* pin; size_t pin_bytes; void* pin_dev;
    size_t copy_in, copy_tex, copy_tex_off;
    FrameParams* Pd;
    std::vector<void*> owned;
};
struct BatchDev { FrameDev f[TSL_NB]; const FrameParams* p[TSL_NB]; int n; };
struct ParamPack { FrameParams p[TSL_NB]; };
struct SetPtrs { FrameParams* p[TSL_NB]; int* header[TSL_NB]; };
struct BatchHost { hipStream_t st; hipEvent_t a_done, b_done, p_done, c_done; bool b_pending, a_recorded, c_recorded; };
struct StageCopy { const uint4* src[2 * TSL_NB]; uint4* dst[2 * TSL_NB]; int n16[2 * TSL_NB]; };
#define TSL_INFLIGHT 8

int fuse_submaps_sequential(tsl_tsdf* g, tsl_tsdf* sub, const float* pose_dev, int nsrc);
int esdf_finish(tsl_tsdf* m);
void esdf_release(tsl_tsdf* m);
}

#define TSL_ESDF_SLOTS 4
struct EsdfSlot { hipEvent_t ev; int* host; int rounds; tsl_esdf_stats st; };
struct tsl_tsdf {
    tsl_tsdf_cfg cfg;
    int device;
    hipStream_t stream_;
    tsl::FSet fset[TSL_NSETS]; tsl::BatchHost batch[TSL_NBATCH]; hipStream_t copy_st;
    int overlap;
    int cur, npend, pend_points; tsl::FrameParams pend[TSL_NB]; int deferred_rc;
    int64_t frames_issued, frames_consumed;
    int64_t batch_seq; hipEvent_t ring_ev[TSL_INFLIGHT]; int64_t ring_upto[TSL_INFLIGHT];
    int last_set, last_batch_n;
    hipStream_t producers[4]; int nproducers;
    hipEvent_t in_ev[8]; int in_ev_next;
    bool scratch_ready;
    int N, Nz, nbx, nbz, nb3, nsub, npose;
    int pcl_lo, pcl_ext, pcl_bits;
    tsl::MapDev M;
    tsl::FrameDev F;
    tsl::FrameParams P;
    std::vector<double> baseR, baseT;
    std::vector<float> baseRf, baseTf;
    double gbaseR[9], gbaseT[3];
    int active;
    float surf_thres, disp_floor, disp_ceiling;
    void* sort_temp; size_t sort_temp_bytes;
    tsl_frame_stats* h_stats;
    int* h_ints;
    float *exp_xyz, *exp_rgb, *exp_val; int* num_particles; int64_t max_disp;
    float* colormap;
    float* pose_dev;
    void* xbuf; size_t xbuf_bytes;
    uint32_t* mesh_flags;
    float *mesh_v, *mesh_n, *mesh_c; int* mesh_count; int64_t mesh_cap; int mesh_gather;
    void *fuse_acc, *fuse_cnt, *fuse_cacc; bool fuse_dirty;
    uint8_t* mrg_mask; int *mrg_list, *mrg_count; int mrg_nunion;
    void *mrg_pacc, *mrg_pcnt; size_t mrg_pacc_bytes, mrg_pcnt_bytes;
    void *mrg_racc, *mrg_rcnt, *mrg_rec; size_t mrg_racc_bytes, mrg_rcnt_bytes, mrg_rec_bytes; int merge_exchange;
    float* esdf; uint8_t *esdf_fl, *esdf_region, *esdf_par, *esdf_ok; int esdf_mode, esdf_grid; bool fuse_direct; long long esdf_orphans; int *esdf_list, *esdf_queue, *esdf_ctr, *esdf_inq, *esdf_nbr; uint32_t* esdf_note; int esdf_qcap;
    float *esdf_exp_xyz, *esdf_exp_val; int* esdf_exp_count; int esdf_exp_n;
    bool esdf_valid, esdf_force_full; int esdf_submap; float esdf_gamma, esdf_maxd; tsl_esdf_stats esdf_stats;
    bool esdf_query_ok; int* esdf_q_ctr; int esdf_q_rounds;
    hipEvent_t esdf_gate, esdf_gate_ev; bool esdf_gate_set; unsigned esdf_gate_mask;
    hipEvent_t esdf_in, esdf_read, esdf_last;
    bool esdf_overlap; int esdf_ctr_idx;
    void *fseq_keys[2], *fseq_vals[2], *fseq_temp; size_t fseq_bytes[2], fseq_vbytes[2], fseq_tbytes; void* fseq_ctr;
    EsdfSlot esdf_slot[TSL_ESDF_SLOTS]; int esdf_tail, esdf_npend, esdf_rounds_seen, esdf_round_cap; bool esdf_short; tsl_esdf_totals_t esdf_tot;
    bool prof_on, prof_open, prof_group; unsigned prof_mask; std::vector<tsl::ProfSlot> prof; std::vector<hipEvent_t> prof_free;
    double prof_ms[TSL_K_COUNT]; int64_t prof_n[TSL_K_COUNT];
    int semantics;
    int seq_impl;
    bool seq_ready; int64_t seq_bytes0;
    tsl::SeqDev seq_h[TSL_NSETS]; tsl::SeqDev* seq_d;
    void *seqb_keys[TSL_NBATCH][2], *seqb_vals[TSL_NBATCH][2], *seqb_temp[TSL_NBATCH], *seqb_long[TSL_NBATCH], *seqb_lmask[TSL_NBATCH], *seqb_perm[TSL_NBATCH]; size_t seqb_temp_bytes; long long seq_tuple_cap;
    unsigned long long *seq_keys[2], *seq_vals[2], *seq_ctr; void* seq_temp; size_t seq_temp_bytes; long long seq_cap;
    int variant, split, phases, wg, spt, ncu, chunks, unit_max, unit_half, unit_floor, bgrid, ugrid, pgrid, split_launch, adaptive, ramp, ramp_batches, ramp_size; bool clean; uint64_t batch_gen;
    int64_t bytes;
    void* seqv_sum[TSL_NBATCH]; int* seqv_log;
    uint32_t shape_hash; int dry_launches;
};

namespace tsl {
int  grow(void** p, size_t* have, size_t need);
hipStream_t ms(tsl_tsdf* m);
int  flush_pending(tsl_tsdf* m);
void prof_begin(tsl_tsdf* m, int kid, hipStream_t st = nullptr, int count = 1);
void prof_end(tsl_tsdf* m, hipStream_t st = nullptr);
bool prof_slot(tsl_tsdf* m, int kid, int count, hipEvent_t* a, hipEvent_t* b);
void convert_pose(const double* Rb, const double* Tb, const double* R, const double* T, float* outR, float* outT);
int  dev_alloc(tsl_tsdf* m, void** p, size_t bytes, int fill);
int  check_variant2(tsl_tsdf* m);
int  launch_segments(tsl_tsdf* m, const BatchDev& B, const FrameParams* hp, int total, hipStream_t st);
int  launch_apply(tsl_tsdf* m, FSet& S, int total);
int  launch_apply_batch(tsl_tsdf* m, const BatchDev& B, const FrameParams& P, hipEvent_t start = nullptr, hipEvent_t stop = nullptr);
int  launch_brick(tsl_tsdf* m, const BatchDev& B, const FrameParams& P, int kind, hipStream_t st, hipEvent_t start, hipEvent_t stop);
int  launch_slab_apply(tsl_tsdf* m, const BatchDev& B, const FrameParams& P);
int  launch_seq_group(tsl_tsdf* m, const BatchDev& B, const FrameParams* hp, int bi, hipStream_t st);
int  launch_seq_apply(tsl_tsdf* m, const BatchDev& B, const FrameParams& P, int bi);
void seq_release(tsl_tsdf* m);
int  order_before(tsl_tsdf* m, hipStream_t user, hipStream_t q);
int  order_after(tsl_tsdf* m, hipStream_t user, hipStream_t q);
int  seq_prepare(tsl_tsdf* m);
int  selftest_seqdiv(unsigned long long* bad_dev);
int  seq_verify_report(tsl_tsdf* m, int* out, int cap);
int  launch_apply_sequential(tsl_tsdf* m, const BatchDev& B, const FrameParams& P);
}
```

Measured before the change: 34560 frames/s.

## Defer heavy slab apply to overlap next batch and pre-apply into unit bricks

```diff
diff --git a/taichislam_amd/csrc/tsl_integrate.hip b/taichislam_amd/csrc/tsl_integrate.hip
--- a/taichislam_amd/csrc/tsl_integrate.hip
+++ b/taichislam_amd/csrc/tsl_integrate.hip
@@ -439,7 +439,7 @@
 }
 
 __device__ __forceinline__ int plan_class(int w) { return w >= 2560 ? 0 : (w >= 1280 ? 1 : (w >= 512 ? 2 : 3)); }
-__global__ void __launch_bounds__(256) k_plan(MapDev M, BatchDev B, int psegs, int unit_max, int unit_half)
+__global__ void __launch_bounds__(256) k_plan(MapDev M, BatchDev B, int psegs, int unit_max, int unit_half, long long seq)
 {
     if ((int)blockIdx.y >= B.n) return;
     const int y = blockIdx.y;
@@ -476,13 +476,13 @@
         F.bnseg[b] = v;
         const int pool = (np || ucls >= 0) ? pool_claim<false>(M, B.p[y]->slot, b) : -1;
         if (ucls >= 0) {
-            if (u0 < B.f[0].unit_cap) B.f[0].unit_tab[(size_t)ucls * B.f[0].unit_cap + u0] = make_int4(b, wu, pool, tmu);
+            if (u0 < B.f[0].unit_cap) { B.f[0].unit_tab[(size_t)ucls * B.f[0].unit_cap + u0] = make_int4(b, wu, pool, tmu); if (pool >= 0) B.f[0].umark[b] = plan_stamp(seq); }
             else for (int q = 0; q < B.n; ++q) if ((tm >> q) & 1) frame_fail(M, B.f[q], 2);
         }
         if (np && pool >= 0) {
             if ((tmp & -tmp) == (1 << y)) {
                 const int hi = __hip_atomic_fetch_add(&B.f[0].counters[HDR_HEAVY], 1, __ATOMIC_RELAXED, __HIP_MEMORY_SCOPE_AGENT);
-                if (hi < B.f[0].max_frame_bricks) B.f[0].heavy_tab[hi] = make_int4(b, pool, tmp, 0);
+                if (hi < B.f[0].max_frame_bricks) { B.f[0].heavy_tab[hi] = make_int4(b, pool, tmp, 0); B.f[0].hmark[b] = plan_stamp(seq) | (unsigned long long)hi; }
                 else for (int q = 0; q < B.n; ++q) if ((tm >> q) & 1) frame_fail(M, B.f[q], 2);
             }
             if (s0 + np > F.max_frame_bricks || np >= (1 << PART_NP_BITS) || p0 + np > F.part_cap) frame_fail(M, F, 2);
@@ -595,13 +595,15 @@
 #define IT_FMASK 5
 #define IT_OFF  6
 #define IT_N    (IT_OFF + TSL_NB)
+#define IT_PRE  (IT_N + TSL_NB)
 #define IT_WORDS (IT_N + TSL_NB + 2)
 #define NRANGE (PLAN_NCLS * (TSL_NB + 1))
 
 template <bool TEX, bool FASTDIV, int NT, int SPT, int WPE>
-__global__ void __launch_bounds__(NT, WPE) k_integrate_batch(MapDev M, BatchDev B, int kind)
-{
-    constexpr int CSEGS = SPT * NT, VPT = TSL_BRK3 / NT, CH = VPT < FLUSH_CHUNK ? VPT : FLUSH_CHUNK;
+__global__ void __launch_bounds__(NT, WPE) k_integrate_batch(MapDev M, BatchDev B, int kind, PrevDev PV)
+{
+    static_assert(sizeof(MapDev) + sizeof(BatchDev) + sizeof(PrevDev) + 16 <= 4096, "kernel arguments");
+    constexpr int CSEGS = SPT * NT, VPT = TSL_BRK3 / NT, CH = VPT < FLUSH_CHUNK ? VPT : FLUSH_CHUNK, PCH = 2;
     static_assert(VPT <= 16, "the written / first-touch masks hold 16 voxels per thread");
 #ifdef TSL_EXP_SLOT16
     __shared__ ulonglong2 s_acc[TSL_BRK3];
@@ -620,6 +622,8 @@
     __shared__ int s_uq[TSL_NB];
     __shared__ int s_cum[NRANGE + 1];
     __shared__ int s_it[3][IT_WORDS];
+    __shared__ int s_uqp[TSL_NB];
+    __shared__ int s_npre;
     uint32_t okmask = 0u;
 #pragma unroll
     for (int q = 0; q < TSL_NB; ++q) if (q < B.n) {
@@ -628,8 +632,9 @@
         const int nact = min(Fq.counters[1], Fq.max_frame_bricks);
         for (int i = blockIdx.x * NT + threadIdx.x; i < nact; i += gridDim.x * NT) { const int b = Fq.act_b[i]; Fq.bhist[b] = 0; Fq.bcursor[b] = 0; }
     }
-    if (threadIdx.x < TSL_NB) s_uq[threadIdx.x] = 0;
+    if (threadIdx.x < TSL_NB) { s_uq[threadIdx.x] = 0; s_uqp[threadIdx.x] = 0; }
     if (threadIdx.x == 0) {
+        s_npre = 0;
         int acc = 0, k = 0;
 #ifdef TSL_CLASS_MAJOR
         for (int c = 0; c < PLAN_NCLS; ++c) {
@@ -661,29 +666,34 @@
         const FrameDev& Fq = B.f[sub - 1];
         return Fq.part_tab[(size_t)cls * Fq.part_cap + local];
     };
-    auto info_of = [&](const int4 e, int kq, int* io, int* in) {
-        *io = 0; *in = 0;
+    auto info_of = [&](const int4 e, int kq, int* io, int* in, int* ipre) {
+        *io = 0; *in = 0; *ipre = 0;
         const int q = threadIdx.x;
+        if (q == 0 && kq < 0 && PV.n && e.z >= 0) {
+            const unsigned long long w = PV.hmark[e.x];
+            if ((w >> PLAN_STAMP_SHIFT) == (PV.stamp >> PLAN_STAMP_SHIFT)) *ipre = (int)(w & ((1ull << PLAN_STAMP_SHIFT) - 1ull)) + 1;
+        }
         if (q < TSL_NB) {
             if (kq < 0) { if ((((uint32_t)e.w) & okmask) >> q & 1u) { *io = B.f[q].boffset[e.x]; *in = B.f[q].bnseg[e.x]; } }
             else if (q == kq) { *io = e.x; *in = e.y & 0xffff; }
         }
     };
-    auto commit = [&](int slot, const int4 e, int kq, int io, int in) {
+    auto commit = [&](int slot, const int4 e, int kq, int io, int in, int ipre) {
         int* it = s_it[slot];
         if (threadIdx.x < TSL_NB) { it[IT_OFF + threadIdx.x] = io; it[IT_N + threadIdx.x] = in; }
         if (threadIdx.x == 0) {
             const uint32_t tm = kq < 0 ? (uint32_t)e.w & okmask : 1u << kq;
             uint32_t fm = tm;
             int pool = e.z;
-            if (fm == 0u) { fm = 1u; pool = -1; }
-            it[IT_UNIT] = kq < 0 ? 1 : 0; it[IT_POOL] = pool; it[IT_SLAB] = kq < 0 ? 0 : e.w; it[IT_NP] = kq < 0 ? 1 : (e.y >> 16) & ((1 << PART_NP_BITS) - 1);
+            if (fm == 0u) { fm = 1u; if (!ipre) pool = -1; }
+            it[IT_PRE] = ipre;
+            it[IT_UNIT] = kq < 0 ? 1 : 0; it[IT_POOL] = pool; it[IT_SLAB] = kq < 0 ? e.x : e.w; it[IT_NP] = kq < 0 ? 1 : (e.y >> 16) & ((1 << PART_NP_BITS) - 1);
             it[IT_TMALL] = (int)tm; it[IT_FMASK] = (int)fm;
         }
     };
     const int r0 = uni(s_claim[0]);
     if (r0 >= total) return;
-    { int kq, io, in; const int4 e = entry_of(r0, &kq); info_of(e, kq, &io, &in); commit(0, e, kq, io, in); }
+    { int kq, io, in, ip; const int4 e = entry_of(r0, &kq); info_of(e, kq, &io, &in, &ip); commit(0, e, kq, io, in, ip); }
     __syncthreads();
     auto steps_of = [&](int sl, uint32_t fm) -> int {
         int n = 0;
@@ -836,19 +846,19 @@
         const long long _tb = wall_clock64();
 #endif
         bool fetching = false;
-        int4 ne = make_int4(0, 0, -1, 0); int nkq = 0, nio = 0, nin = 0;
+        int4 ne = make_int4(0, 0, -1, 0); int nkq = 0, nio = 0, nin = 0, nip = 0;
         if (do_claim) {
             const int r = uni(s_claim[0]);
             if (r < total) { fetching = true; ne = entry_of(r, &nkq); } else exhausted = true;
         }
         if (has_next) TSL_SORT_DEAL(kn, nsegn, Fx)
-        if (fetching) info_of(ne, nkq, &nio, &nin);
+        if (fetching) info_of(ne, nkq, &nio, &nin, &nip);
 #ifdef TSL_TIMING
         const long long _tc = wall_clock64();
         if (threadIdx.x == 0) { _ph[0] += _tb - _ta; _ph[1] += _tc - _tb; _ph[4] += 1; }
 #endif
         if (!last_chunk) {
-            if (fetching) { commit(n_known == 0 ? slot1 : slot2, ne, nkq, nio, nin); ++n_known; __syncthreads(); }
+            if (fetching) { commit(n_known == 0 ? slot1 : slot2, ne, nkq, nio, nin, nip); ++n_known; __syncthreads(); }
             ++c; continue;
         }
         if (p >= 0 && threadIdx.x == 0) M.touch[p] = 1;
@@ -862,6 +872,36 @@
             if (first_frame) {
 #pragma unroll
                 for (int q = 0; q < VPT; ++q) vmask |= ((old[q] >> 16) == 0u ? 1u : 0u) << (16 + q);
+                const int pre = uni(it[IT_PRE]);
+                if (pre) {
+                    const uint32_t ptm = (uint32_t)PV.heavy_tab[pre - 1].z;
+                    const ulonglong2* const pslab = reinterpret_cast<const ulonglong2*>(PV.slab);
+                    for (int pq = 0; pq < PV.n; ++pq) {
+                        if (!((ptm >> pq) & 1u) || reinterpret_cast<const int*>(reinterpret_cast<const char*>(PV.stats[pq]) + 96)[HDR_FAIL] != 0) continue;
+                        const int w = PV.bslab[pq][rk];
+                        const int np = w >> SLAB_SLOT_BITS;
+                        const ulonglong2* const src = pslab + (size_t)(w & ((1 << SLAB_SLOT_BITS) - 1)) * TSL_BRK3 + threadIdx.x;
+                        long long ug = 0;
+#pragma unroll
+                        for (int h = 0; h < VPT; h += PCH) {
+                            ulonglong2 a[PCH];
+#pragma unroll
+                            for (int q = 0; q < PCH; ++q) a[q] = src[(h + q) * NT];
+                            for (int j = 1; j < np; ++j) {
+#pragma unroll
+                                for (int q = 0; q < PCH; ++q) { const ulonglong2 x = src[(size_t)j * TSL_BRK3 + (h + q) * NT]; a[q].x += x.x; a[q].y += x.y; }
+                            }
+#pragma unroll
+                            for (int q = 0; q < PCH; ++q) if (a[q].y != 0ull) {
+                                old[h + q] = apply_update(old[h + q], (long long)a[q].x, (long long)a[q].y);
+                                vmask |= 1u << (h + q); ++ug;
+                            }
+                        }
+                        ug = wave_sum_ll(ug);
+                        if (lane_id() == 0 && ug) atomicAdd(&s_uqp[pq], (int)ug);
+                    }
+                    if (threadIdx.x == 0) ++s_npre;
+                }
             }
 #pragma unroll
             for (int h = 0; h < VPT; h += CH) {
@@ -924,7 +964,7 @@
             if (lane_id() == 0 && u) atomicAdd(&s_uq[f], (int)u);
             uniq = 0;
         }
-        if (fetching) { commit(n_known == 0 ? slot1 : slot2, ne, nkq, nio, nin); ++n_known; }
+        if (fetching) { commit(n_known == 0 ? slot1 : slot2, ne, nkq, nio, nin, nip); ++n_known; }
 #ifdef TSL_TIMING
         if (threadIdx.x == 0 && last_step) _rec[4] = wall_clock64();
         if (threadIdx.x == 0) { _ph[2] += _td - _tc; _ph[3] += wall_clock64() - _td; }
@@ -940,6 +980,10 @@
 #undef TSL_SORT_DEAL
     __syncthreads();
     if (threadIdx.x < TSL_NB && s_uq[threadIdx.x]) atomic_add_i64(&B.f[threadIdx.x].stats->unique, (long long)s_uq[threadIdx.x]);
+    if (PV.n) {
+        if (threadIdx.x < TSL_NB && s_uqp[threadIdx.x]) atomic_add_i64(&PV.stats[threadIdx.x]->unique, (long long)s_uqp[threadIdx.x]);
+        if (threadIdx.x == 0 && s_npre) atomicAdd(M.pool_top + MAP_CTR_PREAPPLY, s_npre);
+    }
 }
 
 #ifndef APPLY_SPLIT
@@ -949,7 +993,7 @@
 #define APPLY_ROUND 2
 #endif
 template <bool TEX>
-__global__ void __launch_bounds__(256) k_apply_slab(MapDev M, BatchDev B)
+__global__ void __launch_bounds__(256) k_apply_slab(MapDev M, BatchDev B, NextDev NX)
 {
     __shared__ int s_uq[TSL_NB];
     constexpr int VP = TSL_BRK3 / APPLY_SPLIT / 256;
@@ -960,11 +1004,14 @@
     const ulonglong2* const slab = reinterpret_cast<const ulonglong2*>(B.f[0].acc);
     if (threadIdx.x < TSL_NB) s_uq[threadIdx.x] = 0;
     __syncthreads();
+    int nskip = 0;
     for (int item = blockIdx.x; item < nheavy * APPLY_SPLIT; item += gridDim.x) {
         const int4 e = B.f[0].heavy_tab[item / APPLY_SPLIT];
         const int b = e.x, p = e.y;
         const uint32_t tm = (uint32_t)e.z & okmask;
-        if (p < 0 || tm == 0u) continue;
+        if (p < 0) continue;
+        if (NX.umark && (NX.umark[b] >> PLAN_STAMP_SHIFT) == (NX.stamp >> PLAN_STAMP_SHIFT)) { if (item % APPLY_SPLIT == 0) ++nskip; continue; }
+        if (tm == 0u) continue;
         const int l0 = (item % APPLY_SPLIT) * (TSL_BRK3 / APPLY_SPLIT) + (int)threadIdx.x;
         uint32_t* tw = M.tw + (size_t)p * TSL_BRK3;
         int w[TSL_NB];
@@ -1037,6 +1084,7 @@
             if ((first[k] >> 16) == 0u) obs[l0 + k * 256] = 1;
         }
     }
+    if (threadIdx.x == 0 && nskip) atomicAdd(M.pool_top + MAP_CTR_SKIP, nskip);
 }
 
 int check_variant2(tsl_tsdf* m)
@@ -1059,31 +1107,36 @@
     int unit_half = std::min(unit_max, m->unit_half <= 2048 ? m->unit_half : std::max(2048, (int)((long long)m->unit_half * B.n / TSL_NB)));
     if (P.seq && m->seq_impl) unit_max = unit_half = 1 << 30;
     prof_begin(m, TSL_K_BIN, st);
-    hipLaunchKernelGGL(k_plan, dim3((B.f[0].max_frame_bricks + 255) / 256, B.n), dim3(256), 0, st, m->M, B, m->chunks * m->wg * m->spt, unit_max, unit_half);
+    hipLaunchKernelGGL(k_plan, dim3((B.f[0].max_frame_bricks + 255) / 256, B.n), dim3(256), 0, st, m->M, B, m->chunks * m->wg * m->spt, unit_max, unit_half, (long long)m->batch_seq);
     hipLaunchKernelGGL(k_scatter, dim3(256, B.n), dim3(256), 0, st, B);
     prof_end(m, st);
     return TSL_OK;
 }
 
-int launch_brick(tsl_tsdf* m, const BatchDev& B, const FrameParams& P, int kind, hipStream_t st, hipEvent_t start, hipEvent_t stop)
-{
+int launch_brick(tsl_tsdf* m, const BatchDev& B, const FrameParams& P, int kind, hipStream_t st, hipEvent_t start, hipEvent_t stop, const PrevDev* prev)
+{
+    PrevDev PV; std::memset(&PV, 0, sizeof(PV));
+    if (prev) PV = *prev;
     const int bg = kind == 2 ? m->pgrid : (B.n <= 2 ? (m->bgrid + 1) / 2 : (kind == 1 ? m->ugrid : m->bgrid));
 #define TSL_LAUNCH_IB(TEXV, FD) do { \
-        if (m->wg == 512 && m->spt == 2 && !TEXV) hipExtLaunchKernelGGL((k_integrate_batch<false, FD, 512, 2, 4>), dim3((2 * m->ncu * bg + 99) / 100), dim3(512), 0, st, start, stop, 0, m->M, B, kind); \
-        else if (m->wg == 512) hipExtLaunchKernelGGL((k_integrate_batch<TEXV, FD, 512, 4, 2>), dim3((m->ncu * bg + 99) / 100), dim3(512), 0, st, start, stop, 0, m->M, B, kind); \
-        else hipExtLaunchKernelGGL((k_integrate_batch<TEXV, FD, 256, 4, (TEXV ? 1 : 2)>), dim3(((TEXV ? 1 : 2) * m->ncu * bg + 99) / 100), dim3(256), 0, st, start, stop, 0, m->M, B, kind); } while (0)
+        if (m->wg == 512 && m->spt == 2 && !TEXV) hipExtLaunchKernelGGL((k_integrate_batch<false, FD, 512, 2, 4>), dim3((2 * m->ncu * bg + 99) / 100), dim3(512), 0, st, start, stop, 0, m->M, B, kind, PV); \
+        else if (m->wg == 512) hipExtLaunchKernelGGL((k_integrate_batch<TEXV, FD, 512, 4, 2>), dim3((m->ncu * bg + 99) / 100), dim3(512), 0, st, start, stop, 0, m->M, B, kind, PV); \
+        else hipExtLaunchKernelGGL((k_integrate_batch<TEXV, FD, 256, 4, (TEXV ? 1 : 2)>), dim3(((TEXV ? 1 : 2) * m->ncu * bg + 99) / 100), dim3(256), 0, st, start, stop, 0, m->M, B, kind, PV); } while (0)
     if (P.tex) { if (P.fastdiv) TSL_LAUNCH_IB(true, true); else TSL_LAUNCH_IB(true, false); }
     else { if (P.fastdiv) TSL_LAUNCH_IB(false, true); else TSL_LAUNCH_IB(false, false); }
 #undef TSL_LAUNCH_IB
     TSL_HIP(hipGetLastError());
     return TSL_OK;
 }
-int launch_slab_apply(tsl_tsdf* m, const BatchDev& B, const FrameParams& P)
-{
-    prof_begin(m, TSL_K_FINALIZE);
-    if (P.tex) hipLaunchKernelGGL(k_apply_slab<true>, dim3(16 * m->ncu), dim3(256), 0, m->stream_, m->M, B);
-    else hipLaunchKernelGGL(k_apply_slab<false>, dim3(16 * m->ncu), dim3(256), 0, m->stream_, m->M, B);
-    prof_end(m);
+int launch_slab_apply(tsl_tsdf* m, const BatchDev& B, const FrameParams& P, hipStream_t st, const NextDev* next)
+{
+    NextDev NX = { nullptr, 0ull };
+    if (next) NX = *next;
+    if (!st) st = m->stream_;
+    prof_begin(m, TSL_K_FINALIZE, st);
+    if (P.tex) hipLaunchKernelGGL(k_apply_slab<true>, dim3(16 * m->ncu), dim3(256), 0, st, m->M, B, NX);
+    else hipLaunchKernelGGL(k_apply_slab<false>, dim3(16 * m->ncu), dim3(256), 0, st, m->M, B, NX);
+    prof_end(m, st);
     TSL_HIP(hipGetLastError());
     return TSL_OK;
 }
diff --git a/taichislam_amd/csrc/tsl_tsdf.hip b/taichislam_amd/csrc/tsl_tsdf.hip
--- a/taichislam_amd/csrc/tsl_tsdf.hip
+++ b/taichislam_amd/csrc/tsl_tsdf.hip
@@ -504,6 +504,27 @@
     return launch_segments(m, B, hp, total, sa);
 }
 
+static void batch_dev_of(tsl_tsdf* m, int bi, int n, BatchDev* B)
+{
+    for (int q = 0; q < n; ++q) { FSet& S = m->fset[bi * TSL_NB + q]; B->f[q] = S.F; B->p[q] = S.Pd; }
+    for (int q = n; q < TSL_NB; ++q) { B->f[q] = B->f[0]; B->p[q] = B->p[0]; }
+    B->n = n;
+}
+int flush_apply(tsl_tsdf* m)
+{
+    if (!m->ap_out) return TSL_OK;
+    m->ap_out = false;
+    BatchHost& H = m->batch[m->ap_bi];
+    BatchDev B; batch_dev_of(m, m->ap_bi, m->ap_n, &B);
+    if (m->ap_prev_side) TSL_HIP(hipStreamWaitEvent(m->stream_, m->ap_prev, 0));
+    FrameParams P = m->P; P.tex = 0;
+    const int rc = launch_slab_apply(m, B, P);
+    TSL_HIP(hipEventRecord(H.x_done, m->stream_));
+    m->ap_prev = H.x_done; m->ap_prev_side = false;
+    H.b_done = H.x_done;
+    return rc;
+}
+
 template <typename K>
 static int launch_batch_t(tsl_tsdf* m)
 {
@@ -521,6 +542,10 @@
         m->shape_hash = (m->shape_hash ^ (uint32_t)n) * 16777619u;
     }
     hipStream_t sa = serial ? m->stream_ : H.st;
+    bool any = false, tex = false; for (int q = 0; q < n; ++q) { any = any || m->pend[q].total > 0; tex = tex || m->pend[q].tex; }
+    const bool defer = !serial && m->defer_apply && !m->split_launch && m->phases == 3 && m->pend[0].variant == 2 && !m->pend[0].seq && !tex && any;
+    const bool pre = defer && m->ap_out && m->ap_slot == m->pend[0].slot;
+    if (!pre) { int rc = flush_apply(m); if (rc) return rc; }
     const int ring = (int)(m->batch_seq % TSL_INFLIGHT);
     if (m->ring_upto[ring] > 0) {
         TSL_HIP(hipEventSynchronize(m->ring_ev[ring]));
@@ -547,9 +572,8 @@
     }
     m->nproducers = 0;
     BatchDev B; ParamPack PP;
-    for (int q = 0; q < n; ++q) { FSet& S = m->fset[bi * TSL_NB + q]; B.f[q] = S.F; B.p[q] = S.Pd; PP.p[q] = m->pend[q]; }
-    for (int q = n; q < TSL_NB; ++q) { B.f[q] = B.f[0]; B.p[q] = B.p[0]; PP.p[q] = PP.p[0]; }
-    B.n = n;
+    batch_dev_of(m, bi, n, &B);
+    for (int q = 0; q < TSL_NB; ++q) PP.p[q] = m->pend[q < n ? q : 0];
     SetPtrs SP;
     for (int q = 0; q < TSL_NB; ++q) { SP.p[q] = const_cast<FrameParams*>(B.p[q]); SP.header[q] = reinterpret_cast<int*>(B.f[q].stats); }
     hipLaunchKernelGGL(k_set_params, dim3(n), dim3(64), 0, sa, PP, SP);
@@ -579,7 +603,23 @@
         TSL_HIP(hipEventRecord(H.a_done, sa)); H.a_recorded = true;
         TSL_HIP(hipStreamWaitEvent(m->stream_, H.a_done, 0));
     }
-    bool any = false; for (int q = 0; q < n; ++q) any = any || m->pend[q].total > 0;
+    PrevDev PV; std::memset(&PV, 0, sizeof(PV));
+    BatchHost* const L = pre ? &m->batch[m->ap_bi] : nullptr;
+    if (pre) {
+        BatchDev BL; batch_dev_of(m, m->ap_bi, m->ap_n, &BL);
+        TSL_HIP(hipStreamWaitEvent(L->st, m->ap_brick, 0));
+        TSL_HIP(hipStreamWaitEvent(L->st, H.a_done, 0));
+        if (m->ap_prev) TSL_HIP(hipStreamWaitEvent(L->st, m->ap_prev, 0));
+        if (m->ap_prev_side) TSL_HIP(hipStreamWaitEvent(m->stream_, m->ap_prev, 0));
+        const NextDev NX = { B.f[0].umark, plan_stamp(m->batch_seq) };
+        FrameParams PL = m->pend[0]; PL.tex = 0;
+        int rc = launch_slab_apply(m, BL, PL, L->st, &NX);
+        if (rc) return rc;
+        TSL_HIP(hipEventRecord(L->x_done, L->st));
+        m->ap_prev = L->x_done; m->ap_prev_side = true; m->ap_out = false; ++m->deferred_applies;
+        PV.slab = BL.f[0].acc; PV.heavy_tab = BL.f[0].heavy_tab; PV.hmark = BL.f[0].hmark; PV.stamp = plan_stamp(m->ap_seq); PV.n = BL.n;
+        for (int q = 0; q < TSL_NB; ++q) { PV.bslab[q] = BL.f[q].bslab; PV.stats[q] = BL.f[q].stats; }
+    }
     const bool split = !serial && m->split_launch && (m->phases & 2) && m->pend[0].variant == 2 && !m->pend[0].seq && n > 2 && any;
     if (split) {
         hipEvent_t pa = nullptr, pb = nullptr;
@@ -601,6 +641,7 @@
                     TSL_HIP(hipStreamWaitEvent(m->stream_, H.p_done, 0));
                     if (!rc) rc = launch_slab_apply(m, B, m->pend[0]);
                 }
+                else if (defer) rc = launch_brick(m, B, m->pend[0], 0, m->stream_, timed ? ea : nullptr, timed ? eb : nullptr, pre ? &PV : nullptr);
                 else rc = launch_apply_batch(m, B, m->pend[0], timed ? ea : nullptr, timed ? eb : nullptr);
             }
         } else {
@@ -614,6 +655,8 @@
     }
     TSL_HIP(hipEventRecord(m->ring_ev[ring], m->stream_)); m->ring_upto[ring] = m->frames_issued; m->batch_seq++;
     if (!serial) { H.b_done = m->ring_ev[ring]; H.b_pending = true; }
+    if (pre) L->b_done = m->ring_ev[ring];
+    if (defer) { m->ap_out = true; m->ap_bi = bi; m->ap_n = n; m->ap_slot = m->pend[0].slot; m->ap_seq = m->batch_seq - 1; m->ap_brick = m->ring_ev[ring]; }
     m->cur = (bi + 1) % TSL_NBATCH;
     TSL_HIP(hipGetLastError());
     return TSL_OK;
@@ -627,7 +670,14 @@
     if (rc && !m->deferred_rc) m->deferred_rc = rc;
     return rc;
 }
-hipStream_t ms(tsl_tsdf* m) { if (m->clean) (void)hipGetLastError(); m->clean = false; (void)flush_pending(m); return m->stream_; }
+hipStream_t ms(tsl_tsdf* m)
+{
+    if (m->clean) (void)hipGetLastError();
+    m->clean = false;
+    (void)flush_pending(m);
+    if (m->ap_out) { const int rc = flush_apply(m); if (rc && !m->deferred_rc) m->deferred_rc = rc; }
+    return m->stream_;
+}
 
 static int batch_cap(const tsl_tsdf* m)
 { return (m->overlap > 0 && m->variant == 2 && m->P.group && (!m->semantics || m->seq_impl)) ? (m->overlap < TSL_NB ? m->overlap : TSL_NB) : 1; }
@@ -753,7 +803,9 @@
         if (si % TSL_NB == 0) {
             if ((rc = own((void**)&G.unit_tab, sizeof(int4) * 4 * (size_t)G.unit_cap))) return rc;
             if ((rc = own((void**)&G.heavy_tab, sizeof(int4) * (size_t)(F.max_frame_bricks + 8)))) return rc;
-        }
+            if ((rc = own((void**)&G.hmark, sizeof(unsigned long long) * (size_t)m->nb3))) return rc;
+            if ((rc = own((void**)&G.umark, sizeof(unsigned long long) * (size_t)m->nb3))) return rc;
+        } else { const FrameDev& G0 = m->fset[(si / TSL_NB) * TSL_NB].F; G.hmark = G0.hmark; G.umark = G0.umark; }
         if ((rc = own(&S.sort_temp, m->sort_temp_bytes + 256))) return rc;
         if ((rc = own((void**)&S.Pd, sizeof(FrameParams)))) return rc;
     }
@@ -859,8 +911,9 @@
     TSL_HIP(hipStreamCreateWithFlags(&m->stream_, hipStreamNonBlocking));
     m->overlap = TSL_NB; m->last_set = 0;
     for (auto& S : m->fset) { S.sort_temp = nullptr; S.header = nullptr; S.Pd = nullptr; S.stage_in = nullptr; S.stage_in_bytes = 0; S.stage_tex = nullptr; S.stage_tex_bytes = 0; S.pin = nullptr; S.pin_bytes = 0; S.pin_dev = nullptr; S.copy_in = S.copy_tex = S.copy_tex_off = 0; }
-    for (auto& H : m->batch) { H.st = nullptr; H.a_done = nullptr; H.b_done = nullptr; H.p_done = nullptr; H.c_done = nullptr; H.b_pending = false; H.a_recorded = false; H.c_recorded = false; }
+    for (auto& H : m->batch) { H.st = nullptr; H.a_done = nullptr; H.b_done = nullptr; H.p_done = nullptr; H.c_done = nullptr; H.x_done = nullptr; H.b_pending = false; H.a_recorded = false; H.c_recorded = false; }
     m->frames_issued = 0; m->frames_consumed = 0; m->batch_seq = 0;
+    m->defer_apply = 1; m->ap_out = false; m->ap_bi = 0; m->ap_n = 0; m->ap_slot = 0; m->ap_seq = 0; m->ap_brick = nullptr; m->ap_prev = nullptr; m->ap_prev_side = false; m->deferred_applies = 0;
     for (int k = 0; k < TSL_INFLIGHT; ++k) { m->ring_ev[k] = nullptr; m->ring_upto[k] = 0; }
     m->cur = 0; m->npend = 0; m->pend_points = 0; m->deferred_rc = 0;
     const int blk = cfg->num_voxel_per_blk_axis;
@@ -926,7 +979,7 @@
     if (cfg->texture_enabled) { if ((rc = dev_alloc(m, (void**)&M.col, sizeof(uint16_t) * 4 * (size_t)want * TSL_BRK3, 0))) return rc; }
     if ((rc = dev_alloc(m, (void**)&M.owner, sizeof(int) * (size_t)want, 0))) return rc;
     if ((rc = dev_alloc(m, (void**)&M.touch, (size_t)want, 0))) return rc;
-    if ((rc = dev_alloc(m, (void**)&M.pool_top, sizeof(int) * 4, 0))) return rc;
+    if ((rc = dev_alloc(m, (void**)&M.pool_top, sizeof(int) * 8, 0))) return rc;
     M.err = M.pool_top + 1;
 
     FrameDev& F = m->F; std::memset(&F, 0, sizeof(F));
@@ -950,6 +1003,7 @@
         TSL_HIP(hipEventCreateWithFlags(&H.a_done, evf));
         TSL_HIP(hipEventCreateWithFlags(&H.p_done, evf));
         TSL_HIP(hipEventCreateWithFlags(&H.c_done, evf));
+        TSL_HIP(hipEventCreateWithFlags(&H.x_done, evf));
     }
     for (int k = 0; k < TSL_INFLIGHT; ++k) TSL_HIP(hipEventCreateWithFlags(&m->ring_ev[k], evf));
     TSL_HIP(hipStreamCreateWithFlags(&m->copy_st, hipStreamNonBlocking));
@@ -1007,6 +1061,7 @@
         if (H.a_done) (void)hipEventDestroy(H.a_done);
         if (H.p_done) (void)hipEventDestroy(H.p_done);
         if (H.c_done) (void)hipEventDestroy(H.c_done);
+        if (H.x_done) (void)hipEventDestroy(H.x_done);
     }
     for (auto& S : m->fset) {
 
@@ -1059,6 +1114,7 @@
     if (m->clean && m->npend == 0 && !m->deferred_rc) return TSL_OK;
     TSL_HIP(hipSetDevice(m->device));
     int rc = flush_pending(m);
+    if (m->ap_out) { const int ra = flush_apply(m); if (!rc) rc = ra; }
     for (auto& H : m->batch) if (H.st) TSL_HIP(hipStreamSynchronize(H.st));
     if (m->copy_st) TSL_HIP(hipStreamSynchronize(m->copy_st));
     const int ec = take_dev_err(m);
@@ -1133,6 +1189,10 @@
     if (!std::strcmp(name, "overlapped_launches")) { *value = (int)m->batch_seq - m->dry_launches; return TSL_OK; }
     if (!std::strcmp(name, "variant")) { *value = m->variant; return TSL_OK; }
     if (!std::strcmp(name, "split")) { *value = m->split; return TSL_OK; }
+    if (!std::strcmp(name, "defer_apply")) { *value = m->defer_apply; return TSL_OK; }
+    if (!std::strcmp(name, "deferred_applies")) { *value = (int)(m->deferred_applies > 0x7fffffffll ? 0x7fffffffll : m->deferred_applies); return TSL_OK; }
+    if (!std::strcmp(name, "unit_preapplies")) { int rc = tsl_tsdf_sync(m); if (rc) return rc; return read_int(m, m->M.pool_top + MAP_CTR_PREAPPLY, value); }
+    if (!std::strcmp(name, "apply_skips")) { int rc = tsl_tsdf_sync(m); if (rc) return rc; return read_int(m, m->M.pool_top + MAP_CTR_SKIP, value); }
     set_error("unknown option"); return TSL_ERR_ARG;
 }
 int tsl_tsdf_bricks_in_use(tsl_tsdf* m, int32_t* n)
@@ -1529,6 +1589,7 @@
     if (!std::strcmp(name, "ramp")) { TSL_REQUIRE(value >= 0 && value <= 16, "ramp must be 0..16 half batches"); m->ramp_batches = value; return TSL_OK; }
     if (!std::strcmp(name, "ugrid") || !std::strcmp(name, "pgrid")) { TSL_REQUIRE(value >= 5 && value <= 200, "ugrid / pgrid must be 5..200 (percent of the resident workgroup slots)"); { int rc = tsl_tsdf_sync(m); if (rc) return rc; } (name[0] == 'u' ? m->ugrid : m->pgrid) = value; return TSL_OK; }
     if (!std::strcmp(name, "split_launch")) { TSL_REQUIRE(value == 0 || value == 1, "split_launch must be 0 or 1"); { int rc = tsl_tsdf_sync(m); if (rc) return rc; } m->split_launch = value; return TSL_OK; }
+    if (!std::strcmp(name, "defer_apply")) { TSL_REQUIRE(value == 0 || value == 1, "defer_apply must be 0 or 1"); { int rc = tsl_tsdf_sync(m); if (rc) return rc; } m->defer_apply = value; return TSL_OK; }
     if (!std::strcmp(name, "bgrid")) { TSL_REQUIRE(value >= 10 && value <= 200, "bgrid must be 10..200 (percent of the resident workgroup slots)"); { int rc = tsl_tsdf_sync(m); if (rc) return rc; } m->bgrid = value; return TSL_OK; }
     if (!std::strcmp(name, "spt")) { TSL_REQUIRE(value == 2 || value == 4, "spt must be 2 or 4"); { int rc = tsl_tsdf_sync(m); if (rc) return rc; } m->spt = value; return TSL_OK; }
     if (!std::strcmp(name, "wg")) { TSL_REQUIRE(value == 256 || value == 512, "wg must be 256 or 512"); { int rc = tsl_tsdf_sync(m); if (rc) return rc; } m->wg = value; return TSL_OK; }
diff --git a/taichislam_amd/csrc/tsl_tsdf.hpp b/taichislam_amd/csrc/tsl_tsdf.hpp
--- a/taichislam_amd/csrc/tsl_tsdf.hpp
+++ b/taichislam_amd/csrc/tsl_tsdf.hpp
@@ -47,6 +47,7 @@
     int4  *part_tab; int part_cap;
     int4  *unit_tab; int unit_cap;
     int4  *heavy_tab;
+    unsigned long long *hmark, *umark;
     int*   slot_tab;
     int*   touched;
     int*   touched_b;
@@ -82,6 +83,11 @@
 #define HDR_SEQ_CLAIM 35
 #define HDR_SEQ_SLOTS 29
 
+#define PLAN_STAMP_SHIFT 16
+__host__ __device__ __forceinline__ unsigned long long plan_stamp(long long seq) { return (unsigned long long)(seq + 1) << PLAN_STAMP_SHIFT; }
+#define MAP_CTR_PREAPPLY 4
+#define MAP_CTR_SKIP 5
+
 __device__ __forceinline__ void frame_fail(const MapDev& M, const FrameDev& F, int bits) { atomicOr(&F.counters[11], bits); atomicOr(M.err, bits); }
 
 #define H_INL 13
@@ -179,9 +185,11 @@
     std::vector<void*> owned;
 };
 struct BatchDev { FrameDev f[TSL_NB]; const FrameParams* p[TSL_NB]; int n; };
+struct PrevDev { const unsigned long long* slab; const int4* heavy_tab; const unsigned long long* hmark; unsigned long long stamp; const int* bslab[TSL_NB]; tsl_frame_stats* stats[TSL_NB]; int n; };
+struct NextDev { const unsigned long long* umark; unsigned long long stamp; };
 struct ParamPack { FrameParams p[TSL_NB]; };
 struct SetPtrs { FrameParams* p[TSL_NB]; int* header[TSL_NB]; };
-struct BatchHost { hipStream_t st; hipEvent_t a_done, b_done, p_done, c_done; bool b_pending, a_recorded, c_recorded; };
+struct BatchHost { hipStream_t st; hipEvent_t a_done, b_done, p_done, c_done, x_done; bool b_pending, a_recorded, c_recorded; };
 struct StageCopy { const uint4* src[2 * TSL_NB]; uint4* dst[2 * TSL_NB]; int n16[2 * TSL_NB]; };
 #define TSL_INFLIGHT 8
 
@@ -202,6 +210,9 @@
     int64_t frames_issued, frames_consumed;
     int64_t batch_seq; hipEvent_t ring_ev[TSL_INFLIGHT]; int64_t ring_upto[TSL_INFLIGHT];
     int last_set, last_batch_n;
+    int defer_apply; bool ap_out; int ap_bi, ap_n, ap_slot; int64_t ap_seq; hipEvent_t ap_brick;
+    hipEvent_t ap_prev; bool ap_prev_side;
+    int64_t deferred_applies;
     hipStream_t producers[4]; int nproducers;
     hipEvent_t in_ev[8]; int in_ev_next;
     bool scratch_ready;
@@ -264,8 +275,9 @@
 int  launch_segments(tsl_tsdf* m, const BatchDev& B, const FrameParams* hp, int total, hipStream_t st);
 int  launch_apply(tsl_tsdf* m, FSet& S, int total);
 int  launch_apply_batch(tsl_tsdf* m, const BatchDev& B, const FrameParams& P, hipEvent_t start = nullptr, hipEvent_t stop = nullptr);
-int  launch_brick(tsl_tsdf* m, const BatchDev& B, const FrameParams& P, int kind, hipStream_t st, hipEvent_t start, hipEvent_t stop);
-int  launch_slab_apply(tsl_tsdf* m, const BatchDev& B, const FrameParams& P);
+int  launch_brick(tsl_tsdf* m, const BatchDev& B, const FrameParams& P, int kind, hipStream_t st, hipEvent_t start, hipEvent_t stop, const PrevDev* prev = nullptr);
+int  launch_slab_apply(tsl_tsdf* m, const BatchDev& B, const FrameParams& P, hipStream_t st = nullptr, const NextDev* next = nullptr);
+int  flush_apply(tsl_tsdf* m);
 int  launch_seq_group(tsl_tsdf* m, const BatchDev& B, const FrameParams* hp, int bi, hipStream_t st);
 int  launch_seq_apply(tsl_tsdf* m, const BatchDev& B, const FrameParams& P, int bi);
 void seq_release(tsl_tsdf* m);
```

Result: slower. 28210 frames/s (-18.4%).
